# chrhansk/sleqp

Hardware: AMD Instinct MI355X
Metric: KKT factor+solve/sec (numeric refactor + 1 solve with device-controlled refinement, inputs resident in HBM) (higher is better)
Workload: dtype f64; 1 GPU; banded_n1e5_m5e4; n=100000, m=50000, N=150000, nnz_J=1000000, nnz_tril_K=1100000, nnz_L=11646539, nnz_L_stored=12226637, supernodes=569, etree_levels=10, refine_steps=1, hip_graphs=5, solves_per_factor=1, parallelism=single

## Files before the change

sleqp_amd/csrc/abi_options.inc:

```
enum OptionEffect {
  FX_NONE,
  FX_GRAPHS,
  FX_GRAPHS_IF_CHANGED,
  FX_PLANS,
  FX_PLANS_IF_CHANGED,
};
struct OptionRow {
  const char* name;
  const char* env;
  OptionEffect effect;
  int (*set)(hipfact_handle* h, double v);
  const char* doc;
};
#define OPT_STORE(field, conv)                 \
  [](hipfact_handle* h, double v) -> int {     \
    const auto x = (conv);                     \
    const bool changed = h->field != x;        \
    h->field = x;                              \
    return changed;                            \
  }
static const OptionRow kOptions[] = {
    {"refine_steps", "HIPFACT_REFINE", FX_GRAPHS,
     [](hipfact_handle* h, double v) -> int {
       h->refine_steps = std::max(0, (int)v);
// ... 68 lines not shown
       h->check_interval_now = 0;
       return 1;
     },
     "residual check on every k-th solve of a well-conditioned factorisation"},
    {"decide_lazy", "HIPFACT_DECIDE_LAZY", FX_GRAPHS_IF_CHANGED,
     [](hipfact_handle* h, double v) -> int {
       const bool changed = h->decide_lazy != (v != 0.0);
       if (changed) flush_decide(h);
       h->decide_lazy = v != 0.0;
       return changed;
     },
     "0: every solve graph ends with its own verdict launch"},
    {"rhs_fused", "HIPFACT_RHS_FUSED", FX_GRAPHS_IF_CHANGED, OPT_STORE(rhs_fused, v != 0.0),
     "0: k_rhs_saddle in front of the single-launch solve"},
    {"spanel_fold", "HIPFACT_SPANEL_FOLD", FX_PLANS_IF_CHANGED, OPT_STORE(spanel_fold, v != 0.0),
     "0: the solve panels in a launch of their own behind the factorisation"},
    {"spanel_fold_room", nullptr, FX_PLANS_IF_CHANGED, OPT_STORE(spanel_fold_room, (int)v),
     "solve-panel items dealt in beside a level's own pivot and panel items of the dataflow launch: workgroup slots per level (default 224)"},
    {"factor_hint_peek", "HIPFACT_HINT_PEEK", FX_NONE, OPT_STORE(factor_hint_peek, v != 0.0),
     "0: a refactorisation does not look at the last delivered refinement verdict (every first solve graph carries a correction pass)"},
    {"top_block_breakeven", nullptr, FX_NONE, OPT_STORE(top_block_breakeven, (int)v),
     "solves of one factorisation from which forming the dense top block of the solve tree pays (default 48)"},
    {"solve_fused", nullptr, FX_PLANS, OPT_STORE(solve_fused, v != 0.0),
     "0: the per-level solve kernels on the factor panels"},
    {"top_block_after", "HIPFACT_TOP_BLOCK_AFTER", FX_PLANS, OPT_STORE(top_block_after, std::max(0, (int)v)),
     "the top levels of the solve tree as one dense block from this solve of a factorisation on (0: never)"},
    {"boundary_fast", "HIPFACT_BOUNDARY_FAST", FX_NONE,
     [](hipfact_handle* h, double v) -> int {
       h->boundary_fast = v != 0.0;
       h->sol_prefetched = false;
       return 1;
     },
     "0: host vectors through pageable borrows and three blocking points (round 3)"},
    {"validate_rhs", nullptr, FX_NONE, OPT_STORE(validate_rhs, v != 0.0),
     "walk the index array of every sparse right-hand side on the host (debug)"},
    {"boundary_profile", nullptr, FX_NONE,
     [](hipfact_handle* h, double v) -> int {
       int rc = enter(h);
       if (rc) return rc;
       h->bd_profile = v != 0.0;
       if (h->bd_profile)
         for (hipEvent_t& ev : h->bd_ev)
           if (!ev) HCHECK(h, hipEventCreate(&ev));
       h->bd_stage_us = h->bd_queue_us = h->bd_rhs_us = h->bd_device_us = h->bd_d2h_us = h->bd_wait_us = h->bd_copyout_us = 0;
       h->bd_count = 0;
       h->bd_pending = false;
       return 1;
     },
     "where solve + solution spend their time (info keys bd_*); resets the sums"},
    {"superset_vtable", nullptr, FX_NONE,
     [](hipfact_handle* h, double v) -> int {
       const bool changed = h->superset_vtable != (v != 0.0);
       if (changed) h->vj->clear();
       h->superset_vtable = v != 0.0;
       return changed;
     },
     "0: no reuse across working sets (every changed pattern is analysed on its own rows; active bounds are still eliminated - exact_pattern = 1 for K as it is)"},
    {"spmv_stream", nullptr, FX_NONE, OPT_STORE(spmv_stream, v != 0.0),
     "0: every sparse product through the lanes-per-row kernel (default: matrices from spmv_stream_min entries on are streamed in row blocks)"},
    {"spmv_stream_min", nullptr, FX_NONE, OPT_STORE(spmv_stream_min, (long long)v),
     "entries from which a sparse product is streamed (default 4 M: below, the matrix lives in the Infinity Cache)"},
    {"exact_pattern", nullptr, FX_NONE,
     [](hipfact_handle* h, double v) -> int {
       const bool changed = h->exact_pattern != (v != 0.0);
       if (changed) h->vj->clear();
       h->exact_pattern = v != 0.0;
       return changed;
     },
     "1: K is analysed exactly as given - no row dictionary, unit rows of active bounds stay in the structure (what hipfact_reduced_matrix needs)"},
    {"assemble_superset", nullptr, FX_NONE, OPT_STORE(assemble_superset, v != 0.0),
     "0: hipfact_assemble_kkt analyses every working set on its own rows (no superset plan)"},
    {"plan_cache", nullptr, FX_NONE,
     [](hipfact_handle* h, double v) -> int {
       h->plan_cache_max = std::max(0, (int)v);
       while ((int)h->cache.size() > h->plan_cache_max) h->cache.pop_back();
       return 1;
     },
     "inactive plan states kept (LRU); 0: one pattern at a time"},
    {"profile", nullptr, FX_NONE,
     [](hipfact_handle* h, double v) -> int {
       if (h->prof.on) prof_collect(h);
       if (v < 0)
         for (int c = 0; c < PC_COUNT; ++c) h->prof.ms[c] = 0, h->prof.max_ms[c] = 0, h->prof.cnt[c] = 0;
       h->prof.tagged.clear();
       h->prof.on = v > 0;
       return 1;
     },
     "event-time every kernel class; value < 0 resets the counters"},
    {"ordering", nullptr, FX_PLANS, OPT_STORE(prm.ordering, (int)v),
     "0 nested dissection + AMD leaves (default), 1 AMD on the whole graph, 2 natural"},
    {"max_children", nullptr, FX_PLANS, OPT_STORE(prm.max_children, (int)v),
     "relaxed amalgamation keeps fronts at this many children (default 4 = what the pull extend-add takes in one block)"},
    {"force_generic", nullptr, FX_PLANS, OPT_STORE(prm.force_generic, v != 0.0),
     "1: no saddle-point structure detection, static 1 x 1 pivots on K as given (symmetric positive definite input: the PSD shim)"},
    {"dense_mode", nullptr, FX_PLANS, OPT_STORE(prm.dense_mode, std::min(2, std::max(0, (int)v))),
     "1: late elimination inside the tree (default), 2: low-rank correction, 0: off"},
    {nullptr, "HIPFACT_DATAFLOW_RETRY", FX_NONE, OPT_STORE(df_retry_every, std::max(0, (int)v)), nullptr},
    {nullptr, "HIPFACT_CHECK_LAUNCHES", FX_NONE, OPT_STORE(check_launches, v != 0.0), nullptr},
    {nullptr, "HIPFACT_SOL_SPLIT", FX_NONE, OPT_STORE(sol_split, v != 0.0), nullptr},
    {nullptr, "HIPFACT_XCD_CLASSES", FX_NONE, OPT_STORE(xcd_classes, std::max(1, std::min(XCD_CLASSES_MAX, (int)v))), nullptr},
};
#undef OPT_STORE

static void options_from_environment(hipfact_handle* h) {
  for (const OptionRow& row : kOptions)
    if (const char* s = row.env ? getenv(row.env) : nullptr) (void)row.set(h, (double)atoi(s));
}

int hipfact_set_option(hipfact_handle* h, const char* name, double value) {
  if (!h || !name) return HIPFACT_EINVAL;
  {
    bool known = false;
    const int rc = multi_set_option(h, name, value, known);
    if (known) return rc;
  }
  for (const OptionRow& row : kOptions) {
    if (!row.name || strcmp(name, row.name)) continue;
    const int changed = row.set(h, value);
    if (changed < 0) return changed;
    if (row.effect == FX_GRAPHS || (row.effect == FX_GRAPHS_IF_CHANGED && changed)) drop_graphs(h);
    if (row.effect == FX_PLANS || (row.effect == FX_PLANS_IF_CHANGED && changed)) invalidate_plans(h);
    return HIPFACT_OK;
  }
  h->error = std::string("unknown option: ") + name;
  return HIPFACT_EINVAL;
}

int hipfact_debug_copy(hipfact_handle* h, const char* name, void* out, size_t bytes) {
  int rc = enter(h);
  if (rc) return rc;
  if (!name || !out) return HIPFACT_EINVAL;
  auto host_copy = [&](const auto& v) {
    if (bytes > v.size() * sizeof(v[0])) {
      h->error = "hipfact_debug_copy: unknown buffer or size";
      return HIPFACT_EINVAL;
    }
    if (bytes) memcpy(out, v.data(), bytes);
    return HIPFACT_OK;
  };
  const Plan& P = h->plan;
  if (!strcmp(name, "perm")) return host_copy(P.perm);
  if (!strcmp(name, "sn_c0")) return host_copy(P.sn_c0);
  if (!strcmp(name, "sn_r")) return host_copy(P.sn_r);
  if (!strcmp(name, "sn_rowptr")) return host_copy(P.sn_rowptr);
  if (!strcmp(name, "sn_rows")) return host_copy(P.sn_rows);
  if (!strcmp(name, "sn_Loff")) return host_copy(P.sn_Loff);
  if (!strcmp(name, "late_cols")) return host_copy(P.late_cols);
  if (!strcmp(name, "sn_level")) return host_copy(P.sn_level);
  if (!strcmp(name, "dense_cols")) return host_copy(P.dense_cols);
  const DevBuf* b = nullptr;
  if (!strcmp(name, "L")) b = &h->d_L;
  else if (!strcmp(name, "U")) b = &h->d_U;
  else if (!strcmp(name, "SPf")) b = &h->d_SPf;
  else if (!strcmp(name, "SPb")) b = &h->d_SPb;
  else if (!strcmp(name, "sitems")) b = &h->d_sitems;
  else if (!strcmp(name, "y")) b = &h->d_y;
  else if (!strcmp(name, "xhat")) b = &h->d_xhat;
  else if (!strcmp(name, "ysol")) b = &h->d_ysol;
  else if (!strcmp(name, "uvec")) b = &h->d_uvec;
  else if (!strcmp(name, "dscale")) b = &h->d_dscale;
  else if (!strcmp(name, "Kval")) b = &h->d_Kval;
  else if (!strcmp(name, "mY")) b = &h->d_mY;
  if (!b || !b->p || bytes > b->bytes) {
    h->error = "hipfact_debug_copy: unknown buffer or size";
    return HIPFACT_EINVAL;
  }
  HCHECK(h, hipStreamSynchronize(h->stream));
  HCHECK(h, hipMemcpy(out, b->p, bytes, hipMemcpyDeviceToHost));
  return HIPFACT_OK;
}

int hipfact_debug_place_rows(int m, const int* Ar_ptr, long long fill_bytes, int classes, long long* bounds, int* classes_out,
                             int* grid_out, int* blocks) {
  if (m < 0 || (m > 0 && !Ar_ptr) || fill_bytes < 0 || classes < 1 || classes > XCD_CLASSES_MAX || !bounds || !classes_out ||
      !grid_out || !blocks)
    return HIPFACT_EINVAL;
  ClassBounds cb;
  *grid_out = place_rows(m, Ar_ptr, (size_t)fill_bytes, classes, cb);
  *classes_out = cb.C;
  for (int g = 0; g <= cb.C; ++g) bounds[g] = cb.b[g];
  for (int g = 0; g < cb.C; ++g) class_row_blocks(cb, g, FB / RL, blocks[2 * g], blocks[2 * g + 1]);
  return HIPFACT_OK;
}
int hipfact_debug_place_items(int nfronts, const int* counts, int classes, int* order, int* lost) {
  if (nfronts < 0 || (nfronts > 0 && !counts) || classes < 1 || classes > XCD_CLASSES_MAX) return HIPFACT_EINVAL;
  long long total = 0;
  for (int f = 0; f < nfronts; ++f) {
    if (counts[f] < 0) return HIPFACT_EINVAL;
    total += counts[f];
  }
  if (total >= (1LL << 31) || (total > 0 && (!order || !lost))) return HIPFACT_EINVAL;
  std::vector<int> o, l;
  deal_items(std::vector<int>(counts, counts + nfronts), classes, o, &l);
  for (size_t i = 0; i < o.size(); ++i) {
    order[i] = o[i];
    lost[i] = l[i];
  }
  return HIPFACT_OK;
}

int hipfact_debug_multi_slices(int u, int slice_rows, int* tile_bounds, int cap) {
  if (u < 0 || !multi_slice_rows_valid(slice_rows)) return HIPFACT_EINVAL;
  const int ns = multi_nslice(u, slice_rows);
  if (tile_bounds && ns <= cap)
    for (int k = 0; k <= ns; ++k) tile_bounds[k] = multi_slice_tile(u, ns, k);
  return ns;
}

int hipfact_get_info(const hipfact_handle* h, const char* name, double* value) {
  if (!h || !name || !value) return HIPFACT_EINVAL;
  const Plan& P = h->plan;
  if (!strncmp(name, "prof_", 5)) {
    prof_collect(const_cast<hipfact_handle*>(h));
    if (!strcmp(name, "prof_schur_best_flops") || !strcmp(name, "prof_schur_best_ms")) {
      double fmax = 0.0, best_rate = 0.0, bf = 0.0, bm = 0.0;
      for (auto& t : h->prof.tagged) fmax = std::max(fmax, t.first);
      for (auto& t : h->prof.tagged)
        if (t.first >= 0.5 * fmax && t.second > 0.0 && t.first / t.second > best_rate) {
          best_rate = t.first / t.second;
          bf = t.first;
          bm = t.second;
        }
      *value = !strcmp(name, "prof_schur_best_flops") ? bf : bm;
      return HIPFACT_OK;
    }
    for (int c = 0; c < PC_COUNT; ++c) {
      const size_t len = strlen(kProfNames[c]);
      if (!strncmp(name + 5, kProfNames[c], len) && name[5 + len] == '_') {
        if (!strcmp(name + 6 + len, "ms")) {
          *value = h->prof.ms[c];
          return HIPFACT_OK;
        }
        if (!strcmp(name + 6 + len, "count")) {
          *value = (double)h->prof.cnt[c];
          return HIPFACT_OK;
        }
        if (!strcmp(name + 6 + len, "max_ms")) {
          *value = h->prof.max_ms[c];
          return HIPFACT_OK;
        }
      }
    }
    return HIPFACT_EINVAL;
  }
  if (!strncmp(name, "level_", 6)) {
    const char* us = strrchr(name, '_');
    const int l = atoi(us + 1);
    if (us == name + 5 || l < 0 || l >= P.nlevels || (int)P.level_ptr.size() <= l + 1) return HIPFACT_EINVAL;
    const size_t len = (size_t)(us - (name + 6));
    double fronts = 0, ent = 0, rows = 0, flops = 0, blk = 0;
    for (int q = P.level_ptr[l]; q < P.level_ptr[l + 1]; ++q) {
      const int s = P.level_sn[q];
      const double w = P.sn_c0[s + 1] - P.sn_c0[s], r = P.sn_r[s];
      fronts += 1;
      ent += w * r - w * (w - 1) / 2;
      blk += w * (w + 1) / 2;
      rows += r;
      for (int k = 0; k < (int)w; ++k) flops += (r - k) * (r - k);
    }
    if (len == 6 && !strncmp(name + 6, "fronts", 6)) *value = fronts;
    else if (len == 3 && !strncmp(name + 6, "ent", 3)) *value = ent;
    else if (len == 3 && !strncmp(name + 6, "blk", 3)) *value = blk;
    else if (len == 4 && !strncmp(name + 6, "rows", 4)) *value = rows;
    else if (len == 5 && !strncmp(name + 6, "flops", 5)) *value = flops;
    else return HIPFACT_EINVAL;
    return HIPFACT_OK;
  }
#define INFO(key, expr)       \
  if (!strcmp(name, key)) {   \
    *value = (double)(expr);  \
    return HIPFACT_OK;        \
  }
  INFO("N", h->have_plan ? h->N_ext : P.N) INFO("n", P.n) INFO("m", P.m) INFO("saddle", P.saddle) INFO("nnzK", P.nnzK) INFO("nnzL", P.nnzL)
  INFO("nnzL_true", P.nnzL_true) INFO("flops", P.flops) INFO("flops_dense", P.flops_dense) INFO("nsuper", P.nsuper)
  INFO("nlevels", P.nlevels) INFO("nprod", P.nprod) INFO("L_bytes", P.L_size * 8.0) INFO("U_bytes", P.U_size * 8.0)
  INFO("analysis_s", P.t_total) INFO("order_s", P.t_order) INFO("symbolic_s", P.t_symbolic)
  INFO("num_perturbed", h->num_perturbed) INFO("static_pivot_runs", h->static_pivot_runs) INFO("static_pivot_shift", h->reg_delta)
  INFO("num_zero_pivots", h->info_host[INFO_ZERO_PIVOT]) INFO("num_neg_pivots", h->info_host[INFO_NEG_PIVOT])
  INFO("cache_hits", h->cache_hits) INFO("plan_swaps", h->plan_swaps) INFO("plans_cached", h->cache.size())
  INFO("no_dataflow", h->no_dataflow) INFO("dataflow_fallbacks", h->dataflow_fallbacks) INFO("turn_waits", (double)h->turn_waits) INFO("dataflow_rearmed", h->dataflow_rearmed) INFO("fused_solve", h->fused_solve) INFO("spanel_folded", h->sp_folded) INFO("solve_items", h->n_sitems) INFO("chain_levels_fused", [&] { int c = 0; for (const LevelInfo& li : h->levels) c += li.mini_cnt > 0; return c; }()) INFO("solve_panel_bytes", h->sp_bytes) INFO("spf_bytes", (double)h->d_SPf.bytes) INFO("spb_bytes", (double)h->d_SPb.bytes) INFO("sitem_bytes", (double)sizeof(SolveItem)) INFO("N_internal", P.N) INFO("maps_on", h->maps_on) INFO("m_struct", h->m_struct) INFO("analyses", h->analyses) INFO("num_factor", h->num_factor) INFO("cg_device_runs", h->cg_device_runs) INFO("cg_device_fallbacks", h->cg_device_fallbacks) INFO("lz_device_runs", h->lz_device_runs) INFO("lz_device_fallbacks", h->lz_device_fallbacks) INFO("lz_device_iterations", h->lz_device_iterations) INFO("lsqr_runs", h->lsqr_runs) INFO("lsqr_iters", h->lsqr_iters) INFO("dense_columns", h->nd) INFO("late_columns", P.n_late) INFO("late_rows", P.n_late_rows) INFO("m_rows", P.saddle ? P.my : P.m) INFO("vtable_rows", h->vj->rows()) INFO("vtable_retries", h->vtable_retries) INFO("dense_fallbacks", h->dense_fallbacks) INFO("dense_probes", h->dense_probes) INFO("top_block_cols", h->tb_nT) INFO("top_block_below", h->tb_nfb) INFO("top_block_levels", h->tb_levels) INFO("top_block_items", h->tb_ntf) INFO("top_block_builds", h->tb_builds) INFO("top_block_active", h->tb_valid) INFO("superset_vtable", h->superset_vtable) INFO("exact_pattern", h->exact_pattern) INFO("spmv_stream", h->spmv_stream)
  INFO("boundary_fast", h->boundary_fast) INFO("bd_count", h->bd_count) INFO("bd_stage_us", h->bd_stage_us) INFO("bd_queue_us", h->bd_queue_us) INFO("bd_rhs_us", h->bd_rhs_us) INFO("bd_device_us", h->bd_device_us) INFO("bd_d2h_us", h->bd_d2h_us) INFO("bd_wait_us", h->bd_wait_us) INFO("bd_copyout_us", h->bd_copyout_us)
  INFO("multi_solves", h->multi_solves) INFO("multi_cols", h->multi_cols) INFO("multi_blocks", h->multi_blocks)
  INFO("multi_passes", h->multi_passes) INFO("multi_single_cols", h->multi_single_cols) INFO("multi_failed_col", h->multi_failed_col)
  INFO("multi_sliced_fronts", h->mitems_for < 0 ? 0 : h->n_mcut) INFO("multi_slice_items", h->mitems_for < 0 ? 0 : h->n_mslices) INFO("multi_slice_rows", h->multi_slice_rows)
  INFO("extra_solves", h->extra_solves) INFO("extra_passes", h->extra_passes) INFO("extra_last_status", h->extra_last_status)
  INFO("num_solve", h->num_solve) INFO("num_refined", h->num_refined) INFO("refine_adaptive", h->refine_adaptive)
  INFO("num_passes", h->num_passes) INFO("last_omega", h->last_ctl.omega) INFO("last_iters", h->last_ctl.iters)
  INFO("last_status", h->last_ctl.status) INFO("last_tol", h->last_ctl.tol) INFO("kappa_est", h->last_ctl.kappa)
  INFO("refine_inline", h->refine_inline) INFO("refine_tol", h->refine_tol) INFO("equilibrate", h->equilibrate)
  INFO("factor_top_level", h->ftop_level) INFO("factor_top_count", h->ftop_count) INFO("solve_timeouts", h->h_info.p ? h->h_info.as<int>()[INFO_TIMEOUT] : 0)
  INFO("top_level", 1 << 30)
  INFO("use_graph", h->use_graph) INFO("num_graphs", h->graphs.size()) INFO("max_r", P.max_r) INFO("max_w", P.max_w) INFO("refine_steps", h->refine_steps)
  INFO("schur_flops_max_level", h->schur_flops_max)
  INFO("chain_pairs", h->n_pairs)
  INFO("xupd_fused", h->xupd_fused ? 1 : 0)
  INFO("rhs_in_tree", h->last_rhs_in_tree) INFO("xupd_in_tree", h->last_xupd_in_tree) INFO("xupd_blocks_launched", h->last_xupd_blocks)
  INFO("solve_sliced_fronts", h->n_sliced) INFO("solve_resorted_levels", h->n_resorted) INFO("tree_solve", tree_solve(h))
  INFO("refine_check_every", h->refine_check_every) INFO("refine_check_interval", h->check_interval_now) INFO("num_checked", h->num_checked)
  INFO("device", h->device) INFO("nnzM", P.Mi.size()) INFO("nnzA", P.Ar_src.size())
  INFO("rows_total", P.sn_rows.size()) INFO("ent_fused", h->ent_fused) INFO("ent_split", h->ent_split)
  INFO("rows_fused", h->rows_fused) INFO("rows_split", h->rows_split)
  INFO("long_row_segments", h->n_rseg) INFO("row_scale_blocks", row_scale_in_sequence(h) ? h->rs_grid : 0)
  INFO("arena_fill_bytes", arena_fill_bytes(P))
  INFO("xcd_classes", h->xcd_classes) INFO("dealt_multi_item_fronts", h->dealt_multi) INFO("long_prod_segments", h->n_lprod)
  INFO("active_bounds", h->maps_on ? h->n_bounds : 0)
  INFO("values_in_place",
       h->have_plan && (!h->from_jacobian || (virtual_current(h) && h->vj->identity))) INFO("inactive_rows", h->maps_on ? h->n_inactive : 0)
#undef INFO
  return HIPFACT_EINVAL;
}
```

sleqp_amd/csrc/device_types.h:

```cpp
#pragma once
#include <cstdint>

namespace hipfact {

struct SnDesc {
  long long Loff;
  long long Uoff;
  long long uoff;
  long long rowoff;
  long long reloff;
  int c0;
  int w;
  int r;
  int parent;
  int child_begin;
  int child_end;
  int pad0;
  int pad1;
};

constexpr int MAXCH = 4;
struct PullDesc {
  long long Uoff[MAXCH];
  long long reloff[MAXCH];
  int invoff[MAXCH];
  int uc[MAXCH];
  int n;
  int next;
  int pad[2];
};

struct FrontItem {
  long long Loff, Uoff;
  int w, r;
  int part;
  int nchild;
  PullDesc pd;
};

struct PairDesc {
  long long Loff_a, Uoff_g;
  int w_a, r_a, rowoff_a;
  int u_g, off_g;
};

struct TopFItem {
  FrontItem it;
  int role;
  int front;
  int part2;
  int nwait;
  int wait_id[MAXCH];
  int wait_cnt[MAXCH];
  int target;
  int crows;
  int prows;
  int sidx, scount;
  int post;
  long long xoff;
  int head;
  int wait_head[MAXCH];
};

struct SolveItem {
  long long spf, spb;
  long long uoff, rowoff;
  int c0, w, r, nchild;
  int Qf, Ef, Pb, Eb;
  long long c_uoff[MAXCH];
  int c_invoff[MAXCH];
  long long Loff;
  int xbegin, xend;
  int a0, a1, sl, nsl;
  long long poff;
  int plevel, pad_;
};
constexpr int LONG_ROW = 1024;
constexpr int LONG_COL = 256;
constexpr int LONG_SEG = 2048;
struct LongSeg {
  int id;
  int begin, end;
  int idx, nseg;
  int uid;
  int poff;
  int pad;
};
struct LongProd {
  long long e;
  long long begin, end;
  int idx, nseg, uid, poff;
};
constexpr int XCD_CLASSES_MAX = 16;
struct ClassBounds {
  long long b[XCD_CLASSES_MAX + 1];
  int C, pad;
};
#ifdef __HIP__
#define HIPFACT_HD __host__ __device__
#else
#define HIPFACT_HD
#endif
HIPFACT_HD inline void class_row_blocks(const ClassBounds& cb, int g, int rpb, int& rb0, int& nrb) {
  rb0 = (int)((cb.b[g] + rpb - 1) / rpb);
  nrb = (int)((cb.b[g + 1] + rpb - 1) / rpb) - rb0;
}
struct TopBlockItem {
  long long off;
  int r0, nr;
  int Q, E;
};
struct TopFront {
  int item;
  int parent;
  int tl0;
  int pad;
};
struct TopChunk {
  int front;
  int j0;
};
constexpr int TOP_CB = 4;
constexpr int TOP_LDS = 7 * 1024 + 512;
constexpr int SPMV_NNZ = 2048;
constexpr int SPMV_T = 256;
constexpr int TREE_LDS = 2 * 1024 + 8;
struct TopBlockIn {
  int nT, ntf;
  const TopBlockItem* __restrict__ items;
  const double* __restrict__ XTf;
  const int* __restrict__ tpos;
  const int* __restrict__ gptr;
  const long long* __restrict__ gsrc;
  double* __restrict__ xhatT2;
  double* __restrict__ tT2;
  int ntr;
  unsigned int* __restrict__ gathered2;
  int ltop;
};
constexpr int SOLVE_PREFETCH = 32;

enum { INFO_ZERO_PIVOT = 0, INFO_NEG_PIVOT = 1, INFO_TIMEOUT = 2, INFO_TIMEOUT_WG = 3, INFO_WORDS = 4 };
constexpr int INFO_BYTES = INFO_WORDS * 4 + 32;

}
```

sleqp_amd/csrc/kernels_factor_top.inc:

```

__device__ __forceinline__ void flag_wait_ge(int* __restrict__ addr, int target, int* __restrict__ info) {
  if (threadIdx.x == 0) {
    int spins = 0;
    while (__hip_atomic_load(addr, __ATOMIC_RELAXED, __HIP_MEMORY_SCOPE_AGENT) < target) {
      __builtin_amdgcn_s_sleep(2);
      if (++spins > (1 << 22)) {
        atomicAdd(&info[INFO_TIMEOUT], 1);
        break;
      }
    }
    __builtin_amdgcn_fence(__ATOMIC_ACQUIRE, "agent");
    asm volatile("s_waitcnt vmcnt(0)" ::: "memory");
  }
  __syncthreads();
}

__device__ __forceinline__ void flag_publish_add(int* __restrict__ addr) {
  asm volatile("s_waitcnt vmcnt(0)" ::: "memory");
  __syncthreads();
  if (threadIdx.x == 0) {
    FACTOR_RELEASE_FENCE();
    asm volatile("s_waitcnt vmcnt(0)" ::: "memory");
    __hip_atomic_fetch_add(addr, 1, __ATOMIC_RELAXED, __HIP_MEMORY_SCOPE_AGENT);
  }
}

__device__ __forceinline__ void dev_build_solve_panel(const SolveItem& T, const double* __restrict__ L,
                                                      double* __restrict__ SPf, double* __restrict__ SPb, double* lds);

__global__ __launch_bounds__(512) void k_factor_top(const TopFItem* __restrict__ items, double* __restrict__ L,
                                                   double* __restrict__ U, int* __restrict__ info,
                                                   const int* __restrict__ inv, const int* __restrict__ rel,
                                                   int* __restrict__ bdone, int* __restrict__ cdone,
                                                   int* __restrict__ ddone, double* __restrict__ xarena,
                                                   const SolveItem* __restrict__ sitems, double* __restrict__ SPf,
                                                   double* __restrict__ SPb) {
  extern __shared__ __attribute__((aligned(16))) double lds[];
  const TopFItem& T = items[blockIdx.x];
  const FrontItem& S = T.it;
  TRW(0);
#ifdef HIPFACT_TRACE
  if (threadIdx.x == 0 && blockIdx.x < TRACE_WGS) g_trace[blockIdx.x * 8 + 7] = T.role * 100000 + T.front;
#endif
  if (T.role == 3) {
    if (T.nwait) {
      if (threadIdx.x == 0) {
        int spins = 0;
        while ((__hip_atomic_load(&bdone[T.front], __ATOMIC_RELAXED, __HIP_MEMORY_SCOPE_AGENT) & 15) < 1 ||
               __hip_atomic_load(&cdone[T.front], __ATOMIC_RELAXED, __HIP_MEMORY_SCOPE_AGENT) < T.target) {
          __builtin_amdgcn_s_sleep(8);
          if (++spins > (1 << 22)) {
            atomicAdd(&info[INFO_TIMEOUT], 1);
            break;
          }
        }
        __builtin_amdgcn_fence(__ATOMIC_ACQUIRE, "agent");
        asm volatile("s_waitcnt vmcnt(0)" ::: "memory");
      }
      __syncthreads();
    }
    TRW(1);
    dev_build_solve_panel(sitems[S.part], L, SPf, SPb, lds);
#ifdef HIPFACT_TRACE
    __syncthreads();
#endif
    TRW(2);
    return;
  }
  FrontCtx c = make_ctx(S, L, U, lds);
  c.wt = true;
  c.Xa = T.post ? xarena + T.xoff : nullptr;
  const PullCtx pc = make_pull(S.pd, U, inv, rel, 1);
  ChildWait cw;
  cw.n = T.nwait;
  cw.info = info;
#pragma unroll
  for (int ch = 0; ch < MAXCH; ++ch) {
    cw.addr[ch] = ddone + T.wait_id[ch];
    cw.target[ch] = T.wait_cnt[ch];
  }
  if (T.role == 0) {
    int* hdone = ddone + (ddone - cdone);
#pragma unroll
    for (int ch = 0; ch < MAXCH; ++ch)
      if (T.wait_head[ch] > 0 && ch < T.nwait && T.wait_cnt[ch] > 0) {
        cw.addr[ch] = hdone + T.wait_id[ch];
        cw.target[ch] = T.wait_head[ch];
      }
  }
  if (T.role == 0) {
    dev_pivot_block<false, false, true>(c, info, 15, pc, cw);
    dev_store_pivot_block(c);
    TRW(2);
    flag_publish_add(&bdone[T.front]);
    TRW(3);
    if (T.sidx > 0) {
      const SolveItem& Q = sitems[T.sidx - 1];
      const int w = c.w, r = c.r, lda = c.lda;
      const int lane = threadIdx.x & 63, wave = threadIdx.x >> 6;
      const long long TSf = (long long)r * Q.Qf, TSb = (long long)w * Q.Pb;
      double* __restrict__ sf = SPf + Q.spf;
      double* __restrict__ sb = SPb + Q.spb;
      for (int k = wave; k < w; k += 8) {
        const long long of = (long long)(k / Q.Qf) * TSf + (long long)(k % Q.Qf) * r;
        for (int i = k + lane; i < w; i += 64) sf[of + i] = (i == k) ? 1.0 : c.A[i + k * lda];
      }
      for (int i = wave; i < w; i += 8) {
        const double di = 1.0 / c.dd[i];
        const long long ob = (long long)(i / Q.Pb) * TSb + (long long)(i % Q.Pb) * w;
        for (int k = lane; k <= i; k += 64) sb[ob + k] = ((i == k) ? 1.0 : c.A[i + k * lda]) * di;
      }
    }
  } else if (T.role == 1) {
    TRW(5);
    cw.wait();
    int* invl = reinterpret_cast<int*>(c.A + c.wp * c.lda);
#pragma unroll
    for (int ch = 0; ch < MAXCH; ++ch)
      if (ch < pc.n)
        for (int k = threadIdx.x; k < c.wp; k += blockDim.x) invl[ch * c.wp + k] = (k < c.w) ? pc.inv[ch][k] : -1;
    const int wv = threadIdx.x >> 6;
    const int cstep = T.prows == 64 ? 2 : 1;
    const int R0 = c.w + T.prows * S.part + 16 * (cstep == 2 ? (wv >> 1) : wv);
    double pv[8][4];
    int cis[MAXCH];
    if (c.Xa) {
      const bool mine = 16 * wv < T.prows;
      const int R1 = c.w + T.prows * S.part + 16 * wv;
      const int Rs = mine ? R1 : c.r;
      dev_panel_rows_load<true>(c, Rs, pc, pv, cis);
      __syncthreads();
      dev_panel_rows_gather<true>(c, pc, invl, pv, cis);
      TRW(1);
      dev_panel_rows_subst_posted(c, Rs, pv, mine && R1 < c.r, S.part == 0, info);
      TRW(2);
      flag_publish_add(&cdone[T.front]);
      TRW(3);
      return;
    }
    dev_panel_rows_load(c, R0, pc, pv, cis);
    __syncthreads();
    dev_panel_rows_gather(c, pc, invl, pv, cis);
    if (c.Xa) {
      dev_panel_rows_product_posted(c, R0, pv, cstep, cstep == 2 ? (wv & 1) : 0, R0 < c.r, info);
    } else {
      flag_wait_ge(&bdone[T.front], 1, info);
      TRW(1);
      dev_load_pivot_block(c, true, true);
      if (R0 < c.r) dev_panel_rows_product<true, true>(c, R0, pv, cstep, cstep == 2 ? (wv & 1) : 0);
    }
    TRW(2);
    flag_publish_add(&cdone[T.front]);
    TRW(3);
  } else if (T.role == 4) {
#define FUSED_ARGS c, S.part >> 16, S.part & 0xffff, pc, cw, info, &bdone[T.front], &cdone[T.front], &ddone[T.front], T.target
    if (T.crows == 32) {
      if (c.nbk == 6)
        dev_fused_tile<32, 6>(FUSED_ARGS);
      else
        dev_fused_tile<32, 0>(FUSED_ARGS);
    } else {
      if (c.nbk == 6)
        dev_fused_tile<64, 6>(FUSED_ARGS);
      else
        dev_fused_tile<64, 0>(FUSED_ARGS);
    }
#undef FUSED_ARGS
  } else {
    cw.wait();
    if (T.crows == 64) {
      dev_schur_tile32(c, S.part >> 16, S.part & 0xffff, pc, &cdone[T.front], T.target, info);
    } else {
      const int team = threadIdx.x >> 8;
      const int ij = team ? T.part2 : S.part;
      double* SI = c.A + (size_t)team * (2 * 64 * KC + 64 * MAXCH);
      dev_schur_tile<false>(c, SI, SI + 64 * KC, ij < 0 ? -1 : (ij >> 16), ij & 0xffff, S.nchild == 0, pc,
                            threadIdx.x & 255, &cdone[T.front], T.target, info);
    }
    if (c.Xa)
      for (int e = T.sidx * 512 + threadIdx.x; e < c.wp * c.wp; e += T.scount * 512) sent_f64(c.Xa + e);
    TRW(2);
    flag_publish_add(&ddone[T.front]);
    if (T.head && threadIdx.x == 0)
      __hip_atomic_fetch_add(ddone + (ddone - cdone) + T.front, 1, __ATOMIC_RELAXED, __HIP_MEMORY_SCOPE_AGENT);
    TRW(3);
  }
}
```

sleqp_amd/csrc/kernels_solve_panels.inc:

```
#define SPST(p, v) (*(p) = (v))

__device__ __forceinline__ void dev_build_solve_panel(const SolveItem& T, const double* __restrict__ L,
                                                      double* __restrict__ SPf, double* __restrict__ SPb, double* lds) {
  const int w = T.w, r = T.r;
  const int ua = T.a0, u = T.a1 - T.a0;
  const int top = (T.sl == 0) ? w : 0;
  const int ro = top + u;
  const int tid = threadIdx.x, lane = tid & 63, wave = tid >> 6;
  const int li = lane & 15, lk = lane >> 4;
  const int nbk = (w + 15) >> 4, wp = nbk << 4;
  const int ldx = wp + 1;
  const double* __restrict__ Pn = L + T.Loff;
  double* X = lds;
  double* dinv = X + (size_t)ldx * wp;
  double* tile = dinv + wp + (size_t)wave * (16 * 17);
  long long* offF = reinterpret_cast<long long*>(dinv + wp + (SPB / 64) * (16 * 17));
  long long* offB = offF + wp;
  const int nstrip = (u + 15) >> 4;
  double av[32];
  {
    const int a0 = wave << 4;
    const bool rowok = wave < nstrip && a0 + li < u;
    const double* __restrict__ Lr = Pn + w + ua + a0 + li;
#pragma unroll
    for (int t = 0; t < 32; ++t) {
      const int j = 4 * t + lk;
      av[t] = (rowok && j < w) ? Lr[(long long)j * r] : 0.0;
    }
  }
  for (int k0 = wave; k0 < wp; k0 += 8 * (SPB / 64)) {
    double v[8][2];
#pragma unroll
    for (int t = 0; t < 8; ++t)
#pragma unroll
      for (int h2 = 0; h2 < 2; ++h2) {
        const int k = k0 + t * (SPB / 64), i = lane + 64 * h2;
        v[t][h2] = (i == k) ? 1.0 : 0.0;
        if (i < w && k < w && i > k) v[t][h2] = Pn[i + (long long)k * r];
      }
#pragma unroll
    for (int t = 0; t < 8; ++t)
#pragma unroll
      for (int h2 = 0; h2 < 2; ++h2) {
        const int k = k0 + t * (SPB / 64), i = lane + 64 * h2;
        if (k < wp && i < wp) X[i + k * ldx] = v[t][h2];
      }
  }
  for (int k = tid; k < wp; k += SPB) dinv[k] = (k < w) ? 1.0 / Pn[k + (long long)k * r] : 1.0;
  const int Qf = T.Qf, Pb = T.Pb;
  const long long TSf = (long long)ro * Qf, TSb = (long long)w * Pb;
  for (int k = tid; k < wp; k += SPB) offF[k] = (long long)(k / Qf) * TSf + (long long)(k % Qf) * ro;
  for (int i = tid; i < ro; i += SPB) offB[i] = (long long)(i / Pb) * TSb + (long long)(i % Pb) * w;
  __syncthreads();
  double* __restrict__ sf = SPf + T.spf;
  double* __restrict__ sb = SPb + T.spb;
  for (int st = wave; st < nstrip; st += SPB / 64) {
    const int a0 = st << 4;
    d4_t acc[8];
#pragma unroll
    for (int t = 0; t < 8; ++t) acc[t] = d4_t{0.0, 0.0, 0.0, 0.0};
#pragma unroll
    for (int t = 0; t < 32; ++t) {
      const int j0 = 4 * t;
      if (j0 < wp) {
#pragma unroll
        for (int kt = 0; kt < 8; ++kt)
          if (16 * kt <= j0 + 3 && kt < nbk) acc[kt] = MFMA_F64(av[t], X[(j0 + lk) + (16 * kt + li) * ldx], acc[kt]);
      }
    }
    {
      const int an = (st + SPB / 64) << 4;
      const bool rowok = st + SPB / 64 < nstrip && an + li < u;
      const double* __restrict__ Lr = Pn + w + ua + an + li;
#pragma unroll
      for (int t = 0; t < 32; ++t) {
        const int j = 4 * t + lk;
        av[t] = (rowok && j < w) ? Lr[(long long)j * r] : 0.0;
      }
    }
#pragma unroll
    for (int kt = 0; kt < 8; ++kt) {
      if (kt >= nbk) continue;
#pragma unroll
      for (int q = 0; q < 4; ++q) {
        const int row = lk + 4 * q, k = 16 * kt + li, i = top + a0 + row;
        tile[row * 17 + li] = -acc[kt][q];
        if (a0 + row < u && k < w) SPST(&sb[offB[i] + k], -acc[kt][q]);
      }
      __builtin_amdgcn_fence(__ATOMIC_RELEASE, "wavefront");
      __builtin_amdgcn_wave_barrier();
      __builtin_amdgcn_fence(__ATOMIC_ACQUIRE, "wavefront");
#pragma unroll
      for (int q = 0; q < 4; ++q) {
        const int row = li, col = lk + 4 * q, k = 16 * kt + col, i = top + a0 + row;
        if (a0 + row < u && k < w) SPST(&sf[offF[k] + i], tile[row * 17 + col]);
      }
      __builtin_amdgcn_fence(__ATOMIC_RELEASE, "wavefront");
      __builtin_amdgcn_wave_barrier();
    }
  }
  if (top == 0) return;
  for (int k = wave; k < w; k += SPB / 64)
    for (int i = k + lane; i < w; i += 64) SPST(&sf[offF[k] + i], X[i + k * ldx]);
  for (int i = wave; i < w; i += SPB / 64) {
    const double di = dinv[i];
    for (int k = lane; k <= i; k += 64) SPST(&sb[offB[i] + k], X[i + k * ldx] * di);
  }
}
__global__ __launch_bounds__(SPB) void k_build_solve_panels(const SolveItem* __restrict__ items,
                                                            const double* __restrict__ L, double* __restrict__ SPf,
                                                            double* __restrict__ SPb) {
  extern __shared__ __attribute__((aligned(16))) double lds[];
  dev_build_solve_panel(items[blockIdx.x], L, SPf, SPb, lds);
}
```

sleqp_amd/csrc/kernels_solve_tree.inc:

```

__device__ __forceinline__ void dev_refine_decide(const DecideIn& D, int first) {
  RefineCtl* __restrict__ ctl = D.ctl;
  RefineCtl* __restrict__ hctl = D.hctl;
  __shared__ double sh[3][16];
  const int tid = threadIdx.x, nthr = blockDim.x;
  double r = 0.0, bb = 0.0, zz = 0.0;
  for (int q = tid; q < D.nblk; q += nthr) {
    r = nanmax(r, D.partials[3 * q]);
    bb = nanmax(bb, D.partials[3 * q + 1]);
    zz = nanmax(zz, D.partials[3 * q + 2]);
  }
#pragma unroll
  for (int o = 32; o > 0; o >>= 1) {
    r = nanmax(r, __shfl_down(r, o, 64));
    bb = nanmax(bb, __shfl_down(bb, o, 64));
    zz = nanmax(zz, __shfl_down(zz, o, 64));
  }
  if ((tid & 63) == 0) {
    sh[0][tid >> 6] = r;
    sh[1][tid >> 6] = bb;
    sh[2][tid >> 6] = zz;
  }
  __syncthreads();
  if (tid == 0) {
// ... 23 lines not shown
    } else if (!first && omega > 0.5 * prev) {
      done = 1;
      status = 1;
    }
    ctl->iters = iters;
    ctl->omega_prev = prev;
    ctl->omega = omega;
    ctl->tol = tol;
    ctl->kappa = kappa;
    ctl->rnorm = r;
    ctl->bnorm = bb;
    ctl->status = status;
    ctl->seq = seq;
    ctl->pending = 0;
    ctl->done = done;
    hctl->iters = iters;
    hctl->omega_prev = prev;
    hctl->omega = omega;
    hctl->tol = tol;
    hctl->kappa = kappa;
    hctl->rnorm = r;
    hctl->bnorm = bb;
    hctl->status = status;
    hctl->done = done;
    __hip_atomic_store(&hctl->seq, seq, __ATOMIC_RELAXED, __HIP_MEMORY_SCOPE_SYSTEM);
  }
}
__global__ __launch_bounds__(FB) void k_refine_decide(DecideIn D, int first, int pending_only) {
  if (pending_only) {
    if (!D.ctl->pending) return;
  } else if (!first && D.ctl->done) {
    return;
  }
  dev_refine_decide(D, first);
}

__device__ __forceinline__ double rhs_row_tail(const RhsIn& R, int k, double s) {
  const int i = ext_row(R.M, R.perm[k]);
  return i >= 0 ? s - R.b[i] * R.M.dscale[k] : (i == -2 ? s : 0.0);
}
template <int NT>
__device__ __forceinline__ void rhs_long_rows(const RhsIn& R, int bid, int nb, double* __restrict__ t, double* lds) {
  for (int q = bid; q < R.M.nrseg; q += nb) {
    const LongSeg sg = R.M.rseg[q];
    double s = 0.0;
    for (int p = sg.begin + (int)threadIdx.x; p < sg.end; p += NT) {
      const int j = R.Ar_col[p], v = R.M.vmap ? R.M.vmap[j] : -1;
      s += R.Ar_val[p] * R.b[v >= 0 ? v : j];
    }
    s = block_sum_fixed<NT>(s, lds);
    double tot;
    if (threadIdx.x == 0 && seg_arrive(s, sg.poff, sg.idx, sg.nseg, R.M.segpart, R.M.segcnt + sg.uid, tot))
      t[sg.id] = rhs_row_tail(R, sg.id, tot);
  }
}
__device__ __forceinline__ double rhs_row(const RhsIn& R, int k, int sub) {
  double s = 0.0;
  const int p1 = R.Ar_ptr[k + 1];
  if (p1 - R.Ar_ptr[k] > LONG_ROW) return 0.0;
  if (R.M.vmap) {
    for (int p = R.Ar_ptr[k] + sub; p < p1; p += RL) {
      const int j = R.Ar_col[p], v = R.M.vmap[j];
      s += R.Ar_val[p] * R.b[v >= 0 ? v : j];
    }
  } else {
    for (int p = R.Ar_ptr[k] + sub; p < p1; p += RL) s += R.Ar_val[p] * R.b[R.Ar_col[p]];
  }
#pragma unroll
  for (int o = RL / 2; o > 0; o >>= 1) s += __shfl_down(s, o, RL);
  if (sub == 0) s = rhs_row_tail(R, k, s);
  return s;
}

__device__ __forceinline__ void dev_solve_fwd(const SolveItem& T, const double* __restrict__ SPf,
                                              const long long* __restrict__ xuoff, const int* __restrict__ xinvoff,
                                              const int* __restrict__ inv, const double* __restrict__ y,
                                              double* __restrict__ xhat, double* __restrict__ uvec,
                                              double* __restrict__ ysol, double* lds, int* __restrict__ info,
                                              const RhsIn& R) {
  const int tid = threadIdx.x;
  const int w = T.w, Q = T.Qf, E = T.Ef;
  const int a0 = T.a0, nu = T.a1 - T.a0;
  const int top = (T.sl == 0) ? w : 0;
  const int ro = top + nu;
  const int rl = w + nu;
  const int TS = ro * Q;
  const bool active = tid < TS;
  const int q = active ? tid / ro : 0;
  double* f = lds;
  double* part = lds + rl;
  if (tid < w) sent_f64(ysol + T.c0 + tid);
  const double* __restrict__ sp = SPf + T.spf + tid;
  double pv[SOLVE_PREFETCH];
  const int myrow_f = tid - q * ro;
  const int clim = (active && myrow_f < top) ? myrow_f : (1 << 30);
#pragma unroll
  for (int e = 0; e < SOLVE_PREFETCH; ++e) pv[e] = (active && e < E && q + Q * e <= clim) ? sp[(long long)e * TS] : 0.0;
  const int fr = tid + (tid >= w ? a0 : 0);
  double f0 = 0.0;
  if (R.Ar_ptr) {
    for (int row = tid / RL; row < w; row += ST / RL) {
      const double s = rhs_row(R, T.c0 + row, tid % RL);
      if (tid % RL == 0) part[row] = s;
    }
    __syncthreads();
    if (tid < w) f0 = part[tid];
  } else if (tid < w) {
    f0 = y[T.c0 + tid];
  }
  int iv[MAXCH];
#pragma unroll
  for (int ch = 0; ch < MAXCH; ++ch) iv[ch] = (ch < T.nchild && tid < rl) ? inv[T.c_invoff[ch] + fr] : -1;
  {
    unsigned long long bits[MAXCH];
#pragma unroll
    for (int ch = 0; ch < MAXCH; ++ch)
      bits[ch] = iv[ch] >= 0 ? __hip_atomic_load(reinterpret_cast<const unsigned long long*>(uvec + T.c_uoff[ch] + iv[ch]),
                                                 __ATOMIC_RELAXED, __HIP_MEMORY_SCOPE_AGENT)
                             : 0ull;
#pragma unroll
    for (int ch = 0; ch < MAXCH; ++ch)
      if (iv[ch] >= 0) {
        if (bits[ch] == SOLVE_SENT) bits[ch] = (unsigned long long)__double_as_longlong(poll_f64(uvec + T.c_uoff[ch] + iv[ch], info));
        f0 += __longlong_as_double((long long)bits[ch]);
      }
  }
  for (int x = T.xbegin; x < T.xend; ++x) {
    const int ia = (tid < rl) ? inv[xinvoff[x] + fr] : -1;
    if (ia >= 0) f0 += poll_f64(uvec + xuoff[x] + ia, info);
  }
  if (tid < rl) f[tid] = f0;
  __syncthreads();
  double acc = 0.0;
#pragma unroll
  for (int e = 0; e < SOLVE_PREFETCH; ++e)
    if (e < E) acc = fma(pv[e], f[min(q + Q * e, w - 1)], acc);
  for (int e = SOLVE_PREFETCH; e < E; ++e)
    if (active && q + Q * e <= clim) acc = fma(sp[(long long)e * TS], f[min(q + Q * e, w - 1)], acc);
  if (active) part[tid] = acc;
  __syncthreads();
  if (tid < ro) {
    double s2 = 0.0;
    for (int qq = 0; qq < Q; ++qq) s2 += part[qq * ro + tid];
    if (tid < top) {
      post_f64(xhat + T.c0 + tid, s2);
    } else {
      const int j = tid - top;
      post_f64(uvec + T.uoff + a0 + j, f[w + j] + s2);
    }
  }
}

template <bool DEFER_RESET>
__device__ __forceinline__ void dev_solve_bwd(const SolveItem& T, const double* __restrict__ SPb,
                                              const int* __restrict__ rows, double* __restrict__ y,
                                              double* __restrict__ xhat, double* __restrict__ uvec,
                                              double* __restrict__ ysol, double* __restrict__ spart, double* lds,
                                              int* __restrict__ info, const unsigned int* __restrict__ gathered = nullptr,
                                              int ngather = 0) {
  const int tid = threadIdx.x;
  const int w = T.w, P = T.Pb, E = T.Eb;
  const int a0 = T.a0, nu = T.a1 - T.a0;
  const int top = (T.sl == 0) ? w : 0;
  const int ro = top + nu;
  const int TS = w * P;
  const bool active = tid < TS;
  const int p = active ? tid / w : 0;
  double* tv = lds;
  double* part = lds + ro;
  const double* __restrict__ sp = SPb + T.spb + tid;
  double pv[SOLVE_PREFETCH];
  const int mycol_b = tid - p * w;
#pragma unroll
  for (int e = 0; e < SOLVE_PREFETCH; ++e) {
    const int row = p + P * e;
    pv[e] = (active && e < E && !(row < top && row < mycol_b)) ? sp[(long long)e * TS] : 0.0;
  }
  const int myrow = (tid >= top && tid < ro) ? rows[T.rowoff + w + a0 + (tid - top)] : -1;
  if (tid < top) {
    tv[tid] = poll_f64(xhat + T.c0 + tid, info);
    sent_f64_agent(xhat + T.c0 + tid);
  } else if (myrow >= 0) {
    tv[tid] = poll_f64(ysol + myrow, info);
  }
  if constexpr (!DEFER_RESET) {
    if (tid >= top && tid < ro) sent_f64_agent(uvec + T.uoff + a0 + (tid - top));
  }
  __syncthreads();
  double acc = 0.0;
#pragma unroll
  for (int e = 0; e < SOLVE_PREFETCH; ++e)
    if (e < E) acc = fma(pv[e], tv[min(p + P * e, ro - 1)], acc);
  for (int e = SOLVE_PREFETCH; e < E; ++e)
    if (active && !(p + P * e < top && p + P * e < mycol_b)) acc = fma(sp[(long long)e * TS], tv[min(p + P * e, ro - 1)], acc);
  if (active) part[tid] = acc;
  __syncthreads();
  if (tid < w) {
    double s2 = 0.0;
    for (int pp = 0; pp < P; ++pp) s2 += part[pp * w + tid];
    if (T.sl > 0) {
      post_f64(spart + T.poff + (long long)(T.sl - 1) * w + tid, s2);
    } else {
      for (int s0 = 1; s0 < T.nsl; s0 += 16) {
        unsigned long long bits[16];
#pragma unroll
        for (int j = 0; j < 16; ++j) {
          const int s = s0 + j;
          bits[j] = s < T.nsl ? __hip_atomic_load(reinterpret_cast<const unsigned long long*>(
                                                      spart + T.poff + (long long)(s - 1) * w + tid),
                                                  __ATOMIC_RELAXED, __HIP_MEMORY_SCOPE_AGENT)
                              : 0ull;
        }
#pragma unroll
        for (int j = 0; j < 16; ++j) {
          const int s = s0 + j;
          if (s < T.nsl) {
            double* slot = spart + T.poff + (long long)(s - 1) * w + tid;
            if (bits[j] == SOLVE_SENT) bits[j] = (unsigned long long)__double_as_longlong(poll_f64(slot, info));
            s2 += __longlong_as_double((long long)bits[j]);
            sent_f64_agent(slot);
          }
        }
      }
      y[T.c0 + tid] = s2;
      post_f64(ysol + T.c0 + tid, s2);
    }
  }
  if constexpr (DEFER_RESET) {
   if (tid >= top && tid < ro) {
    int spins = 0;
    while ((int)__hip_atomic_load(gathered, __ATOMIC_RELAXED, __HIP_MEMORY_SCOPE_AGENT) < ngather) {
      __builtin_amdgcn_s_sleep(1);
      if (++spins > (1 << 20)) {
        atomicAdd(&info[INFO_TIMEOUT], 1);
        atomicMax(&info[INFO_TIMEOUT_WG], (1 << 30) - (int)blockIdx.x);
        break;
      }
    }
    sent_f64_agent(uvec + T.uoff + a0 + (tid - top));
   }
  }
}

__device__ __forceinline__ void dev_top_one(const TopBlockIn& B, const TopBlockItem& I, double* __restrict__ y,
                                            const double* __restrict__ uvec, double* __restrict__ ysol_prev,
                                            double* __restrict__ ysol, int par, double* lds, int* __restrict__ info) {
  const int tid = threadIdx.x;
  const int nT = B.nT, nr = I.nr, Q = I.Q, E = I.E;
  const int TS = nr * Q;
  const bool active = tid < TS;
  const int q = tid % Q, rho = tid / Q;
  double* f = lds;
  double* part = lds + nT;
  const double* __restrict__ sp = B.XTf + I.off + tid;
  double pv[SOLVE_PREFETCH];
#pragma unroll
  for (int e = 0; e < SOLVE_PREFETCH; ++e) pv[e] = (active && e < E) ? sp[(long long)e * TS] : 0.0;
  if (tid < nr) {
    sent_f64(ysol_prev + B.tpos[I.r0 + tid]);
    sent_f64(B.tT2 + (size_t)(1 - par) * nT + I.r0 + tid);
  }
  if (tid == 0 && I.r0 == 0) __hip_atomic_store(B.gathered2 + (1 - par), 0u, __ATOMIC_RELAXED, __HIP_MEMORY_SCOPE_AGENT);
  const double* __restrict__ tT = B.tT2 + (size_t)par * nT;
  int* gp = reinterpret_cast<int*>(lds + nT + ST);
  int* gs = gp + nT + 1;
  const int nG = B.gptr[nT];
  for (int i = tid; i <= nT; i += ST) gp[i] = B.gptr[i];
  for (int g = tid; g < nG; g += ST) gs[g] = (int)B.gsrc[g];
  __syncthreads();
  constexpr int GK = 6;
  for (int i = tid; i < nT; i += ST) {
    const int g0 = gp[i], g1 = gp[i + 1];
    unsigned long long bits[GK + 1];
    const double* src[GK + 1];
    src[0] = B.ntr > 0 ? tT + i : y + B.tpos[i];
#pragma unroll
    for (int k = 0; k < GK; ++k) src[k + 1] = (g0 + k < g1) ? uvec + gs[g0 + k] : nullptr;
#pragma unroll
    for (int k = 0; k <= GK; ++k)
      bits[k] = src[k] ? __hip_atomic_load(reinterpret_cast<const unsigned long long*>(src[k]), __ATOMIC_RELAXED,
                                           __HIP_MEMORY_SCOPE_AGENT)
                       : 0ull;
    double f0 = 0.0;
#pragma unroll
    for (int k = 0; k <= GK; ++k)
      if (src[k]) {
        if (bits[k] == SOLVE_SENT && !(k == 0 && B.ntr == 0)) bits[k] = (unsigned long long)__double_as_longlong(poll_f64(src[k], info));
        f0 += __longlong_as_double((long long)bits[k]);
      }
    for (int g = g0 + GK; g < g1; ++g) f0 += poll_f64(uvec + gs[g], info);
    f[i] = f0;
  }
  __syncthreads();
  double acc = 0.0;
#pragma unroll
  for (int e = 0; e < SOLVE_PREFETCH; ++e)
    if (e < E) acc = fma(pv[e], f[min(q + Q * e, nT - 1)], acc);
  for (int e = SOLVE_PREFETCH; e < E; ++e)
    if (active) acc = fma(sp[(long long)e * TS], f[min(q + Q * e, nT - 1)], acc);
  acc = wave_sum(acc);
  if (Q == 64) {
    if ((tid & 63) == 0 && active) {
      const int k = B.tpos[I.r0 + rho];
      y[k] = acc;
      post_f64(ysol + k, acc);
    }
  } else {
    if ((tid & 63) == 0) part[tid >> 6] = acc;
    __syncthreads();
    if (tid < nr) {
      const int kq = Q >> 6;
      double s2 = 0.0;
      for (int j = 0; j < kq; ++j) s2 += part[tid * kq + j];
      const int k = B.tpos[I.r0 + tid];
      y[k] = s2;
      post_f64(ysol + k, s2);
    }
  }
  if (tid == 0) __hip_atomic_fetch_add(B.gathered2 + par, 1u, __ATOMIC_RELAXED, __HIP_MEMORY_SCOPE_AGENT);
}

__global__ __launch_bounds__(FB) void k_top_dinv(int nT, const double* __restrict__ SPb, const long long* __restrict__ dsrc,
                                                 double* __restrict__ dinv) {
  const int c = blockIdx.x * FB + threadIdx.x;
  if (c < nT) dinv[c] = SPb[dsrc[c]];
}
__device__ __forceinline__ int top_syrk_nseg(int nT, int I) {
  const int cstart = (I * ZT) & ~(ZC - 1);
  return (nT - cstart + ZS - 1) / ZS;
}
__global__ __launch_bounds__(FB) void k_top_syrk_mfma(const double* __restrict__ Xd, const double* __restrict__ dinv,
                                                      double* __restrict__ Zp, int nT) {
  __shared__ double As[ZC * (ZT + 1)];
  __shared__ double Bs[ZC * (ZT + 1)];
  const int nt = (nT + ZT - 1) / ZT, ntl = nt * (nt + 1) / 2;
  int t = (int)blockIdx.x, I = 0;
  for (; I < nt; ++I) {
    const int cnt = (I + 1) * top_syrk_nseg(nT, I);
    if (t < cnt) break;
    t -= cnt;
  }
  const int nseg = top_syrk_nseg(nT, I);
  const int J = t / nseg, seg = t % nseg;
  const int I0 = I * ZT, J0 = J * ZT;
  const int tid = threadIdx.x, lane = tid & 63, wave = tid >> 6;
  const int li = lane & 15, lk = lane >> 4;
  const int i0 = 32 * (wave & 1), j0 = 32 * (wave >> 1);
  d4_t acc[2][2];
#pragma unroll
  for (int x = 0; x < 2; ++x)
#pragma unroll
    for (int y = 0; y < 2; ++y) acc[x][y] = (d4_t){0.0, 0.0, 0.0, 0.0};
  constexpr int NE = ZC * ZT / FB;
  const int cc = tid % ZC, ib = tid / ZC;
  double ra[NE], rb[NE];
  auto request = [&](int c0) {
    const int c = c0 + cc;
    const double dv = c < nT ? dinv[c] : 0.0;
#pragma unroll
    for (int e = 0; e < NE; ++e) {
      const int ii = ib + (FB / ZC) * e;
      ra[e] = (c < nT && I0 + ii < nT && c >= I0 + ii) ? Xd[(size_t)c + (size_t)(I0 + ii) * nT] * dv : 0.0;
      rb[e] = (c < nT && J0 + ii < nT && c >= J0 + ii) ? Xd[(size_t)c + (size_t)(J0 + ii) * nT] : 0.0;
    }
  };
  const int cbeg = (I0 & ~(ZC - 1)) + seg * ZS, cend = min(nT, cbeg + ZS);
  request(cbeg);
  for (int c0 = cbeg; c0 < cend; c0 += ZC) {
    __syncthreads();
#pragma unroll
    for (int e = 0; e < NE; ++e) {
      const int ii = ib + (FB / ZC) * e;
      As[cc * (ZT + 1) + ii] = ra[e];
      Bs[cc * (ZT + 1) + ii] = rb[e];
    }
    __syncthreads();
    if (c0 + ZC < cend) request(c0 + ZC);
#pragma unroll
    for (int k0 = 0; k0 < ZC; k0 += 4) {
      const int kk = (k0 + lk) * (ZT + 1);
      const double a0 = Bs[kk + j0 + li], a1 = Bs[kk + j0 + 16 + li];
      const double b0 = As[kk + i0 + li], b1 = As[kk + i0 + 16 + li];
      acc[0][0] = MFMA_F64(a0, b0, acc[0][0]);
      acc[0][1] = MFMA_F64(a0, b1, acc[0][1]);
      acc[1][0] = MFMA_F64(a1, b0, acc[1][0]);
      acc[1][1] = MFMA_F64(a1, b1, acc[1][1]);
    }
  }
  double* __restrict__ out = Zp + ((size_t)seg * ntl + (size_t)(I * (I + 1) / 2 + J)) * (ZT * ZT);
#pragma unroll
  for (int x = 0; x < 2; ++x)
#pragma unroll
    for (int y = 0; y < 2; ++y)
#pragma unroll
      for (int q = 0; q < 4; ++q) out[(i0 + 16 * y + li) + (j0 + 16 * x + lk + 4 * q) * ZT] = acc[x][y][q];
}
__global__ __launch_bounds__(FB) void k_top_syrk_reduce(const double* __restrict__ Zp, double* __restrict__ Zd, int nT) {
  const int nt = (nT + ZT - 1) / ZT, ntl = nt * (nt + 1) / 2;
  int I = (int)((sqrt(8.0 * (double)blockIdx.x + 1.0) - 1.0) * 0.5);
  while (I * (I + 1) / 2 > (int)blockIdx.x) --I;
  while ((I + 1) * (I + 2) / 2 <= (int)blockIdx.x) ++I;
  const int J = (int)blockIdx.x - I * (I + 1) / 2;
  const int nseg = top_syrk_nseg(nT, I);
  for (int e = threadIdx.x; e < ZT * ZT; e += FB) {
    double s2 = 0.0;
    for (int sg = 0; sg < nseg; ++sg) s2 += Zp[((size_t)sg * ntl + blockIdx.x) * (ZT * ZT) + e];
    const int i = I * ZT + e % ZT, j = J * ZT + e / ZT;
    if (i < nT && j < nT) {
      Zd[(size_t)i + (size_t)j * nT] = s2;
      if (I != J) Zd[(size_t)j + (size_t)i * nT] = s2;
    }
  }
}

__global__ __launch_bounds__(ST) void k_top_inverse(const TopChunk* __restrict__ chunks,
                                                    const TopFront* __restrict__ fronts,
                                                    const SolveItem* __restrict__ items,
                                                    const double* __restrict__ SPf, const int* __restrict__ rows,
                                                    const int* __restrict__ tl, double* __restrict__ Xd, int nT) {
  __shared__ double vP[TOP_CB][128];
  __shared__ long long offF[128];
  const int tid = threadIdx.x;
  const TopChunk ch = chunks[blockIdx.x];
  const int j0 = ch.j0;
  int g = ch.front;
  const int colbase = fronts[g].tl0 + j0;
  const int ncol = min(TOP_CB, items[fronts[g].item].w - j0);
  bool first = true;
  while (g >= 0) {
    const TopFront F = fronts[g];
    const SolveItem& T = items[F.item];
    const int w = T.w, r = T.r, Qf = T.Qf;
    const long long TSf = (long long)r * Qf;
    const double* __restrict__ sf = SPf + T.spf;
    for (int k = tid; k < w; k += ST) offF[k] = (long long)(k / Qf) * TSf + (long long)(k % Qf) * r;
    for (int idx = tid; idx < w * TOP_CB; idx += ST) {
      const int i = idx % w, cc = idx / w;
      double v = 0.0;
      if (cc < ncol) v = first ? ((i == j0 + cc) ? 1.0 : 0.0) : Xd[(size_t)(F.tl0 + i) + (size_t)(colbase + cc) * nT];
      vP[cc][i] = v;
    }
    __syncthreads();
    for (int idx = tid; idx < r * TOP_CB; idx += ST) {
      const int i = idx % r, cc = idx / r;
      if (cc >= ncol) continue;
      const int kmax = i < w ? i : w - 1;
      double acc = 0.0;
      for (int k = 0; k <= kmax; ++k) acc = fma(sf[offF[k] + i], vP[cc][k], acc);
      const size_t col = (size_t)(colbase + cc) * nT;
      if (i < w)
        Xd[(size_t)(F.tl0 + i) + col] = acc;
      else
        Xd[(size_t)tl[rows[T.rowoff + i]] + col] += acc;
    }
    __syncthreads();
    g = F.parent;
    first = false;
  }
}
__global__ __launch_bounds__(ST) void k_top_format(TopBlockIn B, const double* __restrict__ Xd, double* __restrict__ XTf) {
  const int it = blockIdx.x;
  const TopBlockItem I = B.items[it];
  const int nT = B.nT, nr = I.nr, Q = I.Q, E = I.E;
  const int TS = nr * Q;
  const int tid = threadIdx.x;
  if (tid >= TS) return;
  const int q = tid % Q, rho = tid / Q;
  const size_t row = (size_t)(I.r0 + rho);
  double* __restrict__ out = XTf + I.off + tid;
  for (int e = 0; e < E; ++e) {
    const int c = q + Q * e;
    double v = 0.0;
    if (c < nT) v = Xd[row + (size_t)c * nT];
    out[(long long)e * TS] = v;
  }
}

__device__ __forceinline__ double x_col_write(const SaddleMaps& M, int j, double s, const double* __restrict__ b,
                                              double* __restrict__ z, int acc) {
  const int v = M.vmap ? M.vmap[j] : -1;
  const double bj = b[j];
  if (v >= 0) {
    const double beta = b[v];
    const double mult = (bj - beta) - s;
    if (acc) {
      z[j] += beta;
      z[v] += mult;
    } else {
      z[j] = beta;
      z[v] = mult;
    }
    return bj * beta;
  }
  if (acc) {
    z[j] += bj - s;
    return 0.0;
  }
  const double zj = bj - s;
  z[j] = zj;
  return bj * zj;
}
template <bool POLL, int NT>
__device__ __forceinline__ double x_long_cols(const SaddleMaps& M, int bid, int nb, const int* __restrict__ Kp,
                                              const double* __restrict__ Ksc, const int* __restrict__ Kc_y,
                                              const double* __restrict__ ys, const double* __restrict__ b,
                                              double* __restrict__ z, int acc, int* __restrict__ info, double* lds) {
  double dsum = 0.0;
  for (int q = bid; q < M.ncseg; q += nb) {
    const LongSeg sg = M.cseg[q];
    double s = 0.0;
    for (int e = sg.begin + (int)threadIdx.x; e < sg.end; e += NT)
      s += Ksc[e] * (POLL ? poll_f64(ys + Kc_y[e], info) : ys[Kc_y[e]]);
    s = block_sum_fixed<NT>(s, lds);
    double tot;
    if (threadIdx.x == 0 && seg_arrive(s, sg.poff, sg.idx, sg.nseg, M.segpart, M.segcnt + sg.uid, tot))
      dsum += x_col_write(M, sg.id, tot, b, z, acc);
  }
  return dsum;
}
__device__ __forceinline__ void dev_x_update(const XupdIn& X, int xb, const double* __restrict__ ys, int m,
                                             int* __restrict__ info, double* lds) {
  constexpr int XL = 8, XE = 2, XP = 4;
  const int sub = threadIdx.x % XL;
  const int cpb = ST / XL;
  const int stride = X.nblocks * cpb;
  const SaddleMaps& M = X.M;
  const unsigned long long* __restrict__ yb = reinterpret_cast<const unsigned long long*>(ys);
  const int k0 = xb * ST + threadIdx.x, kstride = X.nblocks * ST;
  int yi = -1;
  double ysc = 0.0, dsum = 0.0;
  if (k0 < m) {
    yi = ext_row(M, X.perm[k0]);
    ysc = M.dscale[k0];
  }
  for (int jb = xb * cpb + threadIdx.x / XL; jb < X.n; jb += XP * stride) {
    double val[XP][XE];
    int idx[XP][XE], enext[XP], eend[XP];
    bool colok[XP];
#pragma unroll
    for (int p = 0; p < XP; ++p) {
      const int j = jb + p * stride;
      bool ok = j < X.n;
      int e0 = ok ? X.Kp[j] + 1 + sub : 0, e1 = ok ? X.Kp[j + 1] : 0;
      if (e1 - (e0 - sub) > LONG_COL) e1 = e0 = 0, ok = false;
      colok[p] = ok;
#pragma unroll
      for (int t = 0; t < XE; ++t) {
        const int e = e0 + XL * t;
        val[p][t] = (e < e1) ? X.Ksc[e] : 0.0;
        idx[p][t] = (e < e1) ? X.Kc_y[e] : -1;
      }
      enext[p] = e0 + XL * XE;
      eend[p] = e1;
    }
    unsigned long long bits[XP][XE];
#pragma unroll
    for (int p = 0; p < XP; ++p)
#pragma unroll
      for (int t = 0; t < XE; ++t)
        bits[p][t] = (idx[p][t] >= 0) ? __hip_atomic_load(yb + idx[p][t], __ATOMIC_RELAXED, __HIP_MEMORY_SCOPE_AGENT) : 0ull;
#pragma unroll
    for (int p = 0; p < XP; ++p) {
      const int j = jb + p * stride;
      double s = 0.0;
#pragma unroll
      for (int t = 0; t < XE; ++t)
        if (idx[p][t] >= 0) {
          const double yv = (bits[p][t] == SOLVE_SENT) ? poll_f64(ys + idx[p][t], info) : __longlong_as_double((long long)bits[p][t]);
          s += val[p][t] * yv;
        }
      for (int e = enext[p]; e < eend[p]; e += XL) s += X.Ksc[e] * poll_f64(ys + X.Kc_y[e], info);
#pragma unroll
      for (int o = XL / 2; o > 0; o >>= 1) s += __shfl_down(s, o, XL);
      if (sub == 0 && colok[p]) dsum += x_col_write(M, j, s, X.b, X.z, X.acc);
    }
  }
  if (M.ncseg > 0) {
    const double dl = x_long_cols<true, ST>(M, xb, X.nblocks, X.Kp, X.Ksc, X.Kc_y, ys, X.b, X.z, X.acc, info, lds);
    if (threadIdx.x == 0) dsum += dl;
    __syncthreads();
  }
  if (X.dot_out) {
    dsum = wave_sum(dsum);
    if ((threadIdx.x & 63) == 0) lds[threadIdx.x >> 6] = dsum;
    __syncthreads();
    if (threadIdx.x == 0) {
      double a = 0.0;
      for (int q = 0; q < ST / 64; ++q) a += lds[q];
      X.dot_out[xb] = a;
    }
  }
  for (int k = k0; k < m; k += kstride) {
    const int i = (k == k0) ? yi : ext_row(M, X.perm[k]);
    if (i >= 0) {
      const double v = poll_f64(ys + k, info) * ((k == k0) ? ysc : M.dscale[k]);
      if (X.acc)
        X.z[i] += v;
      else
        X.z[i] = v;
    }
  }
}

__global__ __launch_bounds__(ST) void k_solve_tree(const SolveItem* __restrict__ items, int nfwd, int bwd_off, int nbwd,
                                                   TopBlockIn TB,
                                                   const double* __restrict__ SPf, const double* __restrict__ SPb,
                                                   const long long* __restrict__ xuoff,
                                                   const int* __restrict__ xinvoff, const int* __restrict__ inv,
                                                   const int* __restrict__ rows, double* __restrict__ y,
                                                   double* __restrict__ xhat,
                                                   double* __restrict__ uvec, double* __restrict__ ysol2, int m,
                                                   int* __restrict__ epoch, int* __restrict__ info,
                                                   const int* __restrict__ skip, RhsIn R, DecideIn D,
                                                   double* __restrict__ spart, XupdIn X) {
  extern __shared__ __attribute__((aligned(16))) double lds[];
  const int ntop = TB.ntf;
  const int nall = TB.ntr + nfwd + ntop + nbwd;
  if ((int)blockIdx.x == nall) {
    if (D.ctl && D.ctl->pending) dev_refine_decide(D, 1);
    return;
  }
  if (skip && *skip) return;
  const int readers = (int)gridDim.x - 1;
  auto epoch_read_done = [&]() {
    if (X.nblocks == 0) return;
    __syncthreads();
    if (threadIdx.x == 0 &&
        __hip_atomic_fetch_add(epoch + 1, 1, __ATOMIC_RELAXED, __HIP_MEMORY_SCOPE_AGENT) == readers - 1) {
      __hip_atomic_store(epoch + 1, 0, __ATOMIC_RELAXED, __HIP_MEMORY_SCOPE_AGENT);
      __hip_atomic_fetch_add(epoch, 1, __ATOMIC_RELAXED, __HIP_MEMORY_SCOPE_AGENT);
    }
  };
  if ((int)blockIdx.x < TB.ntr) {
    const int par0 = *epoch & 1;
    const int i = (int)blockIdx.x * (ST / RL) + (int)threadIdx.x / RL;
    if (i < TB.nT) {
      const double s = rhs_row(R, TB.tpos[i], threadIdx.x % RL);
      if (threadIdx.x % RL == 0) post_f64(TB.tT2 + (size_t)par0 * TB.nT + i, s);
    }
    epoch_read_done();
    return;
  }
  const int par = *epoch & 1;
  if ((int)blockIdx.x > nall) {
    const int xb = (int)blockIdx.x - nall - 1;
    dev_x_update(X, xb, ysol2 + (size_t)par * m, m, info, lds);
    epoch_read_done();
    return;
  }
  const int b = (int)blockIdx.x - TB.ntr;
  if (b < nfwd) {
    const SolveItem& T = items[b];
    dev_solve_fwd(T, SPf, xuoff, xinvoff, inv, y, xhat, uvec, ysol2 + (size_t)(1 - par) * m, lds, info, R);
  } else if (b < nfwd + TB.ntf) {
    dev_top_one(TB, TB.items[b - nfwd], y, uvec, ysol2 + (size_t)(1 - par) * m, ysol2 + (size_t)par * m, par, lds, info);
  } else {
    const SolveItem& T = items[bwd_off + (b - nfwd - ntop)];
    if (TB.ntf > 0 && T.plevel >= TB.ltop)
      dev_solve_bwd<true>(T, SPb, rows, y, xhat, uvec, ysol2 + (size_t)par * m, spart, lds, info, TB.gathered2 + par, TB.ntf);
    else
      dev_solve_bwd<false>(T, SPb, rows, y, xhat, uvec, ysol2 + (size_t)par * m, spart, lds, info);
  }
  epoch_read_done();
}
```

sleqp_amd/csrc/runtime_plan.inc:

```

static void prof_begin(hipfact_handle* h, int cls) {
  Prof& p = h->prof;
  if (!p.on) return;
  if (p.used + 2 > p.ev.size()) {
    hipEvent_t a, b;
    if (hipEventCreate(&a) != hipSuccess || hipEventCreate(&b) != hipSuccess) return;
    p.ev.push_back(a);
    p.ev.push_back(b);
  }
  p.cls.resize(p.ev.size() / 2);
  p.fl.resize(p.ev.size() / 2);
  p.cls[p.used / 2] = cls;
  p.fl[p.used / 2] = p.next_fl;
  p.next_fl = 0.0;
  (void)hipEventRecord(p.ev[p.used], h->stream);
}
static void prof_end(hipfact_handle* h) {
  Prof& p = h->prof;
  if (!p.on || p.used + 2 > p.ev.size()) return;
  (void)hipEventRecord(p.ev[p.used + 1], h->stream);
  p.used += 2;
}
static void prof_collect(hipfact_handle* h) {
  Prof& p = h->prof;
  if (p.used == 0) return;
  (void)hipStreamSynchronize(h->stream);
  for (size_t i = 0; i < p.used; i += 2) {
    float ms = 0.f;
    if (hipEventElapsedTime(&ms, p.ev[i], p.ev[i + 1]) == hipSuccess) {
      p.ms[p.cls[i / 2]] += ms;
      p.max_ms[p.cls[i / 2]] = std::max(p.max_ms[p.cls[i / 2]], (double)ms);
      p.cnt[p.cls[i / 2]] += 1;
      if (p.fl[i / 2] > 0.0 && p.tagged.size() < 65536) p.tagged.push_back({p.fl[i / 2], (double)ms});
    }
  }
  p.used = 0;
}
static void launch_check(hipfact_handle* h, const char* kernel, dim3 grid, dim3 block, size_t lds) {
  const hipError_t e = hipPeekAtLastError();
  if (e != hipSuccess && !h->launch_reported) {
    h->launch_reported = true;
    fprintf(stderr, "[hipfact] launch of %s failed: %s (grid %u, block %u, LDS %zu bytes)\n", kernel, hipGetErrorString(e),
            grid.x, block.x, lds);
  }
}
#define LAUNCH(cls, kernel, grid, block, lds, ...)                         \
  do {                                                                     \
    prof_begin(h, cls);                                                    \
    hipLaunchKernelGGL(kernel, grid, block, lds, h->stream, __VA_ARGS__);  \
    if (h->check_launches) launch_check(h, #kernel, grid, block, lds);     \
    prof_end(h);                                                           \
  } while (0)

template <class T, class A>
static int upload(hipfact_handle* h, DevBuf& buf, const std::vector<T, A>& v) {
  HCHECK(h, buf.ensure(std::max<size_t>(v.size() * sizeof(T), 16)));
  if (!v.empty()) HCHECK(h, hipMemcpyAsync(buf.p, v.data(), v.size() * sizeof(T), hipMemcpyHostToDevice, h->stream));
  return HIPFACT_OK;
}

static size_t solve_panel_lds(int wmax) {
  const size_t wp = (size_t)((wmax + 15) & ~15);
  return (wp * (wp + 1) + wp + 8 * 16 * 17 + wp + 1024) * sizeof(double);
}

static int dense_upload(hipfact_handle* h, size_t vec_bytes);

static void place_front_end(hipfact_handle* h);

static int upload_plan(hipfact_handle* h) {
  const Plan& P = h->plan;
  const int ns = P.nsuper;
  std::vector<SnDesc> sn(ns);
  for (int s = 0; s < ns; ++s) {
    SnDesc& d = sn[s];
    d.Loff = P.sn_Loff[s];
    d.Uoff = P.sn_Uoff[s];
    d.uoff = P.sn_uoff[s];
    d.rowoff = P.sn_rowptr[s];
    d.reloff = P.rel_ptr[s];
    d.c0 = P.sn_c0[s];
    d.w = P.sn_c0[s + 1] - P.sn_c0[s];
    d.r = P.sn_r[s];
    d.parent = P.sn_parent[s];
    d.child_begin = P.child_ptr[s];
    d.child_end = P.child_ptr[s + 1];
    d.pad0 = P.sn_level[s];
    d.pad1 = 0;
  }
  std::vector<int> pair_role(ns, 0), pair_g(ns, -1);
  long long pair_slot = 0;
  if (h->chain_pairs && h->pull_max_children > 0 && h->chain_fuse && h->factor_top_max > 0) {
    auto single = [&](int l) { return l >= 0 && l < P.nlevels && P.level_ptr[l + 1] - P.level_ptr[l] == 1; };
    auto nch = [&](int s2) { return P.child_ptr[s2 + 1] - P.child_ptr[s2]; };
    int run_pairs = 0;
    for (int l = 1; l + 1 < P.nlevels;) {
      bool ok = single(l) && single(l + 1);
      int a = -1, b = -1, c = -1;
      if (ok) {
        a = P.level_sn[P.level_ptr[l]];
        b = P.level_sn[P.level_ptr[l + 1]];
        ok = P.sn_parent[a] == b && nch(b) == 1 && nch(a) == 1;
      }
      if (ok) {
        c = P.child_idx[P.child_ptr[a]];
        const int ua = sn[a].r - sn[a].w, ub = sn[b].r - sn[b].w, uc = sn[c].r - sn[c].w;
        ok = sn[a].r == uc && sn[b].r == ua && ub > h->factor_top_max_u && ub >= 512 && (long long)ua * ua < (1LL << 40);
      }
      if (!ok) {
        run_pairs = 0;
        ++l;
        continue;
      }
      const long long ua = sn[a].r - sn[a].w;
      pair_role[a] = 1;
      pair_role[b] = 2;
      pair_g[b] = c;
      pair_slot = std::max(pair_slot, (ua * ua + 1) & ~1LL);
      sn[a].pad0 = sn[a].pad0;
      sn[a].Uoff = -(long long)(1 + (run_pairs & 1));
      sn[b].Uoff = sn[a].Uoff;
      ++run_pairs;
      l += 2;
    }
    for (int s = 0; s < ns; ++s)
      if (pair_role[s]) sn[s].Uoff = P.U_size + (-(sn[s].Uoff) - 1) * pair_slot;
  }
  h->pair_extra = 2 * pair_slot;
  h->n_pairs = 0;
  for (int s = 0; s < ns; ++s) h->n_pairs += pair_role[s] == 2;
  std::vector<int> inv;
  {
    long long total = 0;
    for (int s = 0; s < ns; ++s)
      if (P.sn_parent[s] >= 0) total += P.sn_r[P.sn_parent[s]];
    if (total >= (1LL << 31)) {
      h->error = "inverse index map exceeds 2^31 entries";
      return HIPFACT_EINTERNAL;
    }
    inv.assign((size_t)total, -1);
    long long off = 0;
    for (int s = 0; s < ns; ++s) {
      const int p = P.sn_parent[s];
      if (p < 0) continue;
      sn[s].pad1 = (int)off;
      const int us = P.sn_r[s] - (P.sn_c0[s + 1] - P.sn_c0[s]);
      for (int a = 0; a < us; ++a) inv[(size_t)off + P.rel[P.rel_ptr[s] + a]] = a;
      off += P.sn_r[p];
    }
  }
  std::vector<PullDesc> pulls(ns), pullx;
  for (int s = 0; s < ns; ++s) {
    const int nch = P.child_ptr[s + 1] - P.child_ptr[s];
    PullDesc* cur = &pulls[s];
    memset(cur, 0, sizeof(*cur));
    cur->next = -1;
    int last_x = -1;
    for (int k = 0; k < nch; ++k) {
      if (k > 0 && k % MAXCH == 0) {
        PullDesc nb;
        memset(&nb, 0, sizeof(nb));
        nb.next = -1;
        pullx.push_back(nb);
        const int idx = (int)pullx.size() - 1;
        (last_x < 0 ? pulls[s] : pullx[(size_t)last_x]).next = idx;
        last_x = idx;
      }
      PullDesc& pd = last_x < 0 ? pulls[s] : pullx[(size_t)last_x];
      const int ch = P.child_idx[P.child_ptr[s] + k];
      const int q = k % MAXCH;
      pd.Uoff[q] = sn[ch].Uoff;
      pd.reloff[q] = sn[ch].reloff;
      pd.invoff[q] = sn[ch].pad1;
      pd.uc[q] = sn[ch].r - sn[ch].w;
      pd.n = q + 1;
    }
  }
  int rc;
  if ((rc = upload(h, h->d_inv, inv))) return rc;
  if ((rc = upload(h, h->d_pullx, pullx))) return rc;
  if ((rc = upload(h, h->d_sn, sn))) return rc;
  if ((rc = upload(h, h->d_level_sn, P.level_sn))) return rc;
  if ((rc = upload(h, h->d_rows, P.sn_rows))) return rc;
  if ((rc = upload(h, h->d_rel, P.rel))) return rc;
  if ((rc = upload(h, h->d_child, P.child_idx))) return rc;
  h->idx32 = P.saddle && P.L_size < (1LL << 32) && P.nprod < (1LL << 32);
  if (h->idx32) {
    std::vector<unsigned int> t32(P.Mtarget.begin(), P.Mtarget.end());
    if ((rc = upload(h, h->d_Mtarget, t32))) return rc;
  } else if ((rc = upload(h, h->d_Mtarget, P.Mtarget)))
    return rc;
  if ((rc = upload(h, h->d_perm, P.perm))) return rc;
  if ((rc = upload(h, h->d_Kp, P.Kp))) return rc;
  if ((rc = upload(h, h->d_Ki, P.Ki))) return rc;
  if (P.saddle) {
    if (h->idx32) {
      std::vector<unsigned int> p32(P.prod_ptr.begin(), P.prod_ptr.end());
      if ((rc = upload(h, h->d_prod_ptr, p32))) return rc;
    } else if ((rc = upload(h, h->d_prod_ptr, P.prod_ptr)))
      return rc;
    {
      h->prod_packed = P.nnzK < (1LL << 24);
      const size_t np = P.prod_a.size();
      for (size_t p = 0; p < np && h->prod_packed; ++p)
        if (std::abs(P.prod_a[p] - P.prod_b[p]) > 255) h->prod_packed = false;
      if (h->prod_packed) {
        std::vector<int> pk(np);
        for (size_t p = 0; p < np; ++p)
          pk[p] = (int)(((unsigned int)std::min(P.prod_a[p], P.prod_b[p]) << 8) |
                        (unsigned int)std::abs(P.prod_a[p] - P.prod_b[p]));
        if ((rc = upload(h, h->d_prod_a, pk))) return rc;
        h->d_prod_b.release();
      } else {
        if ((rc = upload(h, h->d_prod_a, P.prod_a))) return rc;
        if ((rc = upload(h, h->d_prod_b, P.prod_b))) return rc;
      }
// ... 388 lines not shown
          return sn[a].w != sn[b].w ? sn[a].w > sn[b].w : sn[a].r > sn[b].r;
        });
        std::vector<int> narrow_first(wide_first.rbegin(), wide_first.rend());
        for (int s : wide_first) {
          tf.push_back(base(s, 0, 0));
          const size_t wp = (size_t)((sn[s].w + 15) & ~15);
          lds = std::max(lds, (wp + 2 * (size_t)(2 * 64 * 32 + 64 * MAXCH)) * sizeof(double));
        }
        if (lfused[l]) {
          static const int fused_order = getenv("HIPFACT_FUSED_ORDER") ? atoi(getenv("HIPFACT_FUSED_ORDER")) : 0;
          for (int s : (fused_order ? wide_first : narrow_first)) {
            const int sr = fused_rows(l), nt = (sn[s].r - sn[s].w + sr - 1) / sr;
            const size_t wp = (size_t)((sn[s].w + 15) & ~15);
            for (int I = 0; I < nt; ++I)
              for (int J = 0; J <= I; ++J) {
                TopFItem t = base(s, 4, (I << 16) | J);
                t.crows = sr;
                t.target = (int)nfused(s);
                tf.push_back(t);
              }
            lds = std::max(lds, (wp + wp * (wp + 1) + 4096) * sizeof(double) + (size_t)MAXCH * wp * sizeof(int));
          }
          panel_end.push_back(tf.size());
          level_end.push_back(tf.size());
          continue;
        }
        for (int s : narrow_first) {
          const int u = sn[s].r - sn[s].w;
          const int crows = panel_rows(li.count);
          for (int b = 0; b < (u + crows - 1) / crows; ++b) tf.push_back(base(s, 1, b));
        }
        panel_end.push_back(tf.size());
        for (int pass = 0; pass < 2; ++pass)
          for (int s : narrow_first) {
            const int u = sn[s].r - sn[s].w, nt = fine ? (u + 31) / 32 : (u + 63) / 64;
            std::vector<int> tiles;
            for (int I = 0; I < nt; ++I)
              for (int J = 0; J <= I; ++J) tiles.push_back((I << 16) | J);
            const int stride = fine ? 1 : 2;
            for (size_t k = 0; k < tiles.size(); k += stride) {
              const int t2 = tiles[std::min(k + 1, tiles.size() - 1)];
              const bool hd = h->factor_top_head && (is_head_tile(s, tiles[k] >> 16, fine ? 32 : 64) ||
                                                     (!fine && is_head_tile(s, t2 >> 16, 64)));
              if (hd != (pass == 0)) continue;
              TopFItem t = base(s, 2, tiles[k]);
              t.part2 = fine ? -1 : t2;
              t.sidx = (int)(k / stride);
              t.scount = (int)((tiles.size() + stride - 1) / stride);
              t.head = hd ? 1 : 0;
              tf.push_back(t);
            }
          }
        level_end.push_back(tf.size());
      }
      if (fold) {
        std::vector<TopFItem> out;
        out.reserve(tf.size() + nit);
        int qnext = 0;
        auto filler = [&](int q) {
          const int s = it_front[q];
          TopFItem t;
          memset(&t, 0, sizeof(t));
          t.it.Loff = sn[s].Loff;
          t.it.w = sn[s].w;
          t.it.r = sn[s].r;
          t.it.part = q;
          t.role = 3;
          t.front = s;
          t.part2 = -1;
          if (P.sn_level[s] >= lvl) {
            const int crows = panel_rows(h->levels[P.sn_level[s]].count);
            t.nwait = 1;
            t.target = lfused[P.sn_level[s]] ? (int)nfused(s) : (sn[s].r - sn[s].w + crows - 1) / crows;
          }
          return t;
        };
        std::vector<char> own(ns, 0);
        for (TopFItem& t : tf)
          if (t.role == 0 && t.it.r == t.it.w) {
            t.sidx = first_item[t.front] + 1;
            own[t.front] = 1;
          }
        auto skip_own = [&] {
          while (qnext < nit && own[it_front[qnext]]) ++qnext;
        };
        size_t from = 0;
        for (int l = lvl; l < P.nlevels; ++l) {
          const size_t mid = panel_end[l - lvl], to = level_end[l - lvl];
          out.insert(out.end(), tf.begin() + from, tf.begin() + mid);
          long long room = (long long)h->spanel_fold_room - (long long)(mid - from);
          for (skip_own(); room > 0 && qnext < nit && P.sn_level[it_front[qnext]] <= l; skip_own()) {
            out.push_back(filler(qnext++));
            --room;
          }
          out.insert(out.end(), tf.begin() + mid, tf.begin() + to);
          from = to;
        }
        for (skip_own(); qnext < nit; skip_own()) out.push_back(filler(qnext++));
        tf.swap(out);
        lds = std::max(lds, sp_lds_pre);
        h->sp_folded = true;
      }
      h->ftop_level = lvl;
      h->ftop_count = (int)tf.size();
      h->ftop_lds = lds;
      for (int l = 0; l < lvl; ++l) {
        LevelInfo& lm = h->levels[l];
        if (lm.mini_cnt == 0) continue;
        const int s = P.level_sn[P.level_ptr[l]];
        auto mini = [&](int role, int part) {
          TopFItem t;
          memset(&t, 0, sizeof(t));
          t.it.Loff = sn[s].Loff;
          t.it.Uoff = sn[s].Uoff;
          t.it.w = sn[s].w;
          t.it.r = sn[s].r;
          t.it.part = part;
          t.it.nchild = sn[s].child_end - sn[s].child_begin;
          t.it.pd = pulls[s];
          t.role = role;
          t.front = s;
          t.part2 = 0;
          t.nwait = t.it.nchild;
          for (int k = 0; k < t.nwait; ++k) t.wait_id[k] = P.child_idx[sn[s].child_begin + k];
          t.crows = 64;
          t.prows = panel_rows(1);
          t.post = 1;
          t.xoff = xoff[s];
          t.target = (sn[s].r - sn[s].w + t.prows - 1) / t.prows;
          return t;
        };
        lm.mini_off = (long long)tf.size();
        tf.push_back(mini(0, 0));
        for (int b = 0; b < (sn[s].r - sn[s].w + panel_rows(1) - 1) / panel_rows(1); ++b) tf.push_back(mini(1, b));
        lm.mini_cnt = (int)(tf.size() - (size_t)lm.mini_off);
        lm.mini_lds = std::max(lm.lds_pivot, lm.lds_panel);
      }
      if ((rc = upload(h, h->d_tfitems, tf))) return rc;
    }
  }
  {
    h->fused_solve = false;
    h->n_sitems = 0;
    h->n_sliced = 0;
    bool ok = h->solve_fused && ns > 0;
    for (int s2 = 0; s2 < ns && ok; ++s2) ok = sn[s2].w >= 1 && (h->solve_slices || sn[s2].r <= 1024);
    if (ok) {
      std::vector<SolveItem> si;
      std::vector<long long> xuoff;
      std::vector<int> xinvoff;
      std::vector<int> fx0(ns, 0), fx1(ns, 0);
      std::vector<long long> fpoff(ns, 0);
      si.reserve(nit);
      long long spf = 0, spb = 0, spart = 0;
      int wmax = 1;
      for (int q = 0; q < nit; ++q) {
        const int s2 = it_front[q], sl = it_sl[q], nsl = it_nsl[q];
        SolveItem T;
        memset(&T, 0, sizeof(T));
        T.c0 = sn[s2].c0;
        T.w = sn[s2].w;
        T.r = sn[s2].r;
        T.uoff = sn[s2].uoff;
        T.rowoff = sn[s2].rowoff;
        T.Loff = sn[s2].Loff;
        T.plevel = sn[s2].parent >= 0 ? P.sn_level[sn[s2].parent] : -1;
        const int nch = sn[s2].child_end - sn[s2].child_begin;
        T.nchild = std::min(nch, MAXCH);
        if (sl == 0) {
          fx0[s2] = (int)xuoff.size();
          fpoff[s2] = spart;
          spart += (long long)(nsl - 1) * T.w;
        }
        for (int k = 0; k < nch; ++k) {
          const int ch = P.child_idx[sn[s2].child_begin + k];
          if (k < MAXCH) {
            T.c_uoff[k] = sn[ch].uoff;
            T.c_invoff[k] = sn[ch].pad1;
          } else if (sl == 0) {
            xuoff.push_back(sn[ch].uoff);
            xinvoff.push_back(sn[ch].pad1);
          }
        }
        if (sl == 0) fx1[s2] = (int)xuoff.size();
        T.xbegin = fx0[s2];
        T.xend = fx1[s2];
        T.sl = sl;
        T.nsl = nsl;
        T.poff = fpoff[s2];
        T.a0 = it_a0[q];
        T.a1 = it_a1[q];
        const int ro = (sl == 0 ? T.w : 0) + (T.a1 - T.a0);
        T.Qf = std::max(1, std::min(T.w, 1024 / ro));
        T.Ef = (T.w + T.Qf - 1) / T.Qf;
        T.Pb = std::max(1, std::min(ro, 1024 / T.w));
        T.Eb = (ro + T.Pb - 1) / T.Pb;
        T.spf = spf;
        T.spb = spb;
        spf += ((long long)T.Ef * ro * T.Qf + 1) & ~1LL;
        spb += ((long long)T.Eb * T.w * T.Pb + 1) & ~1LL;
        wmax = std::max(wmax, T.w);
        si.push_back(T);
      }
      h->sp_lds = solve_panel_lds(wmax);
      {
        std::vector<int> lvl_begin(P.nlevels + 1, nit);
        for (int q = nit - 1; q >= 0; --q) lvl_begin[P.sn_level[it_front[q]]] = q;
        for (int l = P.nlevels - 1; l >= 0; --l)
          if (lvl_begin[l] > lvl_begin[l + 1]) lvl_begin[l] = lvl_begin[l + 1];
        for (int l = P.nlevels - 1; l >= 0; --l)
          for (int q = lvl_begin[l]; q < lvl_begin[l + 1];) {
            const int nsl = it_nsl[q];
            for (int k = nsl - 1; k >= 0; --k) {
              const SolveItem t = si[q + k];
              si.push_back(t);
            }
            q += nsl;
          }
      }
      if (h->sp_lds <= 160 * 1024) {
        if ((rc = upload(h, h->d_sitems, si))) return rc;
        if ((rc = upload(h, h->d_sxuoff, xuoff))) return rc;
        if ((rc = upload(h, h->d_sxinvoff, xinvoff))) return rc;
        cold_tick("  upload_plan: descriptors, items, solve lists");
        HCHECK(h, h->d_SPf.ensure(std::max<size_t>((size_t)spf * sizeof(double), 16)));
        HCHECK(h, h->d_SPb.ensure(std::max<size_t>((size_t)spb * sizeof(double), 16)));
        HCHECK(h, hipMemsetAsync(h->d_SPf.p, 0, std::max<size_t>((size_t)spf * sizeof(double), 16), h->stream));
        cold_tick("  upload_plan: solve-panel arenas");
        HCHECK(h, hipMemsetAsync(h->d_SPb.p, 0, std::max<size_t>((size_t)spb * sizeof(double), 16), h->stream));
        HCHECK(h, h->d_xhat.ensure(std::max<size_t>((size_t)P.m * sizeof(double), 16)));
        HCHECK(h, hipMemsetAsync(h->d_xhat.p, 0xFF, std::max<size_t>((size_t)P.m * sizeof(double), 16), h->stream));
        HCHECK(h, h->d_spart.ensure(std::max<size_t>((size_t)spart * sizeof(double), 16)));
        HCHECK(h, hipMemsetAsync(h->d_spart.p, 0xFF, h->d_spart.bytes, h->stream));
        HCHECK(h, hipFuncSetAttribute(reinterpret_cast<const void*>(k_build_solve_panels),
                                      hipFuncAttributeMaxDynamicSharedMemorySize, 160 * 1024));
        h->fused_solve = true;
        h->n_sitems = nit;
        for (int q = 0; q < nit; ++q) h->n_sliced += it_sl[q] == 0 && it_nsl[q] > 1;
        h->sp_bytes = (double)(spf + spb) * sizeof(double);
        h->tb_nT = h->tb_ntf = h->tb_nfb = h->tb_levels = h->tb_nchunks = 0;
        h->tb_valid = false;
        if (h->top_block_after > 0 && P.nlevels >= 4) {
          std::vector<int> lcols(P.nlevels, 0), lfronts(P.nlevels, 0);
          std::vector<char> lsingle(P.nlevels, 1);
          for (int q = 0; q < nit; ++q) {
            const int l = P.sn_level[it_front[q]];
            if (it_sl[q] == 0) {
              lcols[l] += sn[it_front[q]].w;
              lfronts[l] += 1;
            }
            if (it_nsl[q] != 1 || sn[it_front[q]].w > 128) lsingle[l] = 0;
          }
          int ltop = P.nlevels, cols = 0;
          while (ltop > 1 && lsingle[ltop - 1] && lfronts[ltop - 1] <= 32 && cols + lcols[ltop - 1] <= h->top_block_max) {
            --ltop;
            cols += lcols[ltop];
          }
          bool roots_in = true;
          for (int s2 = 0; s2 < ns; ++s2)
            if (sn[s2].parent < 0 && P.sn_level[s2] < ltop) roots_in = false;
          if (P.nlevels - ltop >= 3 && roots_in && cols >= 64) {
            const int nT = cols;
            int nfb = 0;
            while (nfb < nit && P.sn_level[it_front[nfb]] < ltop) ++nfb;
            std::vector<int> tl((size_t)P.m, -1), tpos;
            tpos.reserve((size_t)nT);
            std::vector<int> tf_of(ns, -1);
            std::vector<TopFront> tfronts;
            for (int s2 = 0; s2 < ns; ++s2)
              if (P.sn_level[s2] >= ltop) {
                tf_of[s2] = (int)tfronts.size();
                tfronts.push_back(TopFront{first_item[s2], -1, (int)tpos.size(), 0});
                for (int k = 0; k < sn[s2].w; ++k) {
                  tl[(size_t)(sn[s2].c0 + k)] = (int)tpos.size();
                  tpos.push_back(sn[s2].c0 + k);
                }
              }
            for (int s2 = 0; s2 < ns; ++s2)
              if (tf_of[s2] >= 0 && sn[s2].parent >= 0) tfronts[(size_t)tf_of[s2]].parent = tf_of[sn[s2].parent];
            std::vector<std::vector<long long>> src((size_t)nT);
            bool ok_tb = (int)tpos.size() == nT;
            for (int s2 = 0; s2 < ns && ok_tb; ++s2) {
              if (tf_of[s2] >= 0 || sn[s2].parent < 0 || tf_of[sn[s2].parent] < 0) continue;
              const int u = sn[s2].r - sn[s2].w;
              for (int a = 0; a < u; ++a) {
                const int i = tl[(size_t)P.sn_rows[(size_t)sn[s2].rowoff + sn[s2].w + a]];
                if (i < 0) {
                  ok_tb = false;
                  break;
                }
                src[(size_t)i].push_back(sn[s2].uoff + a);
              }
            }
            {
              long long ng = 0;
              for (const auto& v : src) ng += (long long)v.size();
              if (nT + 1024 + (nT + 1 + ng + 1) / 2 + 8 > TOP_LDS || P.u_size >= (1LL << 31)) ok_tb = false;
            }
            if (ok_tb) {
              std::vector<int> gptr((size_t)nT + 1, 0);
              std::vector<long long> gsrc;
              for (int i = 0; i < nT; ++i) {
                gsrc.insert(gsrc.end(), src[(size_t)i].begin(), src[(size_t)i].end());
                gptr[(size_t)i + 1] = (int)gsrc.size();
              }
              const int kq = std::max(1, (nT + 64 * SOLVE_PREFETCH - 1) / (64 * SOLVE_PREFETCH));
              const int Q = 64 * kq, nr = std::max(1, 1024 / Q), E = (nT + Q - 1) / Q;
              std::vector<TopBlockItem> titems;
              long long off = 0;
              for (int r0 = 0; r0 < nT; r0 += nr) {
                const int n2 = std::min(nr, nT - r0);
                titems.push_back(TopBlockItem{off, r0, n2, Q, E});
                off += ((long long)E * n2 * Q + 1) & ~1LL;
              }
              const int ntf = (int)titems.size();
              std::vector<TopChunk> chunks;
              for (int f2 = 0; f2 < (int)tfronts.size(); ++f2) {
                const int w = si[(size_t)tfronts[(size_t)f2].item].w;
                for (int j0 = 0; j0 < w; j0 += TOP_CB) chunks.push_back(TopChunk{f2, j0});
              }
              std::vector<long long> dsrc((size_t)nT);
              for (const TopFront& F : tfronts) {
                const SolveItem& T = si[(size_t)F.item];
                const long long TSb = (long long)T.w * T.Pb;
                for (int i = 0; i < T.w; ++i)
                  dsrc[(size_t)(F.tl0 + i)] = T.spb + (long long)(i / T.Pb) * TSb + (long long)(i % T.Pb) * T.w + i;
              }
              if ((rc = upload(h, h->d_tb_items, titems))) return rc;
              if ((rc = upload(h, h->d_tb_tpos, tpos))) return rc;
              if ((rc = upload(h, h->d_tb_tl, tl))) return rc;
              if ((rc = upload(h, h->d_tb_gptr, gptr))) return rc;
              if ((rc = upload(h, h->d_tb_gsrc, gsrc))) return rc;
              if ((rc = upload(h, h->d_tb_fronts, tfronts))) return rc;
              if ((rc = upload(h, h->d_tb_chunks, chunks))) return rc;
              if ((rc = upload(h, h->d_tb_dsrc, dsrc))) return rc;
              HCHECK(h, h->d_tb_xtf.ensure((size_t)off * sizeof(double)));
              HCHECK(h, h->d_tb_xd.ensure((size_t)nT * nT * sizeof(double)));
              HCHECK(h, h->d_tb_xhat.ensure((size_t)4 * nT * sizeof(double)));
              HCHECK(h, hipMemsetAsync(h->d_tb_xhat.p, 0xFF, (size_t)4 * nT * sizeof(double), h->stream));
              HCHECK(h, h->d_tb_gathered.ensure(16));
              HCHECK(h, hipMemsetAsync(h->d_tb_gathered.p, 0, 16, h->stream));
              HCHECK(h, hipStreamSynchronize(h->stream));
              h->tb_nT = nT;
              h->tb_ntf = ntf;
              h->tb_nfb = nfb;
              h->tb_levels = P.nlevels - ltop;
              h->tb_nchunks = (int)chunks.size();
            }
          }
        }
      }
    }
    if (h->sp_folded && !h->fused_solve) {
      h->error = "solve-panel items without solve panels";
      return HIPFACT_EINTERNAL;
    }
  }
  {
    size_t solve_lds = 0, asm_lds = 0;
    if (!h->fused_solve)
      for (int l = 0; l < P.nlevels; ++l) solve_lds = std::max(solve_lds, h->levels[l].lds_solve_max);
    for (int l = 0; l < P.nlevels; ++l)
      if (h->levels[l].nA > 0 && !h->levels[l].pull) asm_lds = std::max(asm_lds, h->levels[l].lds_asm);
    char buf[200];
    if (solve_lds > 160 * 1024) {
      snprintf(buf, sizeof buf, "front too large for the LDS-resident solve vectors (%zu KB needed, 160 KB available; "
               "fronts of up to 1024 rows use the fused solve launch instead)", solve_lds >> 10);
      h->error = buf;
      return HIPFACT_EINTERNAL;
    }
    if (max_lds > 160 * 1024 || h->ftop_lds > 160 * 1024 || asm_lds > 160 * 1024) {
      snprintf(buf, sizeof buf, "front too large for the LDS-resident factorisation buffers (%zu KB needed)",
               std::max({max_lds, h->ftop_lds, asm_lds}) >> 10);
      h->error = buf;
      return HIPFACT_EINTERNAL;
    }
  }
  cold_tick("  upload_plan: top block, misc uploads");
  HCHECK(h, hipFuncSetAttribute(reinterpret_cast<const void*>(k_front_assemble),
                                hipFuncAttributeMaxDynamicSharedMemorySize, 160 * 1024));
  for (const void* fn : {reinterpret_cast<const void*>(k_front_pivot<false>), reinterpret_cast<const void*>(k_front_pivot<true>),
                         reinterpret_cast<const void*>(k_front_panel<false>), reinterpret_cast<const void*>(k_front_panel<true>),
                         reinterpret_cast<const void*>(k_front_schur<false>), reinterpret_cast<const void*>(k_front_schur<true>), reinterpret_cast<const void*>(k_front_schur_pair), reinterpret_cast<const void*>(k_factor_top)})
    HCHECK(h, hipFuncSetAttribute(fn, hipFuncAttributeMaxDynamicSharedMemorySize, 160 * 1024));
  HCHECK(h, hipFuncSetAttribute(reinterpret_cast<const void*>(k_factor_level),
                                hipFuncAttributeMaxDynamicSharedMemorySize, 160 * 1024));
  HCHECK(h, hipFuncSetAttribute(reinterpret_cast<const void*>(k_fwd_level),
                                hipFuncAttributeMaxDynamicSharedMemorySize, 160 * 1024));
  HCHECK(h, hipFuncSetAttribute(reinterpret_cast<const void*>(k_bwd_level),
                                hipFuncAttributeMaxDynamicSharedMemorySize, 160 * 1024));
  HCHECK(h, h->d_Kval.ensure(std::max<size_t>((size_t)P.nnzK * sizeof(double), 16)));
  cold_tick("  upload_plan: kernel attributes");
  HCHECK(h, h->d_L.ensure((size_t)P.L_size * sizeof(double) + (size_t)4 * P.nsuper * sizeof(int) + 32));
  HCHECK(h, h->d_U.ensure(std::max<size_t>((size_t)(P.U_size + h->pair_extra) * sizeof(double), 16)));
  HCHECK(h, h->d_uvec.ensure(std::max<size_t>((size_t)P.u_size * sizeof(double), 16)));
  cold_tick("  upload_plan: factor + update arenas");
  HCHECK(h, h->d_y.ensure(std::max<size_t>((size_t)P.m * sizeof(double), 16)));
  HCHECK(h, h->d_ysol.ensure(std::max<size_t>((size_t)2 * P.m * sizeof(double), 16)));
  HCHECK(h, hipMemsetAsync(h->d_uvec.p, 0xFF, std::max<size_t>((size_t)P.u_size * sizeof(double), 16), h->stream));
  HCHECK(h, hipMemsetAsync(h->d_ysol.p, 0xFF, std::max<size_t>((size_t)2 * P.m * sizeof(double), 16), h->stream));
  HCHECK(h, h->d_epoch.ensure(16));
  HCHECK(h, hipMemsetAsync(h->d_epoch.p, 0, 16, h->stream));
  const size_t nb = std::max<size_t>((size_t)std::max(P.N, h->N_ext) * sizeof(double), 16);
  HCHECK(h, h->d_rhs.ensure(nb));
  HCHECK(h, h->d_sol.ensure(nb));
  HCHECK(h, h->d_res.ensure(nb));
  {
    const int drc = dense_upload(h, nb);
    if (drc) return drc;
  }
  h->n_lrows = h->n_rseg = h->n_cseg = h->n_lprod = 0;
  if (P.saddle) {
    std::vector<LongSeg> rs, cs;
    std::vector<LongProd> ls;
    int uid = 0, poff = 0;
    auto cut = [&](std::vector<LongSeg>& out, int id, int b, int e) {
      const int nseg = (e - b + LONG_SEG - 1) / LONG_SEG;
      for (int q = 0; q < nseg; ++q)
        out.push_back(LongSeg{id, b + q * LONG_SEG, std::min(e, b + (q + 1) * LONG_SEG), q, nseg, uid, poff, 0});
      ++uid;
      poff += nseg;
    };
    for (int k = 0; k < P.m; ++k)
      if (P.Ar_ptr[(size_t)k + 1] - P.Ar_ptr[(size_t)k] > LONG_ROW) {
        cut(rs, k, P.Ar_ptr[(size_t)k], P.Ar_ptr[(size_t)k + 1]);
        ++h->n_lrows;
      }
    for (int j = 0; j < P.n; ++j)
      if (P.Kp[(size_t)j + 1] - P.Kp[(size_t)j] - 1 > LONG_COL) cut(cs, j, P.Kp[(size_t)j] + 1, P.Kp[(size_t)j + 1]);
    if (h->n_lrows > 0)
      for (long long e = 0; e + 1 < (long long)P.prod_ptr.size(); ++e) {
        const long long b = P.prod_ptr[(size_t)e], en = P.prod_ptr[(size_t)e + 1];
        if (en - b <= MV_LONG) continue;
        const int nseg = (int)((en - b + MV_LONG - 1) / MV_LONG);
        for (int q = 0; q < nseg; ++q)
          ls.push_back(LongProd{e, b + (long long)q * MV_LONG, std::min(en, b + (long long)(q + 1) * MV_LONG), q, nseg, uid, poff});
        ++uid;
        poff += nseg;
      }
    int lrc;
    if (!rs.empty() && (lrc = upload(h, h->d_rseg, rs))) return lrc;
    if (!cs.empty() && (lrc = upload(h, h->d_cseg, cs))) return lrc;
    if (!ls.empty() && (lrc = upload(h, h->d_lprod, ls))) return lrc;
    h->n_rseg = (int)rs.size();
    h->n_cseg = (int)cs.size();
    h->n_lprod = (int)ls.size();
    if (uid > 0) {
      HCHECK(h, h->d_segpart.ensure((size_t)poff * sizeof(double)));
      HCHECK(h, h->d_segcnt.ensure((size_t)uid * sizeof(unsigned int)));
      HCHECK(h, hipMemsetAsync(h->d_segcnt.p, 0, (size_t)uid * sizeof(unsigned int), h->stream));
      HCHECK(h, hipStreamSynchronize(h->stream));
    }
  }
  if (P.saddle && P.n_late > 0) {
    std::vector<int> mask((size_t)std::max(P.n, 1), -1);
    for (int t = 0; t < P.n_late; ++t) mask[(size_t)P.late_cols[(size_t)t]] = t;
    int lrc;
    if ((lrc = upload(h, h->d_dmask, mask))) return lrc;
    HCHECK(h, h->d_Ar_full.ensure(std::max<size_t>(P.Ar_src.size() * sizeof(double), 16)));
    std::vector<int> cm((size_t)P.m);
    for (int s2 = 0; s2 < P.m; ++s2) cm[(size_t)s2] = s2 < P.my ? P.n + s2 : -2;
    if ((lrc = upload(h, h->d_cmap, cm))) return lrc;
    std::vector<long long> dt((size_t)P.m);
    for (int k = 0; k < P.m; ++k) dt[(size_t)k] = P.Mtarget[P.Mp[k]];
    if ((lrc = upload(h, h->d_diag_target, dt))) return lrc;
    HCHECK(h, hipStreamSynchronize(h->stream));
  }
  HCHECK(h, h->d_info.ensure(INFO_BYTES));
  HCHECK(h, h->d_norms.ensure(3 * sizeof(double) * 4096));
  HCHECK(h, h->h_info.ensure(INFO_WORDS * sizeof(int) + 2 * 64 * sizeof(double)));
  if (!h->d_ctl.p) {
    HCHECK(h, h->d_ctl.ensure(sizeof(RefineCtl)));
    HCHECK(h, hipMemsetAsync(h->d_ctl.p, 0, sizeof(RefineCtl), h->stream));
  }
  if (!h->h_ctl.p) {
    HCHECK(h, h->h_ctl.ensure(sizeof(RefineCtl)));
    memset(h->h_ctl.p, 0, sizeof(RefineCtl));
    HCHECK(h, hipHostGetDevicePointer(&h->h_ctl_dev, h->h_ctl.p, 0));
  }
// ... 16 lines not shown
```

sleqp_amd/csrc/runtime_queue.inc:

```
struct TurnState {
  std::mutex mu;
  hipEvent_t last = nullptr;
  hipfact_handle* owner = nullptr;
  std::atomic<int> live{0};
};
static TurnState g_turn[16];
static hipfact_handle* g_trace_handles[8] = {nullptr};
struct Turn {
  hipfact_handle* h;
  bool counted = false, held = false;
  explicit Turn(hipfact_handle* h_) : h(h_) {
    if (h->capturing) return;
    counted = true;
    if (h->turn_depth++ > 0) return;
    TurnState& T = g_turn[h->device & 15];
    static const bool off = getenv("HIPFACT_NO_TURNS") != nullptr;
    if (off || T.live.load(std::memory_order_acquire) <= 1 || !h->ev_turn) return;
    T.mu.lock();
    held = true;
    if (T.last && T.owner != h) {
      (void)hipStreamWaitEvent(h->stream, T.last, 0);
      h->turn_waits++;
    }
  }
// ... 5 lines not shown
    if (hipEventRecord(h->ev_turn, h->stream) == hipSuccess) {
      T.last = h->ev_turn;
      T.owner = h;
    }
    T.mu.unlock();
  }
  Turn(const Turn&) = delete;
  Turn& operator=(const Turn&) = delete;
};
static void turn_join(hipfact_handle* h) {
  TurnState& T = g_turn[h->device & 15];
  std::lock_guard<std::mutex> g(T.mu);
  if (T.live.fetch_add(1, std::memory_order_acq_rel) == 1) (void)hipDeviceSynchronize();
  for (auto& g : g_trace_handles)
    if (!g) {
      g = h;
      break;
    }
}
static void turn_leave(hipfact_handle* h) {
  TurnState& T = g_turn[h->device & 15];
  std::lock_guard<std::mutex> g(T.mu);
  T.live.fetch_sub(1, std::memory_order_acq_rel);
  for (auto& g : g_trace_handles)
    if (g == h) g = nullptr;
  if (T.owner == h) {
    T.owner = nullptr;
    T.last = nullptr;
  }
}

static DecideIn decide_in(hipfact_handle* h, int col = -1);
static inline bool diag_inactive_needed(const hipfact_handle* h) {
  const Plan& P = h->plan;
  return P.saddle && P.m > 0 && ((h->maps_on && h->n_inactive > 0) || P.n_late > 0);
}
static inline bool row_scale_in_sequence(const hipfact_handle* h) {
  const Plan& P = h->plan;
  return P.saddle && P.n > 0 && P.m > 0;
}
static inline bool dataflow_factor(const hipfact_handle* h) { return h->debug_phases == 15 && !h->no_dataflow; }
static inline bool tree_solve(const hipfact_handle* h) { return h->fused_solve && !h->no_dataflow; }
static inline bool tree_delivers_verdict(const hipfact_handle* h) { return tree_solve(h) && h->plan.m > 0 && h->plan.saddle; }
static inline bool graph_route(const hipfact_handle* h) { return h->use_graph && !h->prof.on && h->debug_phases == 15; }
static inline const int* cmap_or_null(const hipfact_handle* h) { return (h->maps_on || h->plan.n_late > 0) ? h->d_cmap.as<int>() : nullptr; }
static inline bool masked_rows(const hipfact_handle* h) { return h->nd > 0 || h->plan.n_late > 0; }
static inline size_t arena_fill_bytes(const Plan& P) {
  return (size_t)P.L_size * sizeof(double) + (size_t)4 * P.nsuper * sizeof(int);
}
static inline int row_scale_grid(long long m, size_t fill_bytes) {
  const long long nz16 = (long long)((fill_bytes + 15) / 16);
  const int for_fill = (int)std::min<long long>(2048, std::max<long long>(1, nz16 / (FB * 8)));
  return std::max(nblocks(m * 16), for_fill);
}
static int place_rows(int m, const int* Ar_ptr, size_t fill_bytes, int classes, ClassBounds& cb) {
  return place_ranges((long long)m, FB / RL, Ar_ptr, LONG_ROW, classes, row_scale_grid(m, fill_bytes), (long long)((fill_bytes + 15) / 16), cb);
}
static void place_front_end(hipfact_handle* h) {
  const Plan& P = h->plan;
  h->rs_grid = place_rows(P.m, P.Ar_ptr.data(), arena_fill_bytes(P), h->xcd_classes, h->rs_place);
}
template <bool CH>
static void launch_schur(hipfact_handle* h, const LevelInfo& li, int pull) {
  h->prof.next_fl = li.schur_flops;
  if (li.nD <= 0) return;
  const FrontItem* fit = h->d_fitems.as<FrontItem>() + li.itD;
  if (li.pair == 2)
    LAUNCH(PC_FACTOR_D, k_front_schur_pair, dim3(li.nD), dim3(FB), li.lds_schur, fit, h->d_L.as<double>(),
           h->d_U.as<double>(), li.pd);
  else
    LAUNCH(PC_FACTOR_D, k_front_schur<CH>, dim3(li.nD), dim3(FB), li.lds_schur, fit, h->d_L.as<double>(),
           h->d_U.as<double>(), h->d_inv.as<int>(), h->d_rel.as<int>(), h->d_pullx.as<PullDesc>(), pull);
}
static int factor_enqueue(hipfact_handle* h) {
  Turn turn(h);
  const Plan& P = h->plan;
  hipStream_t st = h->stream;
  const size_t fill_bytes = arena_fill_bytes(P);
  const bool fill_rides = row_scale_in_sequence(h);
  if (!fill_rides) {
    HCHECK(h, hipMemsetAsync(h->d_info.p, 0, INFO_BYTES, st));
    if (P.L_size > 0 && fill_bytes > 0) {
      prof_begin(h, PC_MEMSET);
      HCHECK(h, hipMemsetAsync(h->d_L.p, 0, fill_bytes, st));
      prof_end(h);
    }
  }
  const long long nM = (long long)P.Mi.size();
  const int* vmap = h->maps_on ? h->d_vmap.as<int>() : nullptr;
  double* kprod = h->maps_on ? h->d_Kprod.as<double>() : h->d_Ksc.as<double>();
  if (fill_rides) {
    {
      const long long nz16 = (long long)((fill_bytes + 15) / 16);
      const bool masked = masked_rows(h);
      const double* kin = h->vals_ride ? h->vals_ride : h->d_Kval.as<double>();
      if (h->n_rseg > 0)
        LAUNCH(PC_GATHER, k_long_row_norm, dim3(std::min(h->n_rseg, 4096)), dim3(FB), 0, h->n_rseg, h->d_rseg.as<LongSeg>(),
               h->d_Ar_col.as<int>(), h->d_Ar_src.as<int>(), kin, vmap,
               masked ? h->d_dmask.as<int>() : nullptr, P.n_late > 0 ? 1 : 0, h->equilibrate ? 1 : 0,
               h->d_dscale.as<double>(), h->d_segpart.as<double>(), h->d_segcnt.as<unsigned int>());
      LAUNCH(PC_GATHER, k_row_scale, dim3(h->rs_grid), dim3(FB), 0, P.m,
             h->d_Ar_ptr.as<int>(), h->d_Ar_col.as<int>(), h->d_Ar_src.as<int>(), kin, vmap,
             masked ? h->d_dmask.as<int>() : nullptr, h->d_perm.as<int>(), P.n_late > 0 ? P.my : -1,
             h->equilibrate ? 1 : 0, h->d_dscale.as<double>(),
             h->d_Ar_val.as<double>(), masked ? h->d_Ar_full.as<double>() : nullptr, h->d_Ksc.as<double>(), kprod,
             h->vals_ride ? h->d_Kval.as<double>() : nullptr, (long long)P.nnzK,
             reinterpret_cast<double2*>(h->d_L.p), nz16, h->d_info.as<int>(), h->n_rseg,
             h->d_rseg.as<LongSeg>(), decide_in(h), h->decide_rides ? 1 : 0, h->rs_place);
    }
  }
  if (nM > 0) {
    if (P.saddle) {
#define MVALS_LAUNCH(IDX, PK)                                                                                       \
  LAUNCH(PC_MVALS, (k_mvals_prod<IDX, PK>), dim3(nblocks(nM, 1 << 16)), dim3(FB), 0, nM, h->d_prod_ptr.as<IDX>(), \
         h->d_prod_a.as<int>(), h->d_prod_b.as<int>(), h->d_Mtarget.as<IDX>(), kprod,                                  \
         h->d_L.as<double>(), h->n_lprod,                                                                              \
         h->d_lprod.as<LongProd>(), h->d_segpart.as<double>(), h->d_segcnt.as<unsigned int>())
      if (h->idx32 && h->prod_packed)
        MVALS_LAUNCH(unsigned int, true);
      else if (h->idx32)
        MVALS_LAUNCH(unsigned int, false);
      else if (h->prod_packed)
        MVALS_LAUNCH(long long, true);
      else
        MVALS_LAUNCH(long long, false);
#undef MVALS_LAUNCH
    } else {
      LAUNCH(PC_MVALS, k_mvals_src, dim3(nblocks(nM, 1 << 16)), dim3(FB), 0, nM, h->d_src.as<int>(),
                         h->d_Mtarget.as<long long>(), h->d_Kval.as<double>(), h->d_L.as<double>());
    }
  }
  if (diag_inactive_needed(h))
    LAUNCH(PC_GATHER, k_diag_inactive, dim3(nblocks(P.m)), dim3(FB), 0, P.m, h->d_perm.as<int>(), h->d_cmap.as<int>(),
           h->d_diag_target.as<long long>(), h->d_L.as<double>());
  if (P.saddle && h->reg_delta > 0.0 && P.m > 0)
    LAUNCH(PC_GATHER, k_diag_shift, dim3(nblocks(P.m)), dim3(FB), 0, P.m, h->d_perm.as<int>(), cmap_or_null(h),
           h->d_diag_target.as<long long>(), h->d_L.as<double>(), h->reg_delta);
  const bool dataflow = dataflow_factor(h);
  const int lsplit = dataflow ? std::min(h->ftop_level, P.nlevels) : P.nlevels;
  if (h->mini_x_bytes > 0 && dataflow)
    HCHECK(h, hipMemsetAsync(h->d_xarena.as<double>() + h->mini_x_off, 0xFF, h->mini_x_bytes, st));
  for (int l = 0; l < lsplit; ++l) {
    const LevelInfo& li = h->levels[l];
    const int* it = h->d_items.as<int>();
    const int pull = (li.pull && h->debug_phases == 15) ? 1 : 0;
    if (li.nA > 0 && (h->debug_phases & 1) && !pull)
      LAUNCH(PC_FACTOR_A, k_front_assemble, dim3(li.nA), dim3(1024), li.lds_asm, h->d_sn.as<SnDesc>(), it + li.itA, li.nparts,
             h->d_L.as<double>(), h->d_U.as<double>(), h->d_rel.as<int>(), h->d_child.as<int>());
    if (li.split && li.mini_cnt > 0 && dataflow && h->ftop_count > 0) {
      int* flm = reinterpret_cast<int*>(h->d_L.as<double>() + P.L_size);
      LAUNCH(PC_FACTOR_B, k_factor_top, dim3(li.mini_cnt), dim3(512), li.mini_lds,
             h->d_tfitems.as<TopFItem>() + li.mini_off, h->d_L.as<double>(), h->d_U.as<double>(), h->d_info.as<int>(),
             h->d_inv.as<int>(), h->d_rel.as<int>(), flm, flm + P.nsuper, flm + 2 * P.nsuper, h->d_xarena.as<double>(),
             nullptr, nullptr, nullptr);
      launch_schur<false>(h, li, pull);
    } else if (li.split && h->debug_phases == 15) {
      const FrontItem* fit = h->d_fitems.as<FrontItem>();
#define SPLIT_LAUNCHES(CH)                                                                                              \
  LAUNCH(PC_FACTOR_B, k_front_pivot<CH>, dim3(li.count), dim3(512), li.lds_pivot, fit + li.itB, h->d_L.as<double>(),   \
         h->d_U.as<double>(), h->d_info.as<int>(), h->d_inv.as<int>(), h->d_rel.as<int>(), h->d_pullx.as<PullDesc>(), \
         pull);                                                                                                        \
  if (li.nC > 0)                                                                                                       \
    LAUNCH(PC_FACTOR_C, k_front_panel<CH>, dim3(li.nC), dim3(li.panel_threads), li.lds_panel, fit + li.itC,            \
           h->d_L.as<double>(), h->d_U.as<double>(), h->d_inv.as<int>(), h->d_rel.as<int>(),                          \
           h->d_pullx.as<PullDesc>(), pull);                                                                           \
  launch_schur<CH>(h, li, pull);
      if (li.chain) {
        SPLIT_LAUNCHES(true)
      } else {
        SPLIT_LAUNCHES(false)
      }
#undef SPLIT_LAUNCHES
    } else {
      LAUNCH(PC_FACTOR, k_factor_level, dim3(li.count), dim3(FB), li.lds_factor, h->d_sn.as<SnDesc>(),
             h->d_level_sn.as<int>() + li.begin, h->d_L.as<double>(), h->d_U.as<double>(), h->d_rel.as<int>(),
             h->d_child.as<int>(), h->d_info.as<int>(), h->debug_phases);
    }
  }
  if (lsplit < P.nlevels) {
    int* fl = reinterpret_cast<int*>(h->d_L.as<double>() + P.L_size);
    LAUNCH(PC_FACTOR_T, k_factor_top, dim3(h->ftop_count), dim3(512), h->ftop_lds, h->d_tfitems.as<TopFItem>(),
           h->d_L.as<double>(), h->d_U.as<double>(), h->d_info.as<int>(), h->d_inv.as<int>(), h->d_rel.as<int>(), fl,
           fl + P.nsuper, fl + 2 * P.nsuper, h->d_xarena.as<double>(),
           h->sp_folded ? h->d_sitems.as<SolveItem>() : nullptr, h->sp_folded ? h->d_SPf.as<double>() : nullptr,
           h->sp_folded ? h->d_SPb.as<double>() : nullptr);
  }
  if (tree_solve(h) && !(h->sp_folded && lsplit < P.nlevels) && h->n_sitems > 0)
    LAUNCH(PC_SPANEL, k_build_solve_panels, dim3(h->n_sitems), dim3(SPB), h->sp_lds, h->d_sitems.as<SolveItem>(),
           h->d_L.as<double>(), h->d_SPf.as<double>(), h->d_SPb.as<double>());
  HCHECK(h, hipGetLastError());
  return dense_setup_async(h);
}

template <class F>
static int run_cached(hipfact_handle* h, int kind, const void* b, void* z, F enqueue, int passes = 0);

static void flush_decide(hipfact_handle* h);
static void drop_graphs(hipfact_handle* h);
static int reset_dataflow_state(hipfact_handle* h);

static inline bool first_pass_sufficed(const RefineCtl& c) { return c.done && c.status == 0 && c.iters == 0 && c.omega <= 0.25 * c.tol; }
static inline void judge_conditioning(hipfact_handle* h, bool well) {
  h->wc_hint = well;
  h->refine_inline = well ? 0 : std::max(h->refine_inline, std::min(h->refine_steps, 1));
}
static int factor_async(hipfact_handle* h, const double* src = nullptr) {
  const Plan& P = h->plan;
  if (h->no_dataflow && h->df_retry_at >= 0 && h->num_factor >= h->df_retry_at && !h->ctl_pending && !h->decide_deferred &&
      !h->reg_retry) {
    h->no_dataflow = false;
    h->df_retry_at = -1;
    h->dataflow_rearmed++;
    drop_graphs(h);
    h->cache.clear();
    if (const int rrc = reset_dataflow_state(h)) return rrc;
  }
  const bool graphed = graph_route(h);
  const size_t src_bytes = (size_t)P.nnzK * sizeof(double);
  if (!h->reg_retry) {
    h->reg_delta = 0.0;
    h->num_perturbed = 0;
  }
  const bool ride = src && src_bytes > 0 && row_scale_in_sequence(h);
  const bool copy_first = src && src_bytes > 0 && !ride;
  if (!graphed) {
    flush_decide(h);
    if (copy_first) HCHECK(h, hipMemcpyAsync(h->d_Kval.p, src, src_bytes, hipMemcpyDeviceToDevice, h->stream));
  }
  const bool with_decide = graphed && h->decide_deferred;
  const bool with_inactive = diag_inactive_needed(h);
  auto enqueue_all = [&]() -> int {
    if (graphed) {
      h->decide_rides = with_decide && row_scale_in_sequence(h);
      if (with_decide && !h->decide_rides) hipLaunchKernelGGL(k_refine_decide, dim3(1), dim3(FB), 0, h->stream, decide_in(h), 1, 1);
      if (copy_first) HCHECK(h, hipMemcpyAsync(h->d_Kval.p, src, src_bytes, hipMemcpyDeviceToDevice, h->stream));
    }
    h->vals_ride = ride ? src : nullptr;
    const int frc = factor_enqueue(h);
    h->decide_rides = false;
    h->vals_ride = nullptr;
    return frc;
  };
  h->tb_valid = false;
  if (h->factored) h->solves_prev_factor = h->solves_this_factor;
  h->solves_this_factor = 0;
  const int variant = (with_decide ? 4 : 0) + (h->reg_delta > 0.0 ? 8 : 0) + (with_inactive ? 16 : 0);
  h->note('F', variant + (graphed ? 0 : 32));
  const int rc = run_cached(h, 0, graphed ? src : nullptr, nullptr, enqueue_all, variant);
  if (graphed && rc == HIPFACT_OK) h->decide_deferred = false;
  if (rc) return rc;
  h->num_factor++;
  h->sol_prefetched = false;
  h->tb_valid = false;
  h->solves_this_factor = 0;
  h->factored = true;
  h->factor_checked = false;
  h->solved = false;
  h->ctl_pending = false;
  if (h->first_factor_seq < 0) h->first_factor_seq = h->solve_seq;
  if (h->factor_hint_peek && h->refine_adaptive && h->refine_steps > 0) {
    const RefineCtl* hc = h->h_ctl.as<RefineCtl>();
    const int seq = __atomic_load_n(&hc->seq, __ATOMIC_ACQUIRE);
    if (seq > h->first_factor_seq && seq > h->hint_seq_seen) {
      h->hint_seq_seen = seq;
      h->wc_hint = first_pass_sufficed(*hc);
    }
  }
  h->refine_inline = (h->wc_hint && h->refine_adaptive) ? 0 : h->refine_steps;
  h->inline_probe = true;
  h->seq_at_factor = h->solve_seq;
  h->solves_since_check = 0;
  h->check_interval_now = h->refine_check_every;
  return HIPFACT_OK;
}

static int reset_dataflow_state(hipfact_handle* h) {
  const Plan& P = h->plan;
  hipStream_t st = h->stream;
  if (h->d_xarena.p) HCHECK(h, hipMemsetAsync(h->d_xarena.p, 0xFF, h->d_xarena.bytes, st));
  if (h->d_uvec.p) HCHECK(h, hipMemsetAsync(h->d_uvec.p, 0xFF, std::max<size_t>((size_t)P.u_size * sizeof(double), 16), st));
  if (h->d_ysol.p) HCHECK(h, hipMemsetAsync(h->d_ysol.p, 0xFF, std::max<size_t>((size_t)2 * P.m * sizeof(double), 16), st));
  if (h->d_xhat.p) HCHECK(h, hipMemsetAsync(h->d_xhat.p, 0xFF, std::max<size_t>((size_t)P.m * sizeof(double), 16), st));
  if (h->d_spart.p) HCHECK(h, hipMemsetAsync(h->d_spart.p, 0xFF, h->d_spart.bytes, st));
  if (h->d_tb_xhat.p) HCHECK(h, hipMemsetAsync(h->d_tb_xhat.p, 0xFF, h->d_tb_xhat.bytes, st));
  if (h->d_tb_gathered.p) HCHECK(h, hipMemsetAsync(h->d_tb_gathered.p, 0, 16, st));
  if (h->d_epoch.p) HCHECK(h, hipMemsetAsync(h->d_epoch.p, 0, 16, st));
  HCHECK(h, hipMemsetAsync(h->d_info.p, 0, INFO_BYTES, st));
  HCHECK(h, hipMemsetAsync(h->d_ctl.p, 0, sizeof(RefineCtl), st));
  HCHECK(h, hipStreamSynchronize(st));
  memset(h->h_ctl.p, 0, sizeof(RefineCtl));
  h->solve_seq = h->seq_at_factor = 0;
  h->ctl_pending = false;
  return HIPFACT_OK;
}

static void trace_timeout(hipfact_handle* h, const char* msg) {
  static const bool on = getenv("HIPFACT_TRACE_TIMEOUT") != nullptr;
  if (!on) return;
  const Plan& P = h->plan;
  std::vector<int> fl((size_t)4 * P.nsuper);
  if (h->d_L.p && hipMemcpy(fl.data(), h->d_L.as<double>() + P.L_size, fl.size() * sizeof(int), hipMemcpyDeviceToHost) == hipSuccess)
    for (int l = 0; l < P.nlevels; ++l) {
      int open = 0, nb = 0, nc = 0, nd = 0;
      for (int q = P.level_ptr[l]; q < P.level_ptr[l + 1]; ++q) {
        const int sn = P.level_sn[q];
        open += fl[sn] == 0;
        nb += fl[sn];
        nc += fl[P.nsuper + sn];
        nd += fl[2 * P.nsuper + sn];
      }
      fprintf(stderr, "   level %2d fronts %4d  without pivot flag %4d  sums bdone %d cdone %d ddone %d\n", l,
              P.level_ptr[l + 1] - P.level_ptr[l], open, nb, nc, nd);
    }
  fprintf(stderr, "[hipfact %p] %s; factorisation %ld, solve %ld, turn waits %lld, handles on the device %d\n", (void*)h, msg,
          (long)h->num_factor, (long)h->solve_seq, h->turn_waits, g_turn[h->device & 15].live.load());
  fprintf(stderr, "   first solve workgroup that timed out: %d (items %d, top block %d: %d below)\n",
          h->info_host[INFO_TIMEOUT_WG] ? (1 << 30) - h->info_host[INFO_TIMEOUT_WG] : -1, h->n_sitems, (int)h->tb_valid, h->tb_nfb);
  for (hipfact_handle* o : g_trace_handles)
    if (o && o != h) {
      fprintf(stderr, "   other handle %p: factorisations %ld, analyses %ld, turn waits %lld, launches %u, last:", (void*)o,
              (long)o->num_factor, (long)o->analyses, o->turn_waits, o->n_notes);
      for (unsigned k = o->n_notes > 6 ? o->n_notes - 6 : 0; k < o->n_notes; ++k) fprintf(stderr, " %c%d", o->notes[k & 63].kind, o->notes[k & 63].key);
      fprintf(stderr, "\n");
    }
  fprintf(stderr, "   last launches:");
  for (unsigned k = h->n_notes > 64 ? h->n_notes - 64 : 0; k < h->n_notes; ++k)
    fprintf(stderr, " %c%d", h->notes[k & 63].kind, h->notes[k & 63].key);
  fprintf(stderr, "\n");
}

enum class Phase { factor, solve };
static int check_info(hipfact_handle* h, Phase phase = Phase::factor, bool* switched = nullptr) {
  if (switched) *switched = false;
  HCHECK(h, hipMemcpyAsync(h->h_info.p, h->d_info.p, INFO_BYTES, hipMemcpyDeviceToHost, h->stream));
  HCHECK(h, hipStreamSynchronize(h->stream));
  memcpy(h->info_host, h->h_info.p, INFO_WORDS * sizeof(int));
  if (phase == Phase::factor) {
    unsigned long long mm[2];
    memcpy(mm, h->h_info.as<char>() + INFO_WORDS * sizeof(int), sizeof(mm));
    const unsigned long long nlo = ~mm[0];
    double lo, hi;
    memcpy(&lo, &nlo, 8);
    memcpy(&hi, &mm[1], 8);
    h->pivot_ratio = (mm[1] == 0ull) ? 1.0 : ((lo > 0.0 && hi >= lo) ? hi / lo : INFINITY);
  }
  const bool factor_was_checked = h->factor_checked;
  h->factor_checked = true;
  if (h->fake_timeouts > 0) {
    --h->fake_timeouts;
    h->info_host[INFO_TIMEOUT] += 1;
  }
  char buf[200];
  if (h->info_host[INFO_TIMEOUT] != 0) {
    snprintf(buf, sizeof buf, "dependency wait timed out inside the single-launch %s kernels (%d waits)",
             phase == Phase::solve ? "solve" : "factorisation", h->info_host[INFO_TIMEOUT]);
    const bool in_solve = phase == Phase::solve && factor_was_checked;
    if (!in_solve) h->factored = false;
    h->solved = false;
    const int rc = reset_dataflow_state(h);
    h->error = buf;
    trace_timeout(h, buf);
    if (!h->no_dataflow) {
      h->no_dataflow = true;
      h->dataflow_fallbacks++;
      h->df_retry_at = h->df_retry_every > 0
                           ? h->num_factor + ((long)h->df_retry_every << std::min<long>(h->dataflow_fallbacks - 1, 8))
                           : -1;
      drop_graphs(h);
      if (switched) *switched = true;
    }
    return rc ? rc : HIPFACT_EINTERNAL;
  }
  if (h->info_host[INFO_ZERO_PIVOT] > 0) {
    snprintf(buf, sizeof buf, "matrix is singular: %d zero or non-finite pivot(s)", h->info_host[INFO_ZERO_PIVOT]);
    h->error = buf;
    h->factored = false;
    return HIPFACT_ESINGULAR;
  }
  if (h->plan.saddle && h->info_host[INFO_NEG_PIVOT] != h->plan.n_late) {
    snprintf(buf, sizeof buf, "working set is numerically rank deficient: %d negative pivot(s) of A A^T",
             h->info_host[INFO_NEG_PIVOT] - h->plan.n_late);
    h->error = buf;
    h->factored = false;
    return HIPFACT_ESINGULAR;
  }
  return HIPFACT_OK;
}

static inline SaddleMaps saddle_maps(const hipfact_handle* h) {
  SaddleMaps M;
  M.vmap = h->maps_on ? h->d_vmap.as<int>() : nullptr;
  M.cmap = cmap_or_null(h);
  M.dscale = h->d_dscale.as<double>();
  M.n = h->plan.n;
  M.nrseg = h->n_rseg;
  M.ncseg = h->n_cseg;
  M.rseg = h->d_rseg.as<LongSeg>();
  M.cseg = h->d_cseg.as<LongSeg>();
  M.segpart = h->d_segpart.as<double>();
  M.segcnt = h->d_segcnt.as<unsigned int>();
  return M;
}

static void solve_m_async(hipfact_handle* h, const int* skip, const RhsIn* rhs = nullptr, const XupdIn* xup = nullptr) {
  const Plan& P = h->plan;
  if (tree_solve(h)) {
    XupdIn X;
    memset(&X, 0, sizeof(X));
    if (xup) X = *xup;
    TopBlockIn TB;
    memset(&TB, 0, sizeof(TB));
    int nfwd = h->n_sitems, bwd_off = h->n_sitems, nbwd = h->n_sitems;
    if (h->tb_valid && h->tb_nT > 0) {
      TB.nT = h->tb_nT;
      TB.ntf = h->tb_ntf;
      TB.items = h->d_tb_items.as<TopBlockItem>();
      TB.XTf = h->d_tb_xtf.as<double>();
      TB.tpos = h->d_tb_tpos.as<int>();
      TB.gptr = h->d_tb_gptr.as<int>();
      TB.gsrc = h->d_tb_gsrc.as<long long>();
      TB.xhatT2 = h->d_tb_xhat.as<double>();
      TB.gathered2 = h->d_tb_gathered.as<unsigned int>();
      TB.ltop = P.nlevels - h->tb_levels;
      TB.tT2 = TB.xhatT2 + (size_t)2 * h->tb_nT;
      TB.ntr = (rhs && rhs->Ar_ptr) ? (h->tb_nT + (ST / RL) - 1) / (ST / RL) : 0;
      nfwd = nbwd = h->tb_nfb;
      bwd_off = 2 * h->n_sitems - h->tb_nfb;
    }
    const size_t tree_lds = (size_t)(TB.ntf > 0 ? TOP_LDS : TREE_LDS) * sizeof(double);
    LAUNCH(PC_TREE, k_solve_tree, dim3(TB.ntr + nfwd + TB.ntf + nbwd + 1 + X.nblocks), dim3(ST), tree_lds, h->d_sitems.as<SolveItem>(),
           nfwd, bwd_off, nbwd, TB,
           h->d_SPf.as<double>(),
           h->d_SPb.as<double>(), h->d_sxuoff.as<long long>(), h->d_sxinvoff.as<int>(),
           h->d_inv.as<int>(), h->d_rows.as<int>(), h->d_y.as<double>(),
           h->d_xhat.as<double>(), h->d_uvec.as<double>(), h->d_ysol.as<double>(), P.m, h->d_epoch.as<int>(),
           h->d_info.as<int>(), skip, rhs ? *rhs : RhsIn{},
           decide_in(h), h->d_spart.as<double>(), X);
    return;
  }
  for (int l = 0; l < P.nlevels; ++l) {
    const LevelInfo& li = h->levels[l];
    LAUNCH(PC_FWD, k_fwd_level, dim3(li.count), dim3(SB), li.lds_fwd, h->d_sn.as<SnDesc>(),
           h->d_level_sn.as<int>() + li.begin, h->d_L.as<double>(), h->d_rel.as<int>(), h->d_child.as<int>(),
           h->d_y.as<double>(), h->d_uvec.as<double>(), skip);
  }
  for (int l = P.nlevels - 1; l >= 0; --l) {
    const LevelInfo& li = h->levels[l];
    LAUNCH(PC_BWD, k_bwd_level, dim3(li.count), dim3(SB), li.lds_bwd, h->d_sn.as<SnDesc>(),
           h->d_level_sn.as<int>() + li.begin, h->d_L.as<double>(), h->d_rows.as<int>(), h->d_y.as<double>(), skip);
  }
}

static void launch_rhs_saddle(hipfact_handle* h, const SaddleMaps& M, const double* b, const int* skip, double* y = nullptr) {
  const Plan& P = h->plan;
  LAUNCH(PC_RHS, k_rhs_saddle, dim3(nblocks((long long)P.m * 16)), dim3(FB), 0, P.m, h->d_Ar_ptr.as<int>(),
         h->d_Ar_col.as<int>(), h->d_Ar_val.as<double>(), h->d_perm.as<int>(), M, b, y ? y : h->d_y.as<double>(), skip);
}
static void launch_x_saddle(hipfact_handle* h, const SaddleMaps& M, const double* b, double* z, bool acc, const int* skip,
                            int* epoch, const double* y = nullptr) {
  const Plan& P = h->plan;
  auto go = [&](auto ACC) {
    LAUNCH(PC_XUPD, k_x_saddle<decltype(ACC)::value>, dim3(nblocks((long long)P.n * 8)), dim3(FB), 0, P.n, P.m, h->d_Kp.as<int>(),
           h->d_Ksc.as<double>(), h->d_Kc_y.as<int>(), h->d_perm.as<int>(), M, y ? y : h->d_y.as<double>(), b, z, skip, epoch);
  };
  acc ? go(std::true_type()) : go(std::false_type());
}

static void launch_rhs_perm(hipfact_handle* h, const double* b, const int* skip, double* y = nullptr) {
  const Plan& P = h->plan;
  LAUNCH(PC_PERM, k_gather_skip, dim3(nblocks(P.m)), dim3(FB), 0, (long long)P.m, h->d_perm.as<int>(), b,
         y ? y : h->d_y.as<double>(), skip);
}
static void launch_x_perm(hipfact_handle* h, double* z, bool acc, const int* skip, int* epoch, const double* y = nullptr) {
  const Plan& P = h->plan;
  if (!y) y = h->d_y.as<double>();
  if (acc)
    LAUNCH(PC_PERM, k_scatter_acc, dim3(nblocks(P.m)), dim3(FB), 0, (long long)P.m, h->d_perm.as<int>(), y, z, skip, epoch);
  else
    LAUNCH(PC_PERM, k_scatter, dim3(nblocks(P.m)), dim3(FB), 0, (long long)P.m, h->d_perm.as<int>(), y, z, epoch);
}

static void solve_once_async(hipfact_handle* h, const double* b, double* z, bool acc, const int* skip, bool raw = false) {
  Turn turn(h);
  const Plan& P = h->plan;
  if (h->N_ext == 0) return;
  if (h->nd > 0 && !raw) {
    double* const dot_req = h->x_dot_out;
    h->x_dot_out = nullptr;
    solve_once_async(h, b, h->d_dtmp.as<double>(), false, skip, true);
    h->x_dot_out = dot_req;
    dense_correct_async(h, z, acc, skip);
    return;
  }
  const bool tree = tree_solve(h);
  int* epoch = (tree && P.m > 0) ? h->d_epoch.as<int>() : nullptr;
  h->last_rhs_in_tree = h->last_xupd_in_tree = h->last_xupd_blocks = 0;
  if (P.saddle) {
    const SaddleMaps M = saddle_maps(h);
    const bool rhs_in_tree = tree && h->rhs_fused && h->n_lrows == 0;
    const bool whole = tree && h->rhs_fused && h->xupd_fused && P.n > 0 && P.m > 0;
    if (P.m > 0) {
      if (!rhs_in_tree) launch_rhs_saddle(h, M, b, skip);
      const RhsIn R{rhs_in_tree ? h->d_Ar_ptr.as<int>() : nullptr, h->d_Ar_col.as<int>(), h->d_Ar_val.as<double>(), h->d_perm.as<int>(), M, b};
      XupdIn X;
      memset(&X, 0, sizeof(X));
      if (whole) {
        X.n = P.n;
        X.Kp = h->d_Kp.as<int>();
        X.Ksc = h->d_Ksc.as<double>();
        X.Kc_y = h->d_Kc_y.as<int>();
        X.perm = h->d_perm.as<int>();
        X.M = M;
        X.b = b;
        X.z = z;
        X.acc = acc ? 1 : 0;
        X.nblocks = std::max(1, std::min(h->xupd_blocks, (P.n + (ST / 8) - 1) / (ST / 8)));
        if (h->x_dot_out && !acc) {
          X.dot_out = h->x_dot_out;
          h->x_dot_blocks = X.nblocks;
        }
      }
      h->last_rhs_in_tree = rhs_in_tree;
      h->last_xupd_in_tree = whole;
      h->last_xupd_blocks = X.nblocks;
      solve_m_async(h, skip, (rhs_in_tree || whole) ? &R : nullptr, whole ? &X : nullptr);
    }
    if (!whole) launch_x_saddle(h, M, b, z, acc, skip, epoch);
  } else {
    launch_rhs_perm(h, b, skip);
    solve_m_async(h, skip);
    launch_x_perm(h, z, acc, skip, epoch);
  }
}

static const int g_resid_cap = 2048;
static inline int resid_blocks(const Plan& P) {
  return P.saddle ? std::max(2, nblocks((long long)P.N * 8, g_resid_cap) & ~1) : nblocks(P.N, g_resid_cap);
}

static DecideIn decide_in(hipfact_handle* h, int col) {
  const bool own = col >= 0;
  const size_t j = own ? (size_t)col : 0;
  return DecideIn{(own ? h->d_mctl : h->d_ctl).as<RefineCtl>() + j, static_cast<RefineCtl*>(own ? h->h_mctl_dev : h->h_ctl_dev) + j,
                  (own ? h->d_mnorms : h->d_norms).as<double>() + j * 3 * g_resid_cap, resid_blocks(h->plan),
                  h->refine_adaptive ? h->refine_tol : -1.0, minmax_ptr(h)};
}

static void residual_async(hipfact_handle* h, const double* b, const double* z, double* res, bool first,
                           bool defer = false, int col = -1) {
  const Plan& P = h->plan;
  const DecideIn D = decide_in(h, col);
  RefineCtl* ctl = D.ctl;
  double* norms = const_cast<double*>(D.partials);
  int* dflag = defer ? &ctl->pending : nullptr;
  if (P.saddle) {
    LAUNCH(PC_RESID, k_residual_saddle, dim3(resid_blocks(P)), dim3(FB), 0, P.n, P.m, h->d_Kp.as<int>(),
           h->d_Ki.as<int>(), h->d_Kval.as<double>(), h->d_Ar_ptr.as<int>(), h->d_Ar_col.as<int>(),
           (masked_rows(h) ? h->d_Ar_full : h->d_Ar_val).as<double>(), h->d_perm.as<int>(), saddle_maps(h), b, z, res, ctl,
           norms,
           first ? 1 : 0, dflag);
  } else {
    LAUNCH(PC_RESID, k_residual_sym, dim3(resid_blocks(P)), dim3(FB), 0, P.N, h->d_Kp.as<int>(), h->d_Ki.as<int>(),
           h->d_Kval.as<double>(), h->d_Tp.as<int>(), h->d_Ti.as<int>(), h->d_Tsrc.as<int>(), b, z, res, ctl,
           norms, first ? 1 : 0, dflag);
  }
  if (!defer) LAUNCH(PC_RESID, k_refine_decide, dim3(1), dim3(FB), 0, D, first ? 1 : 0, 0);
}

static void flush_decide(hipfact_handle* h) {
  if (!h->decide_deferred) return;
  hipLaunchKernelGGL(k_refine_decide, dim3(1), dim3(FB), 0, h->stream, decide_in(h), 1, 1);
  h->decide_deferred = false;
}

static void drop_graphs(hipfact_handle* h) {
  h->graphs.clear();
  for (auto& st : h->cache) st->graphs.clear();
}
static void drop_solve_graphs(hipfact_handle* h) {
  std::vector<GraphEntry> keep;
  for (auto& g : h->graphs.v) {
    if (g.kind == 0)
      keep.push_back(g);
    else
      (void)hipGraphExecDestroy(g.exec);
  }
  h->graphs.v.swap(keep);
}

static void invalidate_plans(hipfact_handle* h) {
  h->graphs.clear();
  h->have_plan = false;
  h->factored = false;
  h->cache.clear();
}

template <class F>
static int run_cached(hipfact_handle* h, int kind, const void* b, void* z, F enqueue, int passes) {
  auto direct = [&]() -> int {
    Turn turn(h);
    return enqueue();
  };
  auto launch = [&](hipGraphExec_t exec) -> int {
    Turn turn(h);
    HCHECK(h, hipGraphLaunch(exec, h->stream));
    return HIPFACT_OK;
  };
  if (!graph_route(h)) return direct();
  for (auto& g : h->graphs)
    if (g.kind == kind && g.b == b && g.z == z && g.passes == passes) return launch(g.exec);
  Turn turn(h);
  hipGraph_t graph = nullptr;
  if (hipStreamBeginCapture(h->stream, hipStreamCaptureModeThreadLocal) != hipSuccess) {
    (void)hipGetLastError();
    return direct();
  }
  h->capturing = true;
  const int rc = enqueue();
  h->capturing = false;
  const hipError_t e = hipStreamEndCapture(h->stream, &graph);
  if (rc != HIPFACT_OK || e != hipSuccess || !graph) {
    if (graph) (void)hipGraphDestroy(graph);
    (void)hipGetLastError();
    if (rc != HIPFACT_OK) return rc;
    h->use_graph = false;
    return direct();
  }
  hipGraphExec_t exec = nullptr;
  const hipError_t ei = hipGraphInstantiate(&exec, graph, nullptr, nullptr, 0);
  (void)hipGraphDestroy(graph);
  if (ei != hipSuccess || !exec) {
    (void)hipGetLastError();
    h->use_graph = false;
    return direct();
  }
  if (h->graphs.size() >= 16) drop_graphs(h);
  h->graphs.push_back({kind, b, z, passes, exec});
  return launch(exec);
}

static int correct_enqueue(hipfact_handle* h, const double* bb, double* z, int passes) {
  const int* skip = &h->d_ctl.as<RefineCtl>()->done;
  for (int it = 0; it < passes; ++it) {
    solve_once_async(h, h->d_res.as<double>(), z, true, skip);
    residual_async(h, bb, z, h->d_res.as<double>(), false);
  }
  HCHECK(h, hipGetLastError());
  return HIPFACT_OK;
}

static bool defers_decide(const hipfact_handle* h) {
  return h->decide_lazy && h->refine_steps > 0 && h->refine_adaptive && h->refine_inline == 0 && tree_delivers_verdict(h);
}

static inline int top_block_key(const hipfact_handle* h) { return h->tb_valid ? 1000 : 0; }
static inline int solve_graph_key(const hipfact_handle* h, bool defer) {
  return (h->refine_steps > 0 ? (defer ? -2 : h->refine_inline) : -1) + top_block_key(h);
}

static int solve_enqueue(hipfact_handle* h, const double* b, double* z) {
  const double* bb = b;
  if (h->refine_steps > 0 && b == z) {
    HCHECK(h, hipMemcpyAsync(h->d_rhs.p, b, (size_t)h->N_ext * sizeof(double), hipMemcpyDeviceToDevice, h->stream));
    bb = h->d_rhs.as<double>();
  }
  solve_once_async(h, bb, z, false, nullptr);
  if (h->refine_steps > 0 && !h->skip_resid_now) {
    residual_async(h, bb, z, h->d_res.as<double>(), true, defers_decide(h));
    return correct_enqueue(h, bb, z, h->refine_inline);
  }
  HCHECK(h, hipGetLastError());
  return HIPFACT_OK;
}

static int top_block_build(hipfact_handle* h) {
  const int nT = h->tb_nT;
  hipStream_t st = h->stream;
  HCHECK(h, hipMemsetAsync(h->d_tb_xd.p, 0, (size_t)nT * nT * sizeof(double), st));
  HCHECK(h, hipMemsetAsync(h->d_tb_xhat.p, 0xFF, (size_t)4 * nT * sizeof(double), st));
  HCHECK(h, hipMemsetAsync(h->d_tb_gathered.p, 0, 16, st));
  hipLaunchKernelGGL(k_top_inverse, dim3(h->tb_nchunks), dim3(ST), 0, st, h->d_tb_chunks.as<TopChunk>(),
                     h->d_tb_fronts.as<TopFront>(), h->d_sitems.as<SolveItem>(), h->d_SPf.as<double>(), h->d_rows.as<int>(),
                     h->d_tb_tl.as<int>(), h->d_tb_xd.as<double>(), nT);
  TopBlockIn TB;
  memset(&TB, 0, sizeof(TB));
  TB.nT = nT;
  TB.ntf = h->tb_ntf;
  TB.items = h->d_tb_items.as<TopBlockItem>();
  {
    HCHECK(h, h->d_tb_zd.ensure((size_t)nT * nT * sizeof(double)));
    const int nt = (nT + ZT - 1) / ZT;
    HCHECK(h, h->d_tb_dinv.ensure((size_t)nT * sizeof(double)));
    hipLaunchKernelGGL(k_top_dinv, dim3((nT + FB - 1) / FB), dim3(FB), 0, st, nT, h->d_SPb.as<double>(), h->d_tb_dsrc.as<long long>(),
                       h->d_tb_dinv.as<double>());
    const int ntl = nt * (nt + 1) / 2;
    int nwork = 0, maxseg = 1;
    for (int I = 0; I < nt; ++I) {
      const int nsg = (nT - ((I * ZT) & ~(ZC - 1)) + ZS - 1) / ZS;
      nwork += (I + 1) * nsg;
      maxseg = std::max(maxseg, nsg);
    }
    HCHECK(h, h->d_tb_zp.ensure((size_t)maxseg * ntl * ZT * ZT * sizeof(double)));
    hipLaunchKernelGGL(k_top_syrk_mfma, dim3(nwork), dim3(FB), 0, st, h->d_tb_xd.as<double>(), h->d_tb_dinv.as<double>(),
                       h->d_tb_zp.as<double>(), nT);
    hipLaunchKernelGGL(k_top_syrk_reduce, dim3(ntl), dim3(FB), 0, st, h->d_tb_zp.as<double>(), h->d_tb_zd.as<double>(), nT);
    hipLaunchKernelGGL(k_top_format, dim3(h->tb_ntf), dim3(ST), 0, st, TB, h->d_tb_zd.as<double>(), h->d_tb_xtf.as<double>());
  }
  HCHECK(h, hipGetLastError());
  h->tb_valid = true;
  h->tb_builds++;
  h->note('T', 0);
  return HIPFACT_OK;
}

static int top_block_touch(hipfact_handle* h) {
  const int after = (h->solves_prev_factor >= h->top_block_breakeven) ? h->top_block_after
                                                                       : std::max(h->top_block_after, h->top_block_breakeven);
  if (!h->tb_valid && h->tb_nT > 0 && h->top_block_after > 0 && h->solves_this_factor >= after &&
      tree_solve(h) && !h->prof.on && h->debug_phases == 15)
    return top_block_build(h);
  return HIPFACT_OK;
}

static int solve_async(hipfact_handle* h, const double* b, double* z) {
  h->sol_prefetched = false;
  if (h->N_ext == 0) return HIPFACT_OK;
  ++h->solves_this_factor;
  if (int rc = top_block_touch(h)) return rc;
  if (h->refine_steps > 0 && h->refine_adaptive && h->inline_probe && h->solve_seq > h->seq_at_factor) {
    const RefineCtl* hc = h->h_ctl.as<RefineCtl>();
    if (__atomic_load_n(&hc->seq, __ATOMIC_ACQUIRE) == h->solve_seq) {
      judge_conditioning(h, first_pass_sufficed(*hc));
      h->inline_probe = false;
    }
  }
  const bool defer = defers_decide(h);
  if (h->check_interval_now < 1) h->check_interval_now = h->refine_check_every;
  const bool unchecked = defer && (!h->inline_probe || h->wc_hint) && h->check_interval_now > 1 &&
                         (h->solves_since_check % h->check_interval_now) != 0;
  if (!unchecked && h->refine_check_every > 1 && h->solves_since_check >= h->check_interval_now && h->refine_check_backoff > 1)
    h->check_interval_now = std::min(std::max(h->refine_check_max, h->refine_check_every), h->check_interval_now * h->refine_check_backoff);
  h->solves_since_check = unchecked ? h->solves_since_check + 1 : 1;
  h->num_checked += (!unchecked && h->refine_steps > 0);
  if (!tree_delivers_verdict(h)) flush_decide(h);
  h->skip_resid_now = unchecked;
  h->last_solve_checked = !unchecked;
  const int key = solve_graph_key(h, defer);
  h->note(unchecked ? 'U' : 'S', key);
  int rc = unchecked ? solve_enqueue(h, b, z) : run_cached(h, 1, b, z, [&] { return solve_enqueue(h, b, z); }, key);
  h->skip_resid_now = false;
  if (rc) return rc;
  if (!unchecked) h->decide_deferred = defer;
  h->num_solve++;
  h->solved = true;
  if (h->refine_steps > 0 && !unchecked) h->solve_seq++;
  h->ctl_pending = h->refine_steps > 0 && (!unchecked || h->ctl_pending);
  h->last_b = (b == z) ? h->d_rhs.as<double>() : b;
  h->last_z = z;
  return HIPFACT_OK;
}

static bool vtable_can_retry(const hipfact_handle* h);
static int vtable_retry_exact(hipfact_handle* h);
static bool static_pivot_applies(const hipfact_handle* h);
static int static_pivot_retry(hipfact_handle* h, int rc);

enum class Verdict { accepted, stalled, out_of_range };
static Verdict refine_verdict(const hipfact_handle* h, const RefineCtl& c) {
  if (!h->refine_adaptive || c.status == 2) return Verdict::accepted;
  if (c.omega > h->fail_omega) return Verdict::stalled;
  if (h->reg_delta > 0.0 && c.rnorm > h->fail_omega * c.bnorm) return Verdict::out_of_range;
  return Verdict::accepted;
}
static void set_verdict_error(hipfact_handle* h, Verdict v, const RefineCtl& c, int col = -1) {
  char of_col[32] = "", subject[48] = "the right-hand side", buf[260];
  if (col >= 0) {
    snprintf(of_col, sizeof of_col, " of column %d", col);
    snprintf(subject, sizeof subject, "column %d of the right-hand sides", col);
  }
  if (v == Verdict::stalled)
    snprintf(buf, sizeof buf, "working set is numerically singular: iterative refinement%s stalled at backward error %.2e after %d "
             "passes (pivot-ratio condition estimate %.2e)", of_col, c.omega, c.iters, c.kappa);
  else
    snprintf(buf, sizeof buf, "working set is rank deficient and %s is not in the range of K: residual %.2e of %s norm after %d "
             "passes on the statically pivoted factor", subject, c.rnorm / c.bnorm, col >= 0 ? "its" : "the right-hand side's", c.iters);
  h->error = buf;
}
static bool stalled_retry_applies(const hipfact_handle* h) { return static_pivot_applies(h) && !h->no_solve_retry && h->pivot_ratio > 1e14; }

static int finish_solve(hipfact_handle* h, bool* continued = nullptr, bool synced = false) {
  if (continued) *continued = false;
  if (!h->ctl_pending) return HIPFACT_OK;
  const bool verdict_queued_now = h->decide_deferred;
  flush_decide(h);
  if (!synced || verdict_queued_now) HCHECK(h, hipStreamSynchronize(h->stream));
  RefineCtl c;
  memcpy(&c, h->h_ctl.p, sizeof(c));
  int more = 0;
  while (!c.done && h->refine_adaptive && c.iters < h->refine_max) {
    const int passes = std::min(std::max(h->refine_inline, 1), h->refine_max - c.iters);
    const double* b = h->last_b;
    double* z = h->last_z;
    h->note('C', passes + top_block_key(h));
    int rc = run_cached(h, 2, b, z, [&] { return correct_enqueue(h, b, z, passes); }, passes + top_block_key(h));
    if (rc) return rc;
    HCHECK(h, hipStreamSynchronize(h->stream));
    memcpy(&c, h->h_ctl.p, sizeof(c));
    ++more;
  }
  h->ctl_pending = false;
  h->last_ctl = c;
  if (more > 0) h->sol_prefetched = false;
  if (h->inline_probe && h->refine_adaptive && h->refine_steps > 0) {
    if (first_pass_sufficed(c)) judge_conditioning(h, true);
    h->inline_probe = false;
  }
  if (continued) *continued = more > 0;
  if (h->refine_adaptive && c.status == 1 && c.omega > 16.0 * c.tol && !h->no_solve_retry && vtable_can_retry(h)) {
    int rc = vtable_retry_exact(h);
    if (rc) return rc;
    return finish_solve(h, continued);
  }
  if (c.iters > 0) h->num_refined++;
  h->num_passes += c.iters;
  if (more > 0) {
    h->refine_inline = std::min(std::max(h->refine_inline, c.iters), 4);
    h->wc_hint = false;
  }
  const Verdict v = refine_verdict(h, c);
  if (v == Verdict::stalled && stalled_retry_applies(h) && h->last_b && h->last_z) {
    const double* b2 = h->last_b;
    double* z2 = h->last_z;
    if (b2 == z2) return HIPFACT_ESINGULAR;
    if (static_pivot_retry(h, HIPFACT_ESINGULAR) == HIPFACT_OK) {
      if (int r3 = solve_async(h, b2, z2)) return r3;
      return finish_solve(h, continued);
    }
  }
  if (v == Verdict::accepted) return HIPFACT_OK;
  set_verdict_error(h, v, c);
  return HIPFACT_ESINGULAR;
}

static unsigned long long hash_ints(const int* p, size_t n, unsigned long long hsh = 1469598103934665603ull) {
  size_t i = 0;
  for (; i + 1 < n; i += 2) {
// ... 215 lines not shown
```

sleqp_amd/csrc/runtime_types.inc:

```
namespace hipfact {

struct DevBuf {
  void* p = nullptr;
  size_t bytes = 0;
  DevBuf() = default;
  DevBuf(const DevBuf&) = delete;
  DevBuf& operator=(const DevBuf&) = delete;
  DevBuf(DevBuf&& o) noexcept : p(o.p), bytes(o.bytes) {
    o.p = nullptr;
    o.bytes = 0;
  }
  DevBuf& operator=(DevBuf&& o) noexcept {
    if (this != &o) {
      release();
      p = o.p;
      bytes = o.bytes;
      o.p = nullptr;
      o.bytes = 0;
    }
    return *this;
  }
  ~DevBuf() { release(); }
  void release() {
    if (p) (void)hipFree(p);
// ... 25 lines not shown
    if (p) (void)hipHostFree(p);
    p = nullptr;
    bytes = 0;
    hipError_t e = hipHostMalloc(&p, n, hipHostMallocDefault);
    if (e == hipSuccess) bytes = n;
    return e;
  }
  template <class T>
  T* as() const {
    return static_cast<T*>(p);
  }
};

struct LevelInfo {
  int begin = 0, count = 0;
  size_t lds_factor = 0, lds_fwd = 0, lds_bwd = 0;
  bool split = false;
  bool pull = false;
  bool chain = false;
  int nparts = 1;
  long long itA = 0;
  long long itB = 0, itC = 0, itD = 0;
  int nA = 0, nC = 0, nD = 0;
  int panel_threads = 512;
  size_t lds_pivot = 0, lds_panel = 0, lds_schur = 0, lds_asm = 0, lds_solve_max = 0;
  int pair = 0;
  PairDesc pd;
  double schur_flops_full = 0.0, pair_flops_done = 0.0;
  bool compactD = false;
  double schur_flops = 0.0;
  long long mini_off = 0;
  int mini_cnt = 0;
  size_t mini_lds = 0;
};

enum ProfClass { PC_MEMSET = 0, PC_MVALS, PC_GATHER, PC_FACTOR, PC_FACTOR_A, PC_FACTOR_B, PC_FACTOR_C, PC_FACTOR_D, PC_FACTOR_T, PC_FWD, PC_BWD, PC_RHS, PC_XUPD, PC_RESID, PC_AXPY, PC_PERM, PC_SPANEL, PC_TREE, PC_COUNT };
static const char* const kProfNames[PC_COUNT] = {"memset", "mvals", "gather", "factor", "factorA", "factorB", "factorC",
                                                 "factorD", "factorT", "fwd", "bwd", "rhs", "xupd", "resid", "axpy", "perm",
                                                 "spanel", "tree"};

struct Prof {
  bool on = false;
  std::vector<hipEvent_t> ev;
  std::vector<int> cls;
  size_t used = 0;
  double ms[PC_COUNT] = {0};
  double max_ms[PC_COUNT] = {0};
  std::vector<double> fl;
  double next_fl = 0.0;
  std::vector<std::pair<double, double>> tagged;
  long cnt[PC_COUNT] = {0};
  ~Prof() {
    for (hipEvent_t e : ev) (void)hipEventDestroy(e);
  }
};

}

using namespace hipfact;

static thread_local std::string g_create_error;

constexpr size_t CG_DOTS_DOUBLES =
    (size_t)(5 * CG_BLOCKS + 3 * (DOT_BLOCKS > 1024 ? DOT_BLOCKS : 1024)) > (size_t)(2 * 3 * DOT_BLOCKS + 8 + 1024)
        ? (size_t)(5 * CG_BLOCKS + 3 * (DOT_BLOCKS > 1024 ? DOT_BLOCKS : 1024))
        : (size_t)(2 * 3 * DOT_BLOCKS + 8 + 1024);

struct GraphEntry {
  int kind;
  const void* b;
  void* z;
  int passes;
  hipGraphExec_t exec;
};

struct GraphList {
  std::vector<GraphEntry> v;
  GraphList() = default;
  GraphList(const GraphList&) = delete;
  GraphList& operator=(const GraphList&) = delete;
  GraphList(GraphList&& o) noexcept : v(std::move(o.v)) { o.v.clear(); }
  GraphList& operator=(GraphList&& o) noexcept {
    if (this != &o) {
      clear();
      v = std::move(o.v);
      o.v.clear();
    }
    return *this;
  }
  ~GraphList() { clear(); }
  void clear() {
    for (auto& g : v) (void)hipGraphExecDestroy(g.exec);
    v.clear();
  }
  size_t size() const { return v.size(); }
  std::vector<GraphEntry>::iterator begin() { return v.begin(); }
  std::vector<GraphEntry>::iterator end() { return v.end(); }
  void push_back(const GraphEntry& g) { v.push_back(g); }
};

struct FactorMemo {
  bool solved = false;
  long solves_this_factor = 0;
  int refine_inline = 1;
  bool inline_probe = true;
  bool wc_hint = false;
  FactorMemo put_back_over(const FactorMemo& now) const {
    FactorMemo r = *this;
    r.inline_probe = now.inline_probe;
    if (inline_probe) {
      r.refine_inline = now.refine_inline;
      r.wc_hint = now.wc_hint;
    }
    return r;
  }
};

struct PlanState : FactorMemo {
  Plan plan;
  bool have_plan = false, factored = false;
  bool factor_checked = false;
  bool prod_packed = false;
  bool idx32 = false;
  unsigned long long key_hash = 0;
  bool from_jacobian = false;
  std::vector<int> Jp, Ji;
  std::vector<int> sidx;
  int m_struct = 0;
  bool maps_on = false;
  int N_ext = 0;
  int n_inactive = 0;
  int n_bounds = 0;
  unsigned long long use_stamp = 0;
  int seq_at_factor = 0;
  int hint_seq_seen = -1;
  int first_factor_seq = -1;
  GraphList graphs;
  int ftop_level = 1 << 30, ftop_count = 0;
  size_t ftop_lds = 0;
  long long mini_x_off = 0;
  size_t mini_x_bytes = 0;
  double ent_fused = 0, ent_split = 0, rows_fused = 0, rows_split = 0;
  std::vector<LevelInfo> levels;
  DevBuf d_sn, d_level_sn, d_rows, d_rel, d_child, d_Mtarget, d_prod_ptr, d_prod_a, d_prod_b, d_src;
  DevBuf d_items, d_fitems, d_inv, d_tfitems, d_pullx;
  DevBuf d_perm, d_Ar_ptr, d_Ar_col, d_Ar_src, d_Ar_val, d_Kp, d_Ki, d_Kc_y, d_Tp, d_Ti, d_Tsrc;
  DevBuf d_xarena;
  DevBuf d_ysol;
  DevBuf d_Kval, d_L, d_U, d_uvec, d_y, d_rhs, d_sol, d_res;
  DevBuf d_Ksc, d_Kprod, d_dscale, d_vmap, d_cmap, d_diag_target, d_sidx, d_srow, d_jtarget;
  bool fused_solve = false;
  size_t sp_lds = 0;
  double sp_bytes = 0;
  DevBuf d_SPf, d_SPb, d_sitems, d_xhat, d_sxuoff, d_sxinvoff, d_epoch, d_spart;
  int n_sitems = 0;
  int n_sliced = 0;
  int n_resorted = 0;
  int last_rhs_in_tree = 0, last_xupd_in_tree = 0, last_xupd_blocks = 0;
  int tb_nT = 0, tb_ntf = 0, tb_nfb = 0, tb_levels = 0, tb_nchunks = 0;
  bool tb_valid = false;
  long solves_prev_factor = 1 << 20;
  DevBuf d_tb_gathered;
  DevBuf d_tb_zd, d_tb_items, d_tb_xtf, d_tb_tpos, d_tb_tl, d_tb_gptr, d_tb_gsrc, d_tb_xhat, d_tb_xd, d_tb_fronts,
      d_tb_chunks, d_tb_dsrc, d_tb_dinv, d_tb_zp;
  int nd = 0, dense_cap = 0;
  DevBuf d_dmask, d_dcols, d_Bq, d_Zq, d_dtmp, d_dG, d_dMinv, d_dw, d_dfix;
  DevBuf d_Ar_full;
  DevBuf d_rseg, d_cseg, d_lprod, d_segpart, d_segcnt;
  int n_rseg = 0, n_cseg = 0, n_lprod = 0;
  ClassBounds rs_place = {};
  int rs_grid = 1;
  int dealt_multi = 0;
  int n_lrows = 0;
  DevBuf d_mY, d_mU, d_mR, d_mB;
  DevBuf d_mitems, d_mslab, d_mcnt;
  std::vector<int> mitem_ptr;
  int mitems_for = -1;
  int n_mcut = 0, n_mslices = 0;
  size_t mcnt_bytes = 0;
  DevBuf d_xvec;

  PlanState() = default;
  PlanState(PlanState&&) = default;
  PlanState& operator=(PlanState&&) = default;
};

#define VTABLE_SUPERSET_TYPES
#include "vtable_superset.inc"
#undef VTABLE_SUPERSET_TYPES

struct SingleSolveMemo {
  const double* last_b = nullptr;
  double* last_z = nullptr;
  RefineCtl last_ctl = {1, 0, 0, 0, 0, 0, 0.0, 0.0, 0.0, 0.0};
  bool last_solve_checked = true;
  bool sol_prefetched = false;
  int refine_check_every = 8;
  int check_interval_now = 0;
  long solves_since_check = 0;
  long num_solve = 0, num_checked = 0, num_refined = 0, num_passes = 0;
};

struct hipfact_handle : PlanState, SingleSolveMemo {
  std::atomic<int> refcount{1};
  int device = 0;
  hipStream_t stream = nullptr;
  hipStream_t side = nullptr;
  hipEvent_t ev_fork = nullptr, ev_join = nullptr;
  hipEvent_t ev_turn = nullptr;
  int turn_depth = 0;
  struct LaunchNote { char kind; int key; };
  LaunchNote notes[64];
  unsigned n_notes = 0;
  void note(char kind, int key) { notes[n_notes++ & 63] = LaunchNote{kind, key}; }
  long long turn_waits = 0;
  bool capturing = false;
  std::string error;
  PlanParams prm;
  std::vector<std::unique_ptr<PlanState>> cache;
  int plan_cache_max = 4;
  bool chain_fuse = true;
  bool solve_slices = true;
  bool speculate = true;
  bool xupd_fused = true;
  bool rhs_fused = true;
  bool spanel_fold = true;
  int spanel_fold_room = 224;
  bool sp_folded = false;
  bool solve_fused = true;
  bool assemble_superset = true;
  bool spmv_stream = true;
  long long spmv_stream_min = 4 << 20;
  bool exact_pattern = false;
  bool superset_vtable = true;
  std::unique_ptr<VirtualJ> vj{new VirtualJ};
  DevBuf d_kin, d_vsrc;
  DevBuf d_retry_b;
  long vtable_retries = 0;
  long dense_fallbacks = 0;
  bool jdev_valid = false;
  unsigned long long jdev_hash = 0;
  int jdev_n = 0, jdev_nnz = 0;
  unsigned long long use_clock = 0;
  long plan_swaps = 0;
  int refine_steps = 1;
  int refine_max = 10;
  bool refine_adaptive = true;
  double refine_tol = 1e-10;
  double fail_omega = 1e-8;
  bool static_pivot = true;
  double static_delta = 1e-8;
  double reg_delta = 0.0;
  bool reg_retry = false;
  int num_perturbed = 0;
  long static_pivot_runs = 0;
  std::string warning;
  bool equilibrate = true;
  bool decide_lazy = true;
  int refine_check_backoff = 2;
  int refine_check_max = 64;
  double pivot_ratio = 1.0;
  bool no_solve_retry = false;
  long dense_probes = 0;
  bool skip_resid_now = false;
  bool decide_deferred = false;
  bool decide_rides = false;
  const double* vals_ride = nullptr;
  bool ctl_pending = false;
  int solve_seq = 0;
  bool use_graph = true;
  bool no_dataflow = false;
  int fake_timeouts = 0;
  long dataflow_fallbacks = 0;
  int df_retry_every = 256;
  long df_retry_at = -1;
  long dataflow_rearmed = 0;
  int debug_phases = 15;
  int solve_whole_max = 48;
  bool factor_hint_peek = true;
  int top_block_breakeven = 48;
  bool chain_pairs = true;
  int n_pairs = 0;
  long long pair_extra = 0;
  double schur_flops_max = 0.0;
  bool check_launches = false, launch_reported = false;
  double* x_dot_out = nullptr;
  int x_dot_blocks = 0;
  int xupd_blocks = 256;
  bool solve_sorted = true;
  int xcd_classes = 8;
  int factor_top_max = 160;
  int factor_top_levels = 1 << 20;
  int factor_top_max_u = 1024;
  int factor_top_fine = 12;
  int top_block_after = 2;
  int top_block_max = 2048;
  long tb_builds = 0;
  bool factor_top_head = true;
  int factor_top_fused = 30;
  int factor_top_fused32 = 12;
  int factor_top_fused_u = 256;
  int factor_top_post = 64;
  int panel_small_below = 0;
  int pull_max_children = 4;
  long cache_hits = 0, analyses = 0, num_factor = 0;
  int info_host[INFO_WORDS] = {0, 0, 0, 0};
  Prof prof;
// ... 98 lines not shown
```

Before: 1469 factor+solve/s.

## Drop separate backward solve panel and reuse forward panel with stored diagonal inverse

Removes the SPb arena that held a transposed, diagonal-scaled copy of each supernode panel for the backward solve. The backward solve now reads the forward panel SPf in plain column-major layout, plus a small per-item vector of diagonal inverses stored after it, and scales the triangular part on the fly. This halves the panel-build writes and memory footprint during factorization and drops the strided offset tables from LDS. In exchange the backward solve's access pattern changes: threads are remapped to (k,p), and a partial-sum transpose through LDS plus an extra barrier are added.

Measured after the change: 1498 factor+solve/s, median of 6. 1.02x the previous value.

```diff
diff --git a/sleqp_amd/csrc/abi_options.inc b/sleqp_amd/csrc/abi_options.inc
--- a/sleqp_amd/csrc/abi_options.inc
+++ b/sleqp_amd/csrc/abi_options.inc
@@ -244,7 +244,6 @@
   if (!strcmp(name, "L")) b = &h->d_L;
   else if (!strcmp(name, "U")) b = &h->d_U;
   else if (!strcmp(name, "SPf")) b = &h->d_SPf;
-  else if (!strcmp(name, "SPb")) b = &h->d_SPb;
   else if (!strcmp(name, "sitems")) b = &h->d_sitems;
   else if (!strcmp(name, "y")) b = &h->d_y;
   else if (!strcmp(name, "xhat")) b = &h->d_xhat;
@@ -370,7 +369,7 @@
   INFO("num_perturbed", h->num_perturbed) INFO("static_pivot_runs", h->static_pivot_runs) INFO("static_pivot_shift", h->reg_delta)
   INFO("num_zero_pivots", h->info_host[INFO_ZERO_PIVOT]) INFO("num_neg_pivots", h->info_host[INFO_NEG_PIVOT])
   INFO("cache_hits", h->cache_hits) INFO("plan_swaps", h->plan_swaps) INFO("plans_cached", h->cache.size())
-  INFO("no_dataflow", h->no_dataflow) INFO("dataflow_fallbacks", h->dataflow_fallbacks) INFO("turn_waits", (double)h->turn_waits) INFO("dataflow_rearmed", h->dataflow_rearmed) INFO("fused_solve", h->fused_solve) INFO("spanel_folded", h->sp_folded) INFO("solve_items", h->n_sitems) INFO("chain_levels_fused", [&] { int c = 0; for (const LevelInfo& li : h->levels) c += li.mini_cnt > 0; return c; }()) INFO("solve_panel_bytes", h->sp_bytes) INFO("spf_bytes", (double)h->d_SPf.bytes) INFO("spb_bytes", (double)h->d_SPb.bytes) INFO("sitem_bytes", (double)sizeof(SolveItem)) INFO("N_internal", P.N) INFO("maps_on", h->maps_on) INFO("m_struct", h->m_struct) INFO("analyses", h->analyses) INFO("num_factor", h->num_factor) INFO("cg_device_runs", h->cg_device_runs) INFO("cg_device_fallbacks", h->cg_device_fallbacks) INFO("lz_device_runs", h->lz_device_runs) INFO("lz_device_fallbacks", h->lz_device_fallbacks) INFO("lz_device_iterations", h->lz_device_iterations) INFO("lsqr_runs", h->lsqr_runs) INFO("lsqr_iters", h->lsqr_iters) INFO("dense_columns", h->nd) INFO("late_columns", P.n_late) INFO("late_rows", P.n_late_rows) INFO("m_rows", P.saddle ? P.my : P.m) INFO("vtable_rows", h->vj->rows()) INFO("vtable_retries", h->vtable_retries) INFO("dense_fallbacks", h->dense_fallbacks) INFO("dense_probes", h->dense_probes) INFO("top_block_cols", h->tb_nT) INFO("top_block_below", h->tb_nfb) INFO("top_block_levels", h->tb_levels) INFO("top_block_items", h->tb_ntf) INFO("top_block_builds", h->tb_builds) INFO("top_block_active", h->tb_valid) INFO("superset_vtable", h->superset_vtable) INFO("exact_pattern", h->exact_pattern) INFO("spmv_stream", h->spmv_stream)
+  INFO("no_dataflow", h->no_dataflow) INFO("dataflow_fallbacks", h->dataflow_fallbacks) INFO("turn_waits", (double)h->turn_waits) INFO("dataflow_rearmed", h->dataflow_rearmed) INFO("fused_solve", h->fused_solve) INFO("spanel_folded", h->sp_folded) INFO("solve_items", h->n_sitems) INFO("chain_levels_fused", [&] { int c = 0; for (const LevelInfo& li : h->levels) c += li.mini_cnt > 0; return c; }()) INFO("solve_panel_bytes", h->sp_bytes) INFO("spf_bytes", (double)h->d_SPf.bytes) INFO("sitem_bytes", (double)sizeof(SolveItem)) INFO("N_internal", P.N) INFO("maps_on", h->maps_on) INFO("m_struct", h->m_struct) INFO("analyses", h->analyses) INFO("num_factor", h->num_factor) INFO("cg_device_runs", h->cg_device_runs) INFO("cg_device_fallbacks", h->cg_device_fallbacks) INFO("lz_device_runs", h->lz_device_runs) INFO("lz_device_fallbacks", h->lz_device_fallbacks) INFO("lz_device_iterations", h->lz_device_iterations) INFO("lsqr_runs", h->lsqr_runs) INFO("lsqr_iters", h->lsqr_iters) INFO("dense_columns", h->nd) INFO("late_columns", P.n_late) INFO("late_rows", P.n_late_rows) INFO("m_rows", P.saddle ? P.my : P.m) INFO("vtable_rows", h->vj->rows()) INFO("vtable_retries", h->vtable_retries) INFO("dense_fallbacks", h->dense_fallbacks) INFO("dense_probes", h->dense_probes) INFO("top_block_cols", h->tb_nT) INFO("top_block_below", h->tb_nfb) INFO("top_block_levels", h->tb_levels) INFO("top_block_items", h->tb_ntf) INFO("top_block_builds", h->tb_builds) INFO("top_block_active", h->tb_valid) INFO("superset_vtable", h->superset_vtable) INFO("exact_pattern", h->exact_pattern) INFO("spmv_stream", h->spmv_stream)
   INFO("boundary_fast", h->boundary_fast) INFO("bd_count", h->bd_count) INFO("bd_stage_us", h->bd_stage_us) INFO("bd_queue_us", h->bd_queue_us) INFO("bd_rhs_us", h->bd_rhs_us) INFO("bd_device_us", h->bd_device_us) INFO("bd_d2h_us", h->bd_d2h_us) INFO("bd_wait_us", h->bd_wait_us) INFO("bd_copyout_us", h->bd_copyout_us)
   INFO("multi_solves", h->multi_solves) INFO("multi_cols", h->multi_cols) INFO("multi_blocks", h->multi_blocks)
   INFO("multi_passes", h->multi_passes) INFO("multi_single_cols", h->multi_single_cols) INFO("multi_failed_col", h->multi_failed_col)
diff --git a/sleqp_amd/csrc/device_types.h b/sleqp_amd/csrc/device_types.h
--- a/sleqp_amd/csrc/device_types.h
+++ b/sleqp_amd/csrc/device_types.h
@@ -63,7 +63,7 @@
 };
 
 struct SolveItem {
-  long long spf, spb;
+  long long spf, spd;
   long long uoff, rowoff;
   int c0, w, r, nchild;
   int Qf, Ef, Pb, Eb;
diff --git a/sleqp_amd/csrc/kernels_factor_top.inc b/sleqp_amd/csrc/kernels_factor_top.inc
--- a/sleqp_amd/csrc/kernels_factor_top.inc
+++ b/sleqp_amd/csrc/kernels_factor_top.inc
@@ -26,15 +26,14 @@
 }
 
 __device__ __forceinline__ void dev_build_solve_panel(const SolveItem& T, const double* __restrict__ L,
-                                                      double* __restrict__ SPf, double* __restrict__ SPb, double* lds);
+                                                      double* __restrict__ SPf, double* lds);
 
 __global__ __launch_bounds__(512) void k_factor_top(const TopFItem* __restrict__ items, double* __restrict__ L,
                                                    double* __restrict__ U, int* __restrict__ info,
                                                    const int* __restrict__ inv, const int* __restrict__ rel,
                                                    int* __restrict__ bdone, int* __restrict__ cdone,
                                                    int* __restrict__ ddone, double* __restrict__ xarena,
-                                                   const SolveItem* __restrict__ sitems, double* __restrict__ SPf,
-                                                   double* __restrict__ SPb) {
+                                                   const SolveItem* __restrict__ sitems, double* __restrict__ SPf) {
   extern __shared__ __attribute__((aligned(16))) double lds[];
   const TopFItem& T = items[blockIdx.x];
   const FrontItem& S = T.it;
@@ -60,7 +59,7 @@
       __syncthreads();
     }
     TRW(1);
-    dev_build_solve_panel(sitems[S.part], L, SPf, SPb, lds);
+    dev_build_solve_panel(sitems[S.part], L, SPf, lds);
 #ifdef HIPFACT_TRACE
     __syncthreads();
 #endif
@@ -98,18 +97,11 @@
       const SolveItem& Q = sitems[T.sidx - 1];
       const int w = c.w, r = c.r, lda = c.lda;
       const int lane = threadIdx.x & 63, wave = threadIdx.x >> 6;
-      const long long TSf = (long long)r * Q.Qf, TSb = (long long)w * Q.Pb;
       double* __restrict__ sf = SPf + Q.spf;
-      double* __restrict__ sb = SPb + Q.spb;
-      for (int k = wave; k < w; k += 8) {
-        const long long of = (long long)(k / Q.Qf) * TSf + (long long)(k % Q.Qf) * r;
-        for (int i = k + lane; i < w; i += 64) sf[of + i] = (i == k) ? 1.0 : c.A[i + k * lda];
-      }
-      for (int i = wave; i < w; i += 8) {
-        const double di = 1.0 / c.dd[i];
-        const long long ob = (long long)(i / Q.Pb) * TSb + (long long)(i % Q.Pb) * w;
-        for (int k = lane; k <= i; k += 64) sb[ob + k] = ((i == k) ? 1.0 : c.A[i + k * lda]) * di;
-      }
+      double* __restrict__ sd = SPf + Q.spd;
+      for (int k = wave; k < w; k += 8)
+        for (int i = k + lane; i < w; i += 64) sf[(long long)k * r + i] = (i == k) ? 1.0 : c.A[i + k * lda];
+      for (int i = threadIdx.x; i < w; i += blockDim.x) sd[i] = 1.0 / c.dd[i];
     }
   } else if (T.role == 1) {
     TRW(5);
diff --git a/sleqp_amd/csrc/kernels_solve_panels.inc b/sleqp_amd/csrc/kernels_solve_panels.inc
--- a/sleqp_amd/csrc/kernels_solve_panels.inc
+++ b/sleqp_amd/csrc/kernels_solve_panels.inc
@@ -1,7 +1,7 @@
 #define SPST(p, v) (*(p) = (v))
 
 __device__ __forceinline__ void dev_build_solve_panel(const SolveItem& T, const double* __restrict__ L,
-                                                      double* __restrict__ SPf, double* __restrict__ SPb, double* lds) {
+                                                      double* __restrict__ SPf, double* lds) {
   const int w = T.w, r = T.r;
   const int ua = T.a0, u = T.a1 - T.a0;
   const int top = (T.sl == 0) ? w : 0;
@@ -14,8 +14,6 @@
   double* X = lds;
   double* dinv = X + (size_t)ldx * wp;
   double* tile = dinv + wp + (size_t)wave * (16 * 17);
-  long long* offF = reinterpret_cast<long long*>(dinv + wp + (SPB / 64) * (16 * 17));
-  long long* offB = offF + wp;
   const int nstrip = (u + 15) >> 4;
   double av[32];
   {
@@ -47,13 +45,9 @@
       }
   }
   for (int k = tid; k < wp; k += SPB) dinv[k] = (k < w) ? 1.0 / Pn[k + (long long)k * r] : 1.0;
-  const int Qf = T.Qf, Pb = T.Pb;
-  const long long TSf = (long long)ro * Qf, TSb = (long long)w * Pb;
-  for (int k = tid; k < wp; k += SPB) offF[k] = (long long)(k / Qf) * TSf + (long long)(k % Qf) * ro;
-  for (int i = tid; i < ro; i += SPB) offB[i] = (long long)(i / Pb) * TSb + (long long)(i % Pb) * w;
   __syncthreads();
   double* __restrict__ sf = SPf + T.spf;
-  double* __restrict__ sb = SPb + T.spb;
+  const int lb = lk * ro + top + li;
   for (int st = wave; st < nstrip; st += SPB / 64) {
     const int a0 = st << 4;
     d4_t acc[8];
@@ -83,17 +77,16 @@
       if (kt >= nbk) continue;
 #pragma unroll
       for (int q = 0; q < 4; ++q) {
-        const int row = lk + 4 * q, k = 16 * kt + li, i = top + a0 + row;
+        const int row = lk + 4 * q;
         tile[row * 17 + li] = -acc[kt][q];
-        if (a0 + row < u && k < w) SPST(&sb[offB[i] + k], -acc[kt][q]);
       }
       __builtin_amdgcn_fence(__ATOMIC_RELEASE, "wavefront");
       __builtin_amdgcn_wave_barrier();
       __builtin_amdgcn_fence(__ATOMIC_ACQUIRE, "wavefront");
 #pragma unroll
       for (int q = 0; q < 4; ++q) {
-        const int row = li, col = lk + 4 * q, k = 16 * kt + col, i = top + a0 + row;
-        if (a0 + row < u && k < w) SPST(&sf[offF[k] + i], tile[row * 17 + col]);
+        const int row = li, col = lk + 4 * q, k = 16 * kt + col;
+        if (a0 + row < u && k < w) SPST(&sf[lb + ((16 * kt + 4 * q) * ro + a0)], tile[row * 17 + col]);
       }
       __builtin_amdgcn_fence(__ATOMIC_RELEASE, "wavefront");
       __builtin_amdgcn_wave_barrier();
@@ -101,15 +94,12 @@
   }
   if (top == 0) return;
   for (int k = wave; k < w; k += SPB / 64)
-    for (int i = k + lane; i < w; i += 64) SPST(&sf[offF[k] + i], X[i + k * ldx]);
-  for (int i = wave; i < w; i += SPB / 64) {
-    const double di = dinv[i];
-    for (int k = lane; k <= i; k += 64) SPST(&sb[offB[i] + k], X[i + k * ldx] * di);
-  }
+    for (int i = k + lane; i < w; i += 64) SPST(&sf[k * ro + i], X[i + k * ldx]);
+  double* __restrict__ sd = SPf + T.spd;
+  for (int i = tid; i < w; i += SPB) SPST(&sd[i], dinv[i]);
 }
 __global__ __launch_bounds__(SPB) void k_build_solve_panels(const SolveItem* __restrict__ items,
-                                                            const double* __restrict__ L, double* __restrict__ SPf,
-                                                            double* __restrict__ SPb) {
+                                                            const double* __restrict__ L, double* __restrict__ SPf) {
   extern __shared__ __attribute__((aligned(16))) double lds[];
-  dev_build_solve_panel(items[blockIdx.x], L, SPf, SPb, lds);
+  dev_build_solve_panel(items[blockIdx.x], L, SPf, lds);
 }
diff --git a/sleqp_amd/csrc/kernels_solve_tree.inc b/sleqp_amd/csrc/kernels_solve_tree.inc
--- a/sleqp_amd/csrc/kernels_solve_tree.inc
+++ b/sleqp_amd/csrc/kernels_solve_tree.inc
@@ -199,7 +199,7 @@
 }
 
 template <bool DEFER_RESET>
-__device__ __forceinline__ void dev_solve_bwd(const SolveItem& T, const double* __restrict__ SPb,
+__device__ __forceinline__ void dev_solve_bwd(const SolveItem& T, const double* __restrict__ SPf,
                                               const int* __restrict__ rows, double* __restrict__ y,
                                               double* __restrict__ xhat, double* __restrict__ uvec,
                                               double* __restrict__ ysol, double* __restrict__ spart, double* lds,
@@ -212,23 +212,34 @@
   const int ro = top + nu;
   const int TS = w * P;
   const bool active = tid < TS;
-  const int p = active ? tid / w : 0;
+  const int k = active ? tid / P : 0;
+  const int p = tid - k * P;
   double* tv = lds;
   double* part = lds + ro;
-  const double* __restrict__ sp = SPb + T.spb + tid;
+  const int myrow = (tid >= top && tid < ro) ? rows[T.rowoff + w + a0 + (tid - top)] : -1;
+  const double dv = (tid < top) ? SPf[T.spd + tid] : 0.0;
+  const double* __restrict__ sp = SPf + T.spf + (long long)k * ro + p;
   double pv[SOLVE_PREFETCH];
-  const int mycol_b = tid - p * w;
 #pragma unroll
   for (int e = 0; e < SOLVE_PREFETCH; ++e) {
     const int row = p + P * e;
-    pv[e] = (active && e < E && !(row < top && row < mycol_b)) ? sp[(long long)e * TS] : 0.0;
-  }
-  const int myrow = (tid >= top && tid < ro) ? rows[T.rowoff + w + a0 + (tid - top)] : -1;
-  if (tid < top) {
-    tv[tid] = poll_f64(xhat + T.c0 + tid, info);
-    sent_f64_agent(xhat + T.c0 + tid);
-  } else if (myrow >= 0) {
-    tv[tid] = poll_f64(ysol + myrow, info);
+    pv[e] = (active && e < E && row < ro && !(row < top && row < k)) ? sp[P * e] : 0.0;
+  }
+  const double* __restrict__ slot = (tid < top) ? xhat + T.c0 + tid : (myrow >= 0 ? ysol + myrow : nullptr);
+  unsigned long long bits = slot ? __hip_atomic_load(reinterpret_cast<const unsigned long long*>(slot), __ATOMIC_RELAXED,
+                                                     __HIP_MEMORY_SCOPE_AGENT)
+                                 : 0ull;
+  if (tid < top) part[tid] = dv;
+  __syncthreads();
+#pragma unroll
+  for (int e = 0; e < SOLVE_PREFETCH; ++e) {
+    const int row = p + P * e;
+    if (active && row < top && row >= k) pv[e] *= part[row];
+  }
+  if (slot) {
+    if (bits == SOLVE_SENT) bits = (unsigned long long)__double_as_longlong(poll_f64(slot, info));
+    tv[tid] = __longlong_as_double((long long)bits);
+    if (tid < top) sent_f64_agent(xhat + T.c0 + tid);
   }
   if constexpr (!DEFER_RESET) {
     if (tid >= top && tid < ro) sent_f64_agent(uvec + T.uoff + a0 + (tid - top));
@@ -239,8 +250,8 @@
   for (int e = 0; e < SOLVE_PREFETCH; ++e)
     if (e < E) acc = fma(pv[e], tv[min(p + P * e, ro - 1)], acc);
   for (int e = SOLVE_PREFETCH; e < E; ++e)
-    if (active && !(p + P * e < top && p + P * e < mycol_b)) acc = fma(sp[(long long)e * TS], tv[min(p + P * e, ro - 1)], acc);
-  if (active) part[tid] = acc;
+    if (active) acc = fma(p + P * e < ro ? sp[P * e] : 0.0, tv[min(p + P * e, ro - 1)], acc);
+  if (active) part[p * w + k] = acc;
   __syncthreads();
   if (tid < w) {
     double s2 = 0.0;
@@ -367,10 +378,10 @@
   if (tid == 0) __hip_atomic_fetch_add(B.gathered2 + par, 1u, __ATOMIC_RELAXED, __HIP_MEMORY_SCOPE_AGENT);
 }
 
-__global__ __launch_bounds__(FB) void k_top_dinv(int nT, const double* __restrict__ SPb, const long long* __restrict__ dsrc,
+__global__ __launch_bounds__(FB) void k_top_dinv(int nT, const double* __restrict__ SPf, const long long* __restrict__ dsrc,
                                                  double* __restrict__ dinv) {
   const int c = blockIdx.x * FB + threadIdx.x;
-  if (c < nT) dinv[c] = SPb[dsrc[c]];
+  if (c < nT) dinv[c] = SPf[dsrc[c]];
 }
 __device__ __forceinline__ int top_syrk_nseg(int nT, int I) {
   const int cstart = (I * ZT) & ~(ZC - 1);
@@ -651,7 +662,7 @@
 
 __global__ __launch_bounds__(ST) void k_solve_tree(const SolveItem* __restrict__ items, int nfwd, int bwd_off, int nbwd,
                                                    TopBlockIn TB,
-                                                   const double* __restrict__ SPf, const double* __restrict__ SPb,
+                                                   const double* __restrict__ SPf,
                                                    const long long* __restrict__ xuoff,
                                                    const int* __restrict__ xinvoff, const int* __restrict__ inv,
                                                    const int* __restrict__ rows, double* __restrict__ y,
@@ -704,9 +715,9 @@
   } else {
     const SolveItem& T = items[bwd_off + (b - nfwd - ntop)];
     if (TB.ntf > 0 && T.plevel >= TB.ltop)
-      dev_solve_bwd<true>(T, SPb, rows, y, xhat, uvec, ysol2 + (size_t)par * m, spart, lds, info, TB.gathered2 + par, TB.ntf);
+      dev_solve_bwd<true>(T, SPf, rows, y, xhat, uvec, ysol2 + (size_t)par * m, spart, lds, info, TB.gathered2 + par, TB.ntf);
     else
-      dev_solve_bwd<false>(T, SPb, rows, y, xhat, uvec, ysol2 + (size_t)par * m, spart, lds, info);
+      dev_solve_bwd<false>(T, SPf, rows, y, xhat, uvec, ysol2 + (size_t)par * m, spart, lds, info);
   }
   epoch_read_done();
 }
diff --git a/sleqp_amd/csrc/runtime_plan.inc b/sleqp_amd/csrc/runtime_plan.inc
--- a/sleqp_amd/csrc/runtime_plan.inc
+++ b/sleqp_amd/csrc/runtime_plan.inc
@@ -61,7 +61,7 @@
 
 static size_t solve_panel_lds(int wmax) {
   const size_t wp = (size_t)((wmax + 15) & ~15);
-  return (wp * (wp + 1) + wp + 8 * 16 * 17 + wp + 1024) * sizeof(double);
+  return (wp * (wp + 1) + wp + 8 * 16 * 17) * sizeof(double);
 }
 
 static int dense_upload(hipfact_handle* h, size_t vec_bytes);
@@ -756,7 +756,7 @@
       std::vector<int> fx0(ns, 0), fx1(ns, 0);
       std::vector<long long> fpoff(ns, 0);
       si.reserve(nit);
-      long long spf = 0, spb = 0, spart = 0;
+      long long spf = 0, spart = 0;
       int wmax = 1;
       for (int q = 0; q < nit; ++q) {
         const int s2 = it_front[q], sl = it_sl[q], nsl = it_nsl[q];
@@ -800,9 +800,8 @@
         T.Pb = std::max(1, std::min(ro, 1024 / T.w));
         T.Eb = (ro + T.Pb - 1) / T.Pb;
         T.spf = spf;
-        T.spb = spb;
-        spf += ((long long)T.Ef * ro * T.Qf + 1) & ~1LL;
-        spb += ((long long)T.Eb * T.w * T.Pb + 1) & ~1LL;
+        T.spd = spf + (long long)T.Ef * ro * T.Qf;
+        spf += ((long long)T.Ef * ro * T.Qf + (sl == 0 ? T.w : 0) + 1) & ~1LL;
         wmax = std::max(wmax, T.w);
         si.push_back(T);
       }
@@ -828,10 +827,8 @@
         if ((rc = upload(h, h->d_sxinvoff, xinvoff))) return rc;
         cold_tick("  upload_plan: descriptors, items, solve lists");
         HCHECK(h, h->d_SPf.ensure(std::max<size_t>((size_t)spf * sizeof(double), 16)));
-        HCHECK(h, h->d_SPb.ensure(std::max<size_t>((size_t)spb * sizeof(double), 16)));
         HCHECK(h, hipMemsetAsync(h->d_SPf.p, 0, std::max<size_t>((size_t)spf * sizeof(double), 16), h->stream));
-        cold_tick("  upload_plan: solve-panel arenas");
-        HCHECK(h, hipMemsetAsync(h->d_SPb.p, 0, std::max<size_t>((size_t)spb * sizeof(double), 16), h->stream));
+        cold_tick("  upload_plan: solve-panel arena");
         HCHECK(h, h->d_xhat.ensure(std::max<size_t>((size_t)P.m * sizeof(double), 16)));
         HCHECK(h, hipMemsetAsync(h->d_xhat.p, 0xFF, std::max<size_t>((size_t)P.m * sizeof(double), 16), h->stream));
         HCHECK(h, h->d_spart.ensure(std::max<size_t>((size_t)spart * sizeof(double), 16)));
@@ -841,7 +838,7 @@
         h->fused_solve = true;
         h->n_sitems = nit;
         for (int q = 0; q < nit; ++q) h->n_sliced += it_sl[q] == 0 && it_nsl[q] > 1;
-        h->sp_bytes = (double)(spf + spb) * sizeof(double);
+        h->sp_bytes = (double)spf * sizeof(double);
         h->tb_nT = h->tb_ntf = h->tb_nfb = h->tb_levels = h->tb_nchunks = 0;
         h->tb_valid = false;
         if (h->top_block_after > 0 && P.nlevels >= 4) {
@@ -926,9 +923,7 @@
               std::vector<long long> dsrc((size_t)nT);
               for (const TopFront& F : tfronts) {
                 const SolveItem& T = si[(size_t)F.item];
-                const long long TSb = (long long)T.w * T.Pb;
-                for (int i = 0; i < T.w; ++i)
-                  dsrc[(size_t)(F.tl0 + i)] = T.spb + (long long)(i / T.Pb) * TSb + (long long)(i % T.Pb) * T.w + i;
+                for (int i = 0; i < T.w; ++i) dsrc[(size_t)(F.tl0 + i)] = T.spd + i;
               }
               if ((rc = upload(h, h->d_tb_items, titems))) return rc;
               if ((rc = upload(h, h->d_tb_tpos, tpos))) return rc;
diff --git a/sleqp_amd/csrc/runtime_queue.inc b/sleqp_amd/csrc/runtime_queue.inc
--- a/sleqp_amd/csrc/runtime_queue.inc
+++ b/sleqp_amd/csrc/runtime_queue.inc
@@ -181,7 +181,7 @@
       LAUNCH(PC_FACTOR_B, k_factor_top, dim3(li.mini_cnt), dim3(512), li.mini_lds,
              h->d_tfitems.as<TopFItem>() + li.mini_off, h->d_L.as<double>(), h->d_U.as<double>(), h->d_info.as<int>(),
              h->d_inv.as<int>(), h->d_rel.as<int>(), flm, flm + P.nsuper, flm + 2 * P.nsuper, h->d_xarena.as<double>(),
-             nullptr, nullptr, nullptr);
+             nullptr, nullptr);
       launch_schur<false>(h, li, pull);
     } else if (li.split && h->debug_phases == 15) {
       const FrontItem* fit = h->d_fitems.as<FrontItem>();
@@ -211,12 +211,11 @@
     LAUNCH(PC_FACTOR_T, k_factor_top, dim3(h->ftop_count), dim3(512), h->ftop_lds, h->d_tfitems.as<TopFItem>(),
            h->d_L.as<double>(), h->d_U.as<double>(), h->d_info.as<int>(), h->d_inv.as<int>(), h->d_rel.as<int>(), fl,
            fl + P.nsuper, fl + 2 * P.nsuper, h->d_xarena.as<double>(),
-           h->sp_folded ? h->d_sitems.as<SolveItem>() : nullptr, h->sp_folded ? h->d_SPf.as<double>() : nullptr,
-           h->sp_folded ? h->d_SPb.as<double>() : nullptr);
+           h->sp_folded ? h->d_sitems.as<SolveItem>() : nullptr, h->sp_folded ? h->d_SPf.as<double>() : nullptr);
   }
   if (tree_solve(h) && !(h->sp_folded && lsplit < P.nlevels) && h->n_sitems > 0)
     LAUNCH(PC_SPANEL, k_build_solve_panels, dim3(h->n_sitems), dim3(SPB), h->sp_lds, h->d_sitems.as<SolveItem>(),
-           h->d_L.as<double>(), h->d_SPf.as<double>(), h->d_SPb.as<double>());
+           h->d_L.as<double>(), h->d_SPf.as<double>());
   HCHECK(h, hipGetLastError());
   return dense_setup_async(h);
 }
@@ -459,8 +458,7 @@
     const size_t tree_lds = (size_t)(TB.ntf > 0 ? TOP_LDS : TREE_LDS) * sizeof(double);
     LAUNCH(PC_TREE, k_solve_tree, dim3(TB.ntr + nfwd + TB.ntf + nbwd + 1 + X.nblocks), dim3(ST), tree_lds, h->d_sitems.as<SolveItem>(),
            nfwd, bwd_off, nbwd, TB,
-           h->d_SPf.as<double>(),
-           h->d_SPb.as<double>(), h->d_sxuoff.as<long long>(), h->d_sxinvoff.as<int>(),
+           h->d_SPf.as<double>(), h->d_sxuoff.as<long long>(), h->d_sxinvoff.as<int>(),
            h->d_inv.as<int>(), h->d_rows.as<int>(), h->d_y.as<double>(),
            h->d_xhat.as<double>(), h->d_uvec.as<double>(), h->d_ysol.as<double>(), P.m, h->d_epoch.as<int>(),
            h->d_info.as<int>(), skip, rhs ? *rhs : RhsIn{},
@@ -720,7 +718,7 @@
     HCHECK(h, h->d_tb_zd.ensure((size_t)nT * nT * sizeof(double)));
     const int nt = (nT + ZT - 1) / ZT;
     HCHECK(h, h->d_tb_dinv.ensure((size_t)nT * sizeof(double)));
-    hipLaunchKernelGGL(k_top_dinv, dim3((nT + FB - 1) / FB), dim3(FB), 0, st, nT, h->d_SPb.as<double>(), h->d_tb_dsrc.as<long long>(),
+    hipLaunchKernelGGL(k_top_dinv, dim3((nT + FB - 1) / FB), dim3(FB), 0, st, nT, h->d_SPf.as<double>(), h->d_tb_dsrc.as<long long>(),
                        h->d_tb_dinv.as<double>());
     const int ntl = nt * (nt + 1) / 2;
     int nwork = 0, maxseg = 1;
diff --git a/sleqp_amd/csrc/runtime_types.inc b/sleqp_amd/csrc/runtime_types.inc
--- a/sleqp_amd/csrc/runtime_types.inc
+++ b/sleqp_amd/csrc/runtime_types.inc
@@ -201,7 +201,7 @@
   bool fused_solve = false;
   size_t sp_lds = 0;
   double sp_bytes = 0;
-  DevBuf d_SPf, d_SPb, d_sitems, d_xhat, d_sxuoff, d_sxinvoff, d_epoch, d_spart;
+  DevBuf d_SPf, d_sitems, d_xhat, d_sxuoff, d_sxinvoff, d_epoch, d_spart;
   int n_sitems = 0;
   int n_sliced = 0;
   int n_resorted = 0;
```
